# wztzjhn/quantum_basis

Hardware: AMD Instinct MI355X
Metric: lanczos_iters_per_sec (higher is better)
Workload: dtype complex128

## Files before the change

quantum_basis_amd/csrc/qbh_api.cpp:

```cpp
#include <algorithm>
#include <chrono>
#include <cmath>
#include <cstdarg>
#include <cstdlib>
#include <cstring>
#include <initializer_list>
#include <limits>
#include <mutex>
#include <new>
#include <vector>

#include "qbh_api_priv.hpp"

using qbh::d2;
using namespace qbhapi;

namespace qbh {
static thread_local char g_err[512] = "";

void set_error(const char *fmt, ...)
{
    va_list ap;
    va_start(ap, fmt);
    vsnprintf(g_err, sizeof(g_err), fmt, ap);
    va_end(ap);
}

static void parse_debug(const char *e, DebugSw &d)
{
    d = DebugSw{};
    if (!e || !*e) return;
    struct Key { const char *name; int *i; long long *ll; };
    const Key keys[] = {{"flags", &d.flags, nullptr}, {"colmask", &d.colmask, nullptr}, {"tpr", &d.tpr, nullptr}, {"unroll", &d.unroll, nullptr},
                        {"grid", &d.grid, nullptr}, {"wave_tpr", &d.wave_tpr, nullptr}, {"chunk_mult", &d.chunk_mult, nullptr},
                        {"trace_create", &d.trace_create, nullptr}, {"trace_tune", &d.trace_tune, nullptr}, {"trace_dict", &d.trace_dict, nullptr},
                        {"print_ptrs", &d.print_ptrs, nullptr}, {"sec_walk", &d.sec_walk, nullptr}, {"sec_grid", &d.sec_grid, nullptr}, {"sec_tile", &d.sec_tile, nullptr},
                        {"sec_unroll", &d.sec_unroll, nullptr}, {"create_chunk", nullptr, &d.create_chunk},
                        {"force_ragged", &d.force_ragged, nullptr}, {"mf_row", &d.mf_row, nullptr}, {"mf_chunk", &d.mf_chunk, nullptr},
                        {"mf_window", &d.mf_window, nullptr}, {"kronc_abl", &d.kronc_abl, nullptr}, {"kronc_far_chunk", &d.kronc_far_chunk, nullptr},
                        {"kronc_far_ng", &d.kronc_far_ng, nullptr}, {"kronc_far_nt", &d.kronc_far_nt, nullptr}, {"no_far_align", &d.no_far_align, nullptr}, {"far_cols8", &d.far_cols8, nullptr},
                        {"far_vals8", &d.far_vals8, nullptr},
                        {"near_lens", &d.near_lens, nullptr}, {"near_len_cap", &d.near_len_cap, nullptr},
                        {"no_defer", &d.no_defer, nullptr}, {"pipe_nospec", &d.pipe_nospec, nullptr}, {"host_delay_us", &d.host_delay_us, nullptr},
                        {"side_noprio", &d.side_noprio, nullptr}, {"comm_reserve", &d.comm_reserve, nullptr}, {"comm_far_cap", &d.comm_far_cap, nullptr}};
    const std::string all(e);
    size_t pos = 0;
    while (pos <= all.size()) {
        size_t end = all.find(',', pos);
        if (end == std::string::npos) end = all.size();
        const std::string item = all.substr(pos, end - pos);
        pos = end + 1;
        if (item.empty()) continue;
        const size_t eq = item.find('=');
        if (eq == std::string::npos) {
            if (item.find_first_not_of("0123456789") == std::string::npos) d.flags = atoi(item.c_str());
            else fprintf(stderr, "qbhip: QBH_DEBUG: '%s' is not key=value\n", item.c_str());
            continue;
        }
        const std::string k = item.substr(0, eq), v = item.substr(eq + 1);
        bool known = false;
        for (const Key &key : keys)
            if (k == key.name) {
                if (key.i) *key.i = atoi(v.c_str());
                else *key.ll = atoll(v.c_str());
                known = true;
            }
        if (!known) fprintf(stderr, "qbhip: QBH_DEBUG: unknown key '%s'\n", k.c_str());
    }
}

const DebugSw &debug_sw()
{
    static std::mutex mu;
    static std::string seen = "\x01";
    static DebugSw sw[2];
    static int cur = 0;
    const char *e = getenv("QBH_DEBUG");
    std::lock_guard<std::mutex> lock(mu);
    if (seen != (e ? e : "")) {
        seen = e ? e : "";
        cur ^= 1;
        parse_debug(e, sw[cur]);
    }
    return sw[cur];
}
}

extern "C" const char *qbh_last_error(void) { return qbh::g_err; }

extern "C" const char *qbh_strerror(int code)
{
    switch (code) {
    case QBH_OK:        return "success";
    case QBH_EINVAL:    return "invalid argument";
    case QBH_ENODEVICE: return "no HIP device available (libqbhip has no CPU fallback)";
    case QBH_EHIP:      return "HIP runtime call failed";
    case QBH_ENOMEM:    return "out of memory";
    case QBH_ENOTHERM:  return "matrix is not Hermitian";
    case QBH_ECOMM:     return "communicator hook failed";
    case QBH_ENOTNORM:  return "Lanczos start vector is not normalised";
    case QBH_ENOCONV:   return "tridiagonal eigen-solver did not converge";
    case QBH_EUNSUPP:   return "not supported";
    default:            return "unknown error";
    }
}

extern "C" int qbh_version(void) { return QBH_VERSION; }

extern "C" int qbh_device_count(void)
{
    int n = 0;
    if (hipGetDeviceCount(&n) != hipSuccess) {
        (void)hipGetLastError();
        return 0;
    }
    return n;
}

namespace qbhapi {
std::mutex g_defaults_mu;
bool g_have_defaults = false;
qbh_opts g_defaults;
}

extern "C" void qbh_opts_set_default(const qbh_opts *o)
{
    std::lock_guard<std::mutex> lock(g_defaults_mu);
    g_have_defaults = o != nullptr;
    if (o) {
        g_defaults = *o;
        g_defaults.device = -1;
        g_defaults.stream = nullptr;
    }
}

extern "C" void qbh_opts_default(qbh_opts *o)
{
    if (!o) return;
    {
        std::lock_guard<std::mutex> lock(g_defaults_mu);
        if (g_have_defaults) {
            *o = g_defaults;
            return;
        }
    }
    qbh::opts_builtin(o);
}

void qbh::opts_builtin(qbh_opts *o)
{
    o->device = -1;
    o->stream = nullptr;
    o->spmv_kernel = QBH_KERNEL_AUTO;
    o->nnz_per_block = 0;
    o->xcd_swizzle = 2;
    o->value_dict = 1;
    o->profile = 0;
    o->check_hermitian = 1;
    o->real_fast_path = 1;
    o->kron_split = 1;
    o->kron_cols16 = 1;
    o->kron_sliced = 1;
    o->kron_band = 0;
    o->kron_cross_in_near = 1;
    o->kron_coded = -1;
    o->kron_uniform = 7;
    o->gather_parts = 0;
    o->wave_walk = -1;
    o->tile_fold = 1;
    o->autotune = 1;
    o->shard_split = 1;
    o->real_forms = 7;
    o->basis_detect = 1;
    o->sector_orbit = 1;
    o->lanczos_pipeline = 1;
    o->real_wire = 1;
    o->sector_cut = 0;
    o->comm_reserve = 0;
    o->sparse_gather = 1;
    o->major_partition = 0;
    o->kron_minor = 0;
    o->deterministic = 0;
    o->basis_kind = QBH_BASIS_NONE;
    o->n_sites = o->n_up = o->n_dn = 0;
}

namespace qbhapi {

double now_ms()
{
    using namespace std::chrono;
    return duration<double, std::milli>(steady_clock::now().time_since_epoch()).count();
}

int require_device(const qbh_opts *opts, int *dev_out)
// ... 545 lines not shown
                                     int take_ownership, const qbh_opts *opts)
{
    if (!out || !d_ia || !d_ja || !d_val || nrows <= 0 || ncols <= 0 || nnz < 0 || row_offset < 0 ||
        row_offset + nrows > ncols) {
        qbh::set_error("qbh_csr_create_device: invalid argument");
        return QBH_EINVAL;
    }
    if (ncols >= (int64_t)std::numeric_limits<int32_t>::max()) {
        qbh::set_error("ncols %lld does not fit int32 columns", (long long)ncols);
        return QBH_EUNSUPP;
    }
    qbh_csr *A = nullptr;
    QBH_TRY(new_handle(&A, opts));
    A->nrows = nrows;
    A->ncols = ncols;
    A->row_offset = row_offset;
    A->nnz = nnz;
    A->d_ia = d_ia;
    A->d_ja = d_ja;
    A->d_val = reinterpret_cast<d2 *>(d_val);
    A->own_arrays = take_ownership != 0;
    int rc = finalize(A);
    if (rc != QBH_OK) {
        if (!take_ownership && A->d_ia == d_ia) A->own_arrays = false;
        if (!take_ownership && A->d_ia == d_ia) A->d_ia = nullptr, A->d_ja = nullptr, A->d_val = nullptr;
        qbh_csr_destroy(A);
        return rc;
    }
    *out = A;
    return QBH_OK;
}

int qbh::adopt_coded_csr(qbh_csr **out, int64_t nrows, int64_t ncols, int64_t row_offset, int64_t nnz, int64_t *d_ia,
                         int32_t *d_ja, uint8_t *d_code, qbh::d2 *d_dict, int n_dict, const qbh_opts *opts)
{
    if (!out || !d_ia || !d_ja || !d_code || !d_dict || n_dict <= 0 || n_dict > 65536 || nrows <= 0 || nnz < 0 ||
        row_offset < 0 || row_offset + nrows > ncols || ncols >= (int64_t)std::numeric_limits<int32_t>::max()) {
        qbh::set_error("adopt_coded_csr: invalid argument");
        return QBH_EINVAL;
    }
    qbh_csr *A = nullptr;
    QBH_TRY(new_handle(&A, opts));
    A->nrows = nrows;
    A->ncols = ncols;
    A->row_offset = row_offset;
    A->nnz = nnz;
    A->d_ia = d_ia;
    A->d_ja = d_ja;
    A->d_code = d_code;
    A->d_dict = d_dict;
    A->n_dict = n_dict;
    A->own_arrays = true;
    int rc = finalize(A);
    if (rc != QBH_OK) {
        qbh_csr_destroy(A);
        return rc;
    }
    *out = A;
    return QBH_OK;
}

int qbh::adopt_mf_handle(qbh_csr **out, int kind, const std::vector<void *> &own, int64_t bytes, bool values_real, int64_t nrows,
                         int64_t ncols, int64_t row_offset, int64_t nnz_equiv, const qbh_opts *opts)
{
    qbh_csr *A = nullptr;
    if (own.size() > sizeof(A->mf_own) / sizeof(A->mf_own[0])) {
        qbh::set_error("internal: %d device arrays to hand over to a matrix-free operator", (int)own.size());
        return QBH_EHIP;
    }
    QBH_TRY(new_handle(&A, opts));
    A->nrows = nrows;
    A->ncols = ncols;
    A->row_offset = row_offset;
    A->nnz = A->nnz_total = nnz_equiv;
    A->kernel = QBH_KERNEL_ROWS;
    A->values_real = values_real;
    A->n_blocks = (nrows + qbh::kBlock - 1) / qbh::kBlock;
    A->grid = (int)std::min<int64_t>(A->n_blocks, 256 * 8);
    auto fail = [&](int code) {
        qbh_csr_destroy(A);
        return code;
    };
    if (qbh::dev_alloc(&A->d_scal, 16 * sizeof(double)) != hipSuccess) return fail(QBH_ENOMEM);
    if (hipHostMalloc(&A->h_scal, 16 * sizeof(double)) != hipSuccess) return fail(QBH_ENOMEM);
    if (qbh::dev_alloc(&A->d_flag, sizeof(int)) != hipSuccess) return fail(QBH_ENOMEM);
    if (hipMemsetAsync(A->d_flag, 0, sizeof(int), A->stream) != hipSuccess) return fail(QBH_EHIP);
    if (hipEventCreate(&A->ev0) != hipSuccess || hipEventCreate(&A->ev1) != hipSuccess ||
        hipEventCreate(&A->ev2) != hipSuccess || hipEventCreate(&A->ev3) != hipSuccess)
        return fail(QBH_EHIP);
    const size_t nparts = (size_t)std::max(A->grid, qbh::kMaxRedBlocks);
    if (qbh::dev_alloc(&A->d_partials, nparts * 16 * sizeof(double)) != hipSuccess) return fail(QBH_ENOMEM);
    A->stats = qbh_stats{};
    A->stats.ms_spmv_min = std::numeric_limits<double>::infinity();
    A->kind = kind;
    for (void *q : own) A->mf_own[A->n_mf_own++] = q;
    A->mf_bytes = bytes;
    *out = A;
    return QBH_OK;
}

int qbh::adopt_mf_sector(qbh_csr **out, qbh::MfSec *host_tables, qbh::MfSec *dev_tables, int64_t dim, int64_t nnz_equiv,
                         const qbh_opts *opts)
{
    const qbh::MfSec &m = *host_tables;
    std::vector<void *> own;
    for (void *q : {(void *)m.blk, (void *)m.hop, (void *)m.item, (void *)m.ucfg, (void *)m.upell, (void *)m.prank, (void *)m.oid, (void *)m.oek,
                    (void *)m.tpar, (void *)m.usgn, (void *)m.utab, (void *)m.uext, (void *)m.rrow, (void *)m.ria, (void *)m.rja, (void *)m.rval,
                    (void *)dev_tables})
        if (q) own.push_back(q);
    const int64_t bytes = m.n_blocks * (int64_t)sizeof(qbh::MfSecBlock) + m.n_items * 8 + m.n_rrows * 12 + m.rnnz * 20 +
                          (m.orbit ? m.cu * 26 + m.n_orb * m.w_orb * 6 : m.cu * 4 * (1 + m.w_up + m.n_trans));
    QBH_TRY(adopt_mf(out, 3, &qbh_csr::mfsec, host_tables, own, bytes, m.all_real, dim, dim, 0, nnz_equiv, opts));
    (*out)->d_mfsec = dev_tables;
    return QBH_OK;
}

extern "C" int qbh_csr_get_info(const qbh_csr *A, qbh_csr_info *info)
{
    if (!A || !info) return QBH_EINVAL;
    info->nrows = A->nrows;
    info->ncols = A->ncols;
    info->row_offset = A->row_offset;
    const int64_t nnz = A->nnz_total, nb = A->n_blocks + (A->has_rem ? A->rem.n_blocks : 0);
    info->nnz = nnz;
    info->n_blocks = nb;
    info->bytes_matrix = (A->nrows + 1) * 8 * (A->has_rem ? 2 : 1) + nnz * 4 + (A->d_code ? nnz + 256 * 16 : nnz * 16) +
                         (nb + 2) * 12;
    info->bytes_algorithmic = nnz * 20 + (A->nrows + 1) * 8 + A->nrows * 32;
    if (A->kind != 0) info->bytes_matrix = A->mf_bytes;
    info->kernel = A->kind != 0 ? QBH_KERNEL_MATRIX_FREE : A->use_wave ? QBH_KERNEL_WAVE : A->kernel;
    info->value_dict = A->d_code ? A->n_dict : 0;
    info->device = A->device;
    info->stream = (void *)A->stream;
    info->create_ms = A->create_ms;
    info->create_bytes_in = A->create_bytes_in;
    info->kron_minor = A->kron.active ? A->kron.t.S : 0;
    info->kron_far_nnz = A->kron.active ? A->kron.nnz_f : 0;
    info->kron_band = A->kron.active ? A->kron.t.B : 0;
    info->kron_sliced = A->kron.active && A->kron.sliced ? 1 : 0;
    info->kron_inplace = A->kron.active && A->kron.inplace ? 1 : 0;
    info->kron_classes = 0;
    info->kron_cols16 = 0;
    info->kron_cross_nnz = 0;
    info->wire_element_bytes = A->has_comm ? A->wire_bytes_last : 0;
    info->major_partition = A->d_major_inv ? A->major_parts : 0;
    info->gather_sparse = (A->has_comm && A->kron.active && A->kron.comm_tiled && A->kron.sparse) ? 1 : 0;
    info->gather_needed_frac = (A->has_comm && A->kron.active && A->kron.comm_tiled) ? A->kron.need_frac : 1.0;
    info->gather_parts = A->has_comm ? ((A->kron.active && A->kron.comm_tiled) ? A->kron.n_parts : 1) : 0;
    if (A->kron.active) {
        const qbh_csr::KronSplit &K = A->kron;
        info->n_blocks = K.nwb_n + K.nwb_f + K.nwb_x;
        info->bytes_matrix = (A->nrows + 1) * 16 + ((K.sliced ? K.n_groups : A->nrows) + 1) * 8 + (K.n_xrows + 1) * (K.xrow ? 12 : 8) +
                             (K.own_far ? nnz + K.far_slots : nnz) * 20 + (K.nwb_n + K.nwb_f + K.nwb_x + 6) * 16;
        info->bytes_matrix += (A->d_ja ? 0 : -4 * nnz) + 2 * (K.c16_n ? K.nnz_n : 0) + 2 * (K.c16_f ? K.far_slots : 0) + 2 * (K.c8_f ? K.far_slots / 8 + 64 : 0) + 16 * (K.v8_f ? K.far_slots / 8 + 64 : 0) + (K.len_n ? A->nrows + 64 : 0) + ((!A->d_ja && K.own_x) ? 4 * K.nnz_x : 0);
        info->kron_cols16 = (K.c16_n ? 1 : 0) | (K.c16_f ? 2 : 0);
        info->kron_classes = K.map.nc;
        info->kron_cross_nnz = K.nnz_x;
        for (int c = 0; c < K.map.nc; ++c) info->kron_minor = std::max<int64_t>(info->kron_minor, K.map.S[c]);
    }
    info->tuned = A->tuned;
    info->tune_ms_rows = A->tune_ms[0];
    info->tune_ms_wave = A->tune_ms[1];
    info->basis_internal = A->basis.kind;
    info->basis_detected = A->basis.detected ? 1 : 0;
    info->basis_n_sites = A->basis.kind ? A->basis.n_sites : 0;
    info->basis_n_up = A->basis.kind ? A->basis.n_up : 0;
    info->basis_n_dn = A->basis.kind ? A->basis.n_dn : 0;
    info->basis_detect_ms = A->detect_ms;
    info->kron_table_kernel = (A->kronc.active && A->kronc.table_route) ? 1 : 0;
    if (A->kind == 6) info->kron_table_kernel = A->mfqr.tables_lds;
    if (A->kind == 4) info->kron_table_kernel = A->mfq.tables_lds;
    if (A->kronc.active) {
        info->kron_minor = A->kronc.t.S;
        info->kron_far_nnz = A->kronc.sl.active ? A->kronc.sl.slots_f : A->kronc.far_p.nnz;
        info->kron_sliced = A->kronc.sl.active ? 1 : 0;
        info->kron_band = A->kronc.t.B;
    }
    return QBH_OK;
}

extern "C" int qbh_csr_set_basis(qbh_csr *A, int basis_kind, int n_sites, int n_up, int n_dn)
{
    if (!A) return QBH_EINVAL;
    if (A->has_comm || A->has_rem || A->kron.active || A->kronc.active || A->d_code || A->basis.kind != 0 || A->kind != 0) {
        qbh::set_error("qbh_csr_set_basis: needs a plain, unsharded complex128 CSR (value_dict = 0, kron_split = 0 at creation) without a communicator");
        return QBH_EUNSUPP;
    }
    Bind bind(A);
    QBH_HIP(hipStreamSynchronize(A->stream));
    bool applied = false;
    if (basis_kind == QBH_BASIS_DETECT) {
        const double t_d = now_ms();
        QBH_TRY(qbh::basis_detect(A, &applied));
        A->detect_ms = now_ms() - t_d;
    } else {
        QBH_TRY(qbh::basis_to_internal(A, basis_kind, n_sites, n_up, n_dn, &applied));
    }
    if (!applied) return QBH_OK;
    A->opts.basis_kind = A->basis.kind;
    A->opts.n_sites = A->basis.n_sites;
    A->opts.n_up = A->basis.n_up;
    A->opts.n_dn = A->basis.n_dn;
    if (A->opts.kron_split == 0) A->opts.kron_split = 1;
    A->tuned = -1;
    QBH_TRY(build_geometry(A));
    QBH_HIP(hipStreamSynchronize(A->stream));
    return QBH_OK;
}

extern "C" int qbh_sync(const qbh_csr *A)
{
    if (!A) return QBH_EINVAL;
    Bind bind(A);
    QBH_HIP(hipStreamSynchronize(A->stream));
    return QBH_OK;
}

extern "C" int qbh_csr_set_option(qbh_csr *A, const char *name, int value)
{
    if (!A || !name) return QBH_EINVAL;
    const std::string nm(name);
    if (nm == "lanczos_pipeline") A->opts.lanczos_pipeline = value;
    else if (nm == "profile") {
        Bind bind(A);
        harvest_events(A);
        A->opts.profile = value;
    }
    else if (nm == "tile_fold") A->opts.tile_fold = value;
    else if (nm == "comm_reserve") A->opts.comm_reserve = value;
    else {
        qbh::set_error("qbh_csr_set_option: '%s' is not an option that can change after creation", name);
        return QBH_EINVAL;
    }
    return QBH_OK;
}

extern "C" int qbh_csr_major_order(const qbh_csr *A, int32_t *generator_major, int64_t n_major)
{
    if (!A || !generator_major) return QBH_EINVAL;
    if (!A->d_major_inv) {
        qbh::set_error("qbh_csr_major_order: the operator is in the generator's own order");
        return QBH_EUNSUPP;
    }
    if (n_major != A->major_n) return QBH_EINVAL;
    Bind bind(A);
    QBH_HIP(hipMemcpy(generator_major, A->d_major_inv, (size_t)n_major * sizeof(int32_t), hipMemcpyDeviceToHost));
    return QBH_OK;
}

extern "C" int qbh_get_stats(const qbh_csr *Ac, qbh_stats *s, int reset)
{
    qbh_csr *A = const_cast<qbh_csr *>(Ac);
    if (!A) return QBH_EINVAL;
    qbh::harvest_native_comm(A);
    if (s) {
        *s = A->stats;
        if (A->stats.n_spmv == 0) s->ms_spmv_min = 0.0;
    }
    if (reset) {
        A->stats = qbh_stats{};
        A->stats.ms_spmv_min = std::numeric_limits<double>::infinity();
    }
    return QBH_OK;
}


extern "C" int qbh_vec_alloc(qbh_z **d_out, int64_t n)
{
    if (!d_out || n <= 0) return QBH_EINVAL;
    if (qbh_device_count() <= 0) {
        qbh::set_error("no HIP device visible");
        return QBH_ENODEVICE;
    }
    QBH_HIP(qbh::dev_alloc((void **)d_out, (size_t)n * sizeof(qbh_z)));
    return QBH_OK;
}

extern "C" int qbh_vec_free(qbh_z *d)
{
    if (d) QBH_HIP(hipFree(d));
    return QBH_OK;
}

namespace qbhapi {
int vec_h2d(qbh_csr *A, d2 *d_dst, const void *h_src, int64_t n)
{
    if (A->basis.kind == 0) {
        QBH_HIP(hipMemcpyAsync(d_dst, h_src, (size_t)n * sizeof(d2), hipMemcpyHostToDevice, A->stream));
        QBH_HIP(hipStreamSynchronize(A->stream));
        return QBH_OK;
    }
    const int64_t dim = A->nrows;
    if (n % dim != 0) {
        qbh::set_error("vector copy of %lld elements: an operator with a basis map moves whole vectors (%lld elements)", (long long)n, (long long)dim);
        return QBH_EINVAL;
    }
    if (!A->basis.d_stage) QBH_HIP(qbh::dev_alloc(&A->basis.d_stage, (size_t)dim * sizeof(d2)));
    for (int64_t j = 0; j < n / dim; ++j) {
        QBH_HIP(hipMemcpyAsync(A->basis.d_stage, (const char *)h_src + (size_t)j * (size_t)dim * sizeof(d2), (size_t)dim * sizeof(d2),
                               hipMemcpyHostToDevice, A->stream));
        QBH_TRY(qbh::launch_basis_scatter(A->basis.d_map, A->basis.d_stage, d_dst + (size_t)j * (size_t)dim, dim, A->stream));
        QBH_HIP(hipStreamSynchronize(A->stream));
    }
    return QBH_OK;
}
int vec_d2h(qbh_csr *A, void *h_dst, const d2 *d_src, int64_t n)
{
// ... 243 lines not shown
```

quantum_basis_amd/csrc/qbh_api_priv.hpp:

```cpp
#pragma once

#include <initializer_list>
#include <vector>

#include "qbh_internal.hpp"

namespace qbhapi {
using qbh::d2;

double now_ms();
int require_device(const qbh_opts *opts, int *dev_out);
int setup_geometry(qbh_csr *A, const int64_t *d_ia, int64_t nnz, int dict_mode, int *npb_o, int *tpr_o, int *unroll_o, int64_t *window_o,
                   int64_t *n_blocks_o, int32_t **d_rb_o, int64_t **d_bp_o, int *grid_o);
int split_shard(qbh_csr *A);
int setup_wave_geometry(qbh_csr *A, const int64_t *d_ia, int64_t nnz, qbh::WaveDesc **d_wd_o, int64_t *n_wb_o, int *tpr_o, int *grid_o);
int build_geometry(qbh_csr *A);
int autotune_kernel(qbh_csr *A);
int finalize(qbh_csr *A);
int new_handle(qbh_csr **out, const qbh_opts *opts, bool host_arrays = false);
int try_value_dict(qbh_csr *A);
int vec_h2d(qbh_csr *A, d2 *d_dst, const void *h_src, int64_t n);
int vec_d2h(qbh_csr *A, void *h_dst, const d2 *d_src, int64_t n);
void kron_free_aux(qbh_csr *A);
qbh::KronParts kron_parts(const qbh_csr *A);
qbh::KronCols kron_cols_one(int64_t S, int64_t NUg, int B);
int wave_geometry_for(qbh_csr *A, const int64_t *ia, int64_t nr, int64_t nnz, double avg, bool slots, int ops, qbh::WaveDesc **wd_io, int64_t *nwb_o,
                      int *tpr_o, int *grid_o, int64_t shift = 0);
int kron_geometry(qbh_csr *A);
int kron_short_cols(qbh_csr *A);
int kron_near_lens(qbh_csr *A);
int kron_build(qbh_csr *A);
int kron_restore(qbh_csr *A);
void kronc_release(qbh_csr *A);
int kronc_build_sliced(qbh_csr *A, int64_t S, int64_t NU);
int kronc_table_route(qbh_csr *A);
int kronc_build(qbh_csr *A);
int kron_parts_wanted(const qbh_csr *A, const qbh_comm *comm);
int kron_gather_parts(qbh_csr *A, const qbh_comm *comm, int64_t want);
int kron_needed_majors(qbh_csr *A, int nranks, std::vector<uint8_t> *bits_out);
int kron_sparse_setup(qbh_csr *A, const qbh_comm *comm, const std::vector<uint8_t> &bits);
int finish_reduction(qbh_csr *A, int nparts, int ncomp, double *host_out);
void harvest_events(qbh_csr *A);
int next_event_set(qbh_csr *A);
int deferred_reduction(qbh_csr *A, int nparts);
int prof_begin(qbh_csr *A);
int prof_mark(qbh_csr *A, int k);
int cu_count(qbh_csr *A);
int gather_wait(qbh_csr *A, bool expand);
int spmv_finish(qbh_csr *A, int nparts, double *red, bool real_gather);
int spmv_run(qbh_csr *A, const d2 *x, d2 *y, double alpha, double beta, double gamma, double *red);
int enable_real_wire(qbh_csr *A, std::initializer_list<const d2 *> vecs);
int finish_real_wire(qbh_csr *A);
int dotc_run(qbh_csr *A, const d2 *x, const d2 *y, double *res2);
int axpy_norm_run(qbh_csr *A, d2 alpha, const d2 *x, d2 *y, double *nrm2sq);
int axpy_norm_deferred(qbh_csr *A, double scale, const d2 *x, d2 *y, double *dot_out, double *nrm2sq);
int nrm2_run(qbh_csr *A, const d2 *x, double *nrm);
int multmv_host(qbh_csr *A, const qbh_z *x_host, qbh_z *y_host, double beta);
int spmv_kron(qbh_csr *A, const d2 *x, d2 *y, double alpha, double beta, double gamma, double *red);

struct Bind {
    int prev = -1;
    bool ok = true;
    explicit Bind(const qbh_csr *A)
    {
        if (hipGetDevice(&prev) != hipSuccess) prev = -1;
        if (prev != A->device) ok = (hipSetDevice(A->device) == hipSuccess);
    }
    ~Bind()
    {
        if (prev >= 0) (void)hipSetDevice(prev);
    }
};

template <typename T>
class DevPtr {
    T *p_ = nullptr;

  public:
    DevPtr() = default;
    DevPtr(DevPtr &&o) noexcept : p_(o.release()) {}
    DevPtr(const DevPtr &) = delete;
    DevPtr &operator=(const DevPtr &) = delete;
    DevPtr &operator=(DevPtr &&) = delete;
    ~DevPtr() { reset(); }
    hipError_t alloc(size_t count)
    {
        reset();
        const hipError_t e = hipMalloc(&p_, count * sizeof(T));
        if (e != hipSuccess) p_ = nullptr;
        return e;
    }
    T *get() const { return p_; }
    void reset()
    {
        if (p_) (void)hipFree(p_);
        p_ = nullptr;
    }
    T *release()
    {
        T *q = p_;
        p_ = nullptr;
        return q;
    }
};

struct FlagVerdict {
    int rc = QBH_OK;
    hipError_t he = hipSuccess;
    int flag = 0;
    bool ok() const { return rc == QBH_OK && he == hipSuccess; }
};
template <class Launch>
FlagVerdict flag_verdict(qbh_csr *A, Launch &&launch)
{
    FlagVerdict v;
    hipStream_t s = A->stream;
    v.he = hipMemsetAsync(A->d_flag, 0, sizeof(int), s);
    if (v.ok()) v.rc = launch(A->d_flag);
    if (v.ok()) v.he = hipMemcpyAsync(&v.flag, A->d_flag, sizeof(int), hipMemcpyDeviceToHost, s);
    if (v.ok()) v.he = hipStreamSynchronize(s);
    const hipError_t z = hipMemsetAsync(A->d_flag, 0, sizeof(int), s);
    if (v.ok()) v.he = z;
    return v;
}

inline double *scal_buf(qbh_csr *A) { return A->has_comm ? A->comm.d_scal : A->d_scal; }

inline bool kron_path(const qbh_csr *A)
{
    return A->use_wave && A->kron.active && !(A->debug & 1) && A->ovr_yr == nullptr && !(A->real_mode && A->kernel == QBH_KERNEL_ROWS) &&
           (!A->has_comm || A->kron.comm_tiled);
}

inline d2 *tiled_target(const qbh_csr *A)
{
    if (!A->opts.tile_fold || !A->kron.fold || !kron_path(A) || A->kron.map.nc != 1 || A->kron.t.B != 8 || A->kron.t.S < 8) return nullptr;
    if (A->has_comm) return reinterpret_cast<d2 *>(A->comm.d_xsend);
    return (A->nrows == A->ncols && A->kron.xt_cap >= A->nrows) ? A->kron.d_xt : nullptr;
}

inline int tiled_real(const qbh_csr *A) { return (A->has_comm && A->real_wire && A->kron.active && A->kron.comm_tiled) ? 1 : 0; }

inline double *kronc_tiled_target(const qbh_csr *A)
{
    return (A->kronc.active && A->kronc.sl.active && !A->kronc.table_route && !A->has_comm && !A->has_rem && A->opts.tile_fold) ? A->kronc.d_xt : nullptr;
}

struct FoldGuard {
    qbh_csr *A;
    explicit FoldGuard(qbh_csr *a) : A(a)
    {
        A->kron.xt_of = nullptr;
        A->kronc.xt_of = nullptr;
        A->kron.fold = true;
    }
    ~FoldGuard()
    {
        A->kron.xt_of = nullptr;
        A->kron.fold = false;
        A->kronc.xt_of = nullptr;
    }
};

struct WireGuard {
    qbh_csr *A;
    ~WireGuard() { A->real_wire = false; A->real_mode = false; A->xr_of = nullptr; }
};

inline double *packed_target(qbh_csr *A)
{
    if (!A->real_mode || A->kernel != QBH_KERNEL_ROWS) return nullptr;
    if (A->has_comm) return A->real_wire ? reinterpret_cast<double *>(A->comm.d_xsend) : nullptr;
    return (A->nrows == A->ncols) ? A->d_xr : nullptr;
}

}
```

quantum_basis_amd/csrc/qbh_internal.hpp:

```cpp
#pragma once

#include <hip/hip_runtime.h>

#include <cstdint>
#include <cstdio>
#include <string>
#include <vector>

#include "qbhip.h"

namespace qbh {

typedef double d2 __attribute__((ext_vector_type(2)));

constexpr int kBlock = 256;
constexpr int kDictLds = 1024;
constexpr int kMaxRedBlocks = 2048;
constexpr int kRowCap = 1024;

void set_error(const char *fmt, ...);

struct DebugSw {
    int flags = 0;
    int colmask = 0;
    int tpr = 0, unroll = 0, grid = 0, wave_tpr = 0, chunk_mult = 0;
    int trace_create = 0, trace_tune = 0, trace_dict = 0, print_ptrs = 0;
    int sec_walk = -1, sec_grid = 0, sec_unroll = 0, sec_tile = 0;
    long long create_chunk = 0;
    int force_ragged = 0;
    int mf_row = -1, mf_chunk = 0, mf_window = 0;
    int kronc_abl = 0, kronc_far_chunk = 0, kronc_far_ng = 0, kronc_far_nt = 0;
    int no_far_align = 0;
    int far_cols8 = -1;
    int far_vals8 = -1;
    int near_lens = -1;
    int near_len_cap = 0;
    int no_defer = 0;
    int host_delay_us = 0;
    int pipe_nospec = 0;
    int side_noprio = 0;
    int comm_reserve = 0;
    int comm_far_cap = 0;
};
const DebugSw &debug_sw();
void opts_builtin(qbh_opts *o);
inline void opts_generated(const qbh_opts *opts, qbh_opts *out)
{
    if (opts) *out = *opts;
    else opts_builtin(out);
    out->basis_detect = 0;
    if (out->basis_kind == QBH_BASIS_REF_FERMION2) out->basis_kind = QBH_BASIS_NONE;
}

#define QBH_HIP(call)                                                                      \
    do {                                                                                   \
        hipError_t _e = (call);                                                            \
        if (_e != hipSuccess) {                                                            \
            qbh::set_error("%s failed: %s (%s:%d)", #call, hipGetErrorString(_e), __FILE__, \
                           __LINE__);                                                      \
            (void)hipGetLastError();  \
            return (_e == hipErrorOutOfMemory) ? QBH_ENOMEM : QBH_EHIP;                    \
        }                                                                                  \
    } while (0)

#define QBH_TRY(expr)                 \
    do {                              \
        int _rc = (expr);             \
        if (_rc != QBH_OK) return _rc; \
    } while (0)

template <typename... P, typename... A>
inline int launch_kernel(void (*k)(P...), dim3 grid, dim3 block, hipStream_t s, const A &...args)
{
    hipLaunchKernelGGL(k, grid, block, 0, s, args...);
    QBH_HIP(hipGetLastError());
    return QBH_OK;
}

constexpr int kWctrRegions = 3 + 8;

struct WaveDesc {
    int64_t p0;
    int32_t r0;
    int32_t pad;
};

struct SpmvArgs {
    const int64_t *ia;
    const int32_t *ja;
    const d2      *val;
    const uint8_t *code;
    const d2      *dict;
    int            dict_mode;
    const int32_t *rb;
    const int64_t *bp;
    int64_t        n_blocks;
    int64_t        nrows;
    const d2      *xg;
    const double  *xr;
    const d2      *xl;
    d2            *y;
    double         alpha, beta, gamma;
    double        *partials;
    int            swizzle;
    int            chunk_mult;
    int            unroll;
    int            colmask;
    double        *y_re;
    const double  *xl_re;
    const WaveDesc *wd;
    int64_t        n_wb;
    unsigned long long *wctr;
    const d2      *far;
    int64_t        kS, kNU;
    int            kB;
    int            rowmap;
    const struct KronCls *kcls;
    const uint16_t *ja16;
    const uint16_t *ja8;
    const d2      *val8;
    const uint8_t *len8;
    double *chunk_red;
    const d2      *yin;
    const double  *coef;
    int            coef_mode;
};
__device__ __forceinline__ void spmv_args_resolve(SpmvArgs &a)
{
    if (a.coef_mode != 0) {
        a.alpha = a.coef[0];
        if (a.coef_mode == 1) a.beta = a.coef[1];
    }
}

struct KronTile {
    int64_t S, NU;
    int     B;
    __host__ __device__ int64_t tile(int64_t r) const
    {
        const int64_t u = r / S, d = r - u * S;
        const int64_t b = d / B, j = d - b * B;
        const int64_t wB = (S - b * B) < B ? (S - b * B) : B;
        return b * B * NU + u * wB + j;
    }
    __host__ __device__ int64_t orig(int64_t f) const
    {
        const int64_t full = (int64_t)B * NU;
        const int64_t b = f / full;
        const int64_t wB = (S - b * B) < B ? (S - b * B) : B;
        const int64_t rem = f - b * full;
        const int64_t u = rem / wB, j = rem - u * wB;
        return u * S + b * B + j;
    }
};

constexpr int kKronMaxRanks = 16;
struct KronCols {
    int64_t S;
    int     B, nr;
    int64_t cu[kKronMaxRanks + 1];
    __host__ __device__ int64_t tile(int64_t c) const
    {
        const int64_t u = c / S;
        int q = 0;
        while (q + 1 < nr && u >= cu[q + 1]) ++q;
        return cu[q] * S + KronTile{S, cu[q + 1] - cu[q], B}.tile(c - cu[q] * S);
    }
    __host__ __device__ int64_t orig(int64_t i) const
    {
        int q = 0;
        while (q + 1 < nr && i >= cu[q + 1] * S) ++q;
        return cu[q] * S + KronTile{S, cu[q + 1] - cu[q], B}.orig(i - cu[q] * S);
    }
};
constexpr int kKronMaxClasses = 24;
struct KronCls {
    int64_t rbase, S, NU, fbase;
};
struct KronMap {
    int      nc, B, sliced;
    int      cross_near;
    int64_t  U0;
    int64_t  rbase[kKronMaxClasses + 1], S[kKronMaxClasses], NU[kKronMaxClasses];
    int64_t  fbase[kKronMaxClasses + 1];
    KronCols cols;
    __host__ __device__ int cls(int64_t r) const
    {
        int c = 0;
        while (c + 1 < nc && r >= rbase[c + 1]) ++c;
        return c;
    }
    __host__ __device__ bool edge(int c, int64_t d) const { return d >= (S[c] / B) * B; }
    __host__ __device__ int kind(int64_t r, int64_t col) const
    {
        const int c = cls(r);
        const int64_t local = r - rbase[c], u = local / S[c], d = local - u * S[c];
        if (nc == 1) {
            const int64_t cm = col / S[0];
            if (cm == U0 + u) return 0;
            if (col - cm * S[0] == d) return edge(0, d) ? 2 : 1;
            return 2;
        }
        const int64_t lo = rbase[c] + u * S[c];
        if (col >= lo && col < lo + S[c]) return 0;
        if (col >= rbase[c] && col < rbase[c + 1] && (col - rbase[c]) % S[c] == d && !edge(c, d)) return 1;
        return cross_near ? 0 : 2;
    }
    __host__ __device__ int64_t xcol(int64_t col) const
    {
        if (nc == 1) return cols.tile(col);
        const int c = cls(col);
        return rbase[c] + KronTile{S[c], NU[c], B}.tile(col - rbase[c]);
    }
    __host__ __device__ int64_t xcol_orig(int64_t i) const
    {
        if (nc == 1) return cols.orig(i);
        const int c = cls(i);
        return rbase[c] + KronTile{S[c], NU[c], B}.orig(i - rbase[c]);
    }
    __host__ __device__ int64_t frow(int64_t r) const
    {
        const int c = cls(r);
        const int64_t local = r - rbase[c];
        if (sliced && edge(c, local % S[c])) return -1;
        return (sliced ? fbase[c] : rbase[c]) + KronTile{S[c], NU[c], B}.tile(local);
    }
    __host__ __device__ int64_t frow_orig(int64_t f) const
    {
        int c = 0;
        if (sliced) while (c + 1 < nc && f >= fbase[c + 1]) ++c;
        else c = cls(f);
        return rbase[c] + KronTile{S[c], NU[c], B}.orig(f - (sliced ? fbase[c] : rbase[c]));
    }
    __host__ __device__ int64_t nfar_rows() const { return sliced ? fbase[nc] : rbase[nc]; }
};
struct KronParts {
    const int64_t *ia, *ia_n, *fp;
    const int32_t *ja_n, *ja_f;
    const uint16_t *c16_n, *c16_f;
    const d2      *val_n, *val_f;
    const int64_t *ia_x;
    const int32_t *xrow;
    int64_t        n_xrows;
    const int32_t *ja_x;
    const d2      *val_x;
    KronMap        map;
};
int launch_kron_count3(const int64_t *ia, const int32_t *ja, int64_t nrows, const KronMap &map, int32_t *cnt_near, int32_t *cnt_far,
                       int32_t *cnt_x, hipStream_t s);
int launch_kron_far_fill(bool col, const int64_t *ia, const int32_t *ja, const d2 *val, const KronMap &map, const int64_t *fp, int64_t ngroups,
                         int32_t *out_c, d2 *out_v, hipStream_t s);
int launch_kron_part_gather_cols(int part, const int64_t *ia, const int32_t *ja, int64_t r0, int64_t r1, const KronMap &map, const int64_t *iap,
                                 const int32_t *rowidx, int32_t *tmp, hipStream_t s);
int launch_kron_part_gather_vals(int part, const int64_t *ia, const int32_t *ja, const d2 *val, int64_t r0, int64_t r1, const KronMap &map,
                                 const int64_t *iap, const int32_t *rowidx, d2 *tmp, hipStream_t s);
int launch_kron_xrows(const int32_t *cnt_x, int64_t nrows, const int64_t *pos, int32_t *xrow, int32_t *cnt_compact, hipStream_t s);
int launch_kron_flags(const int32_t *cnt, int64_t n, int32_t *flag01, hipStream_t s);
int launch_kron_merge_rows(const KronParts &p, int64_t r0, int64_t r1, int32_t *out_ja, d2 *out_val, int64_t out_base, hipStream_t s);
int launch_kron_remap_cols(int32_t *ja_f, int64_t n, const KronCols &from, const KronCols &to, hipStream_t s);
int launch_kron_combine(const d2 *far, const KronTile &t, const d2 *xl, d2 *y, int64_t n, double alpha, double *partials, int *nparts, hipStream_t s, const double *coef = nullptr);
int launch_kron_cross_rows(const int64_t *ia_x, const int32_t *xrow, int64_t n_xrows, const int32_t *ja_x, const d2 *val_x, const d2 *xt,
                           const KronTile &t, d2 *far, hipStream_t s);
int launch_kron_desc_classes(WaveDesc *wd, int64_t n_wb, const KronCls *cls, int nc, hipStream_t s);
int launch_kron_desc_c16(WaveDesc *wd, int64_t n_wb, int64_t div, bool far, bool undo, hipStream_t s);
int launch_kron_c16_near(const WaveDesc *wd, int64_t n_wb, const int32_t *ja, int64_t S, int64_t col0, uint16_t *out, int *flag, hipStream_t s);
int launch_kron_c16_far(const WaveDesc *wd, const int32_t *ja, int64_t slots, int64_t NU, uint16_t *out, int *flag, hipStream_t s);
int launch_kron_c8_far(const uint16_t *c16, int64_t slots, uint16_t *out, int *flag, hipStream_t s);
int launch_kron_v8_far(const d2 *val, int64_t slots, d2 *out, int *flag, hipStream_t s);
int launch_kron_near_lens(const int64_t *ia, int64_t nrows, const WaveDesc *wd, int64_t n_wb, int cap, uint8_t *out, int *flag, hipStream_t s);
int launch_kron_check2(const int64_t *ia, const int32_t *ja, int64_t nrows, int64_t S, int64_t U0, int *d_flag, hipStream_t s);
int basis_to_internal(qbh_csr *A, int kind, int n_sites, int n_up, int n_dn, bool *applied);
int basis_detect(qbh_csr *A, bool *applied);
int launch_basis_scatter(const uint32_t *map, const d2 *in, d2 *out, int64_t n, hipStream_t s);
int launch_basis_gather(const uint32_t *map, const d2 *in, d2 *out, int64_t n, hipStream_t s);
int launch_basis_scatter_re(const uint32_t *map, const double *in, double *out, int64_t n, hipStream_t s);

hipError_t device_alloc(void **p, size_t bytes);
template <typename T>
inline hipError_t dev_alloc(T **p, size_t bytes)
{
    return device_alloc(reinterpret_cast<void **>(p), bytes);
}

using SpmvKernel = void (*)(SpmvArgs);
int launch_spmv(const SpmvArgs &a, int kernel, int npb, int tpr, int grid, hipStream_t s);
int spmv_grid(int kernel, int64_t n_blocks, int64_t nrows, int tpr);
int rows_kernel_occupancy(int npb, int tpr, int un, int dict_mode);
int vector_kernel_occupancy(int tpr, int un, bool dict);

int launch_spmv_wave(const SpmvArgs &a, int tpr, int grid, hipStream_t s);
int launch_spmv_wave2(const SpmvArgs &a, int tpr, int ops, int grid, hipStream_t s);
int wave2_kernel_occupancy(int tpr, int ops);
int64_t wave2_chunk_slots(int64_t n_wb);
int launch_reduce_chunks(const double *slots, int64_t n_slots, double *partials, int *nparts_out, hipStream_t s);
int wave_kernel_occupancy(int tpr);
int launch_build_wavedesc(const int64_t *d_ia, int64_t nrows, int64_t window, WaveDesc *d_wd, int64_t n_wb, hipStream_t s);

int launch_kron_tile(const d2 *x, d2 *xt, int64_t n, const KronTile &t, hipStream_t s, int xt_real = 0, int *flag = nullptr);
int launch_kron_check(const int64_t *ia, const int32_t *ja, int64_t nrows, int64_t S, int *d_flag, hipStream_t s);
int launch_kron_count(const int64_t *ia, const int32_t *ja, int64_t nrows, const KronTile &t, int32_t *cnt_near, int32_t *cnt_far, hipStream_t s);
int launch_build_slotdesc(const int64_t *gia, int64_t ngroups, int64_t slots, WaveDesc *wd, int64_t n_wb, int64_t shift, hipStream_t s);
int launch_zero_cut_groups(const WaveDesc *wd, int64_t n_wb, int64_t nrows, d2 *far, hipStream_t s);
int launch_kron_group_width(const int32_t *cnt_far, int64_t nrows, int64_t ngroups, int32_t *gw, hipStream_t s);
int launch_kron_fill_sliced(const int64_t *ia, const int32_t *ja, const d2 *val, int64_t nrows, const KronTile &t, const int64_t *ia_n,
                            int32_t *ja_n, d2 *val_n, const int64_t *gia, int64_t ngroups, int32_t *ja_f, d2 *val_f, hipStream_t s);
int launch_kron_fill_codes(const int64_t *ia, const int32_t *ja, const uint8_t *code, int cw, int64_t nrows, const KronTile &t, const int64_t *ia_n,
                           int32_t *ja_n, uint8_t *code_n, const int64_t *ia_f, int32_t *ja_f, uint8_t *code_f, hipStream_t s);
int launch_kron_tile_re(const double *x, double *xt, int64_t n, const KronTile &t, hipStream_t s);
int launch_kron_fill(const int64_t *ia, const int32_t *ja, const d2 *val, int64_t nrows, const KronTile &t, const int64_t *ia_n, int32_t *ja_n,
                     d2 *val_n, const int64_t *ia_f, int32_t *ja_f, d2 *val_f, hipStream_t s);
struct KronPlace {
    const d2 *src;
    d2       *dst;
    int       real, nr, B;
    int64_t   S, NUg, nfb;
    int64_t   cu[kKronMaxRanks + 1];
    int64_t   base[kKronMaxRanks];
    int64_t   off[kKronMaxRanks], len[kKronMaxRanks];
    const int32_t *list;
    int64_t   lo[kKronMaxRanks + 1];
    int64_t   band0, band1;
    int       compact;
    int       skip;
};
int launch_kron_place(const KronPlace &a, hipStream_t s);
struct KronPack {
    const d2 *src;
    d2       *dst;
    int       real, nr, B;
    int64_t   S, NUq, nfb;
    const int32_t *list;
    int64_t   lo[kKronMaxRanks + 1];
    int64_t   base[kKronMaxRanks];
};
int launch_kron_pack(const KronPack &a, hipStream_t s);
int launch_kron_need(const uint16_t *c16_f, const int32_t *ja_f, int64_t far_slots, const int32_t *ja_x, int64_t nnz_x, int64_t S, int64_t NUg, int B,
                     uint8_t *need, hipStream_t s);

int launch_build_rowblocks(const int64_t *d_ia, int64_t nrows, int64_t window, int32_t *d_rb,
                           int64_t *d_bp, int64_t n_blocks, hipStream_t s);
int launch_max_rowlen(const int64_t *d_ia, int64_t nrows, int64_t *d_out, hipStream_t s);
int build_value_dict(const d2 *d_val, int64_t nnz, int cap, uint8_t **d_code_out, d2 **d_dict_out, int *n_out, hipStream_t s);
int exclusive_scan(const int32_t *d_cnt, int64_t n, int64_t *d_ia, hipStream_t s);
int launch_split_count(const int64_t *ia, const int32_t *ja, int64_t nrows, int32_t lo, int32_t hi, int32_t *cnt0, hipStream_t s);
int launch_split_fill(const int64_t *ia, const int32_t *ja, const d2 *val, const uint8_t *code, int64_t nrows, int32_t lo,
                      int32_t hi, const int64_t *ia0, int32_t *ja0, d2 *val0, uint8_t *code0, int64_t *ia1, int32_t *ja1,
                      d2 *val1, uint8_t *code1, int code_w, hipStream_t s);

int blas_grid(int64_t n);
int launch_reduce_partials(const double *partials, int nparts, int ncomp, double *out, hipStream_t s);
int launch_dotc(const d2 *x, const d2 *y, int64_t n, double *partials, hipStream_t s);
int launch_axpy_norm(d2 alpha, const double *alpha_dev, const d2 *x, d2 *y, int64_t n, double *partials, double *yr, int *flag,
                     hipStream_t s, const double *scale_dev = nullptr);
int launch_axpy_norm_tile(d2 alpha, const double *alpha_dev, const d2 *x, d2 *y, d2 *yt, int64_t n, const KronTile &t, double *partials,
                          hipStream_t s, const double *scale_dev = nullptr, int yt_real = 0, int *flag = nullptr);
int launch_lanczos_tail(const double *partials, int nparts, const double *dot, double *state, double *log_slot, double sc_x_host, int use_host,
                        hipStream_t s, const double *sq_ready = nullptr);
int launch_xpby_tile(const d2 *x, double b, d2 *y, d2 *yt, int64_t n, const KronTile &t, hipStream_t s, int yt_real = 0, int *flag = nullptr);
int launch_nrm2sq(const d2 *x, int64_t n, double *partials, hipStream_t s);
int launch_scal(double a, d2 *x, int64_t n, hipStream_t s);
int launch_scal_to(double a, const d2 *x, d2 *y, int64_t n, hipStream_t s);
int launch_axpy_norm_re(double alpha, const double *alpha_dev, const double *x, double *y, int64_t n, double *partials, hipStream_t s,
                        double *yt = nullptr, const KronTile &t = KronTile{1, 1, 1});
int launch_cg_update_re(double alpha, const double *p, const double *pp, double *v, double *r, int64_t n, double *partials, hipStream_t s);
int launch_xpby_re(const double *x, double b, double *y, int64_t n, hipStream_t s);
int launch_dot_re(const double *x, const double *y, int64_t n, double *partials, hipStream_t s);
int launch_nrm2sq_re(const double *x, int64_t n, double *partials, hipStream_t s);
int launch_scal_re(double a, double *x, int64_t n, hipStream_t s);
int launch_xpby(const d2 *x, double b, d2 *y, int64_t n, double *yr, int *flag, hipStream_t s);
int launch_cg_update(d2 alpha, const d2 *p, const d2 *pp, d2 *v, d2 *r, int64_t n, double *partials,
                     hipStream_t s, const double *delta_dev = nullptr, double accu2 = 0.0);
int launch_randomize(d2 *x, double *xr, int64_t n, int64_t global_offset, uint32_t seed, double *partials, hipStream_t s, const int32_t *major_inv = nullptr, int64_t S = 0);
int launch_fill_const(d2 *x, int64_t n, double re, hipStream_t s);
int launch_pack_real(const d2 *x, double *out, int64_t n, int *flag, hipStream_t s);
int launch_unpack_real(const double *in, d2 *out, int64_t n, hipStream_t s);
int launch_imag_norm(const d2 *x, int64_t n, double *partials, hipStream_t s);
struct Coef8 { double v[16]; };
int launch_multi_dot8(const d2 *V, int64_t ldv, const d2 *w, int64_t n, int nv, double *partials, hipStream_t s);
int launch_multi_axpy8(const d2 *V, int64_t ldv, const Coef8 &c, int nv, d2 *w, int64_t n, double *partials, hipStream_t s);
int launch_basis_rotate(d2 *V, int64_t ldv, int64_t n, int m, int keep, const double *d_S, hipStream_t s);

int device_cu_count();

int symmetric_eigen_jacobi(int m, double *a, double *w, double *z);

struct KroncSliced {
    bool      active = false;
    int64_t   S = 0, NU = 0;
    int       nb = 0;
    int64_t   slots_n = 0, slots_f = 0;
    int64_t  *gia_n = nullptr, *gia_f = nullptr;
    uint16_t *ja_n = nullptr;
    uint16_t *ja_f = nullptr;
    bool      near_uni = false;
    uint8_t  *dcode = nullptr;
    bool      far_uni = false;
    int64_t  *tf_ptr = nullptr;
    uint8_t  *code_n = nullptr, *code_f = nullptr;
    double   *d_far = nullptr;
    double   *d_dictr = nullptr;
};
int launch_kronc_near_uniform(const int64_t *ia, const int32_t *ja, const uint8_t *code, int64_t S, int64_t n, int *d_flag, hipStream_t s);
int launch_kronc_s_widths(const int64_t *ia, const int32_t *ja, int64_t S, int nb, int32_t *ws, hipStream_t s);
int launch_kronc_s_fill(const int64_t *ia, const int32_t *ja, const uint8_t *code, int64_t S, int nb, int zcode, const int64_t *gs, uint16_t *scol,
                        uint8_t *scode, hipStream_t s);
int launch_kronc_dcode(const int64_t *ia, const int32_t *ja, const uint8_t *code, int64_t n, int zcode, uint8_t *dcode, hipStream_t s);
int launch_kronc_far_uniform(const int64_t *ia, const int32_t *ja, const uint8_t *code, int64_t S, int64_t n, int *d_flag, hipStream_t s);
int launch_kronc_t_widths(const int64_t *ia, const int32_t *ja, int64_t S, int64_t NU, int32_t *wt, hipStream_t s);
int launch_kronc_t_fill(const int64_t *ia, const int32_t *ja, const uint8_t *code, int64_t S, int64_t NU, int zcode, const int64_t *tp, uint16_t *tcol,
                        uint8_t *tcode, hipStream_t s);
int launch_kronc_widths(const int64_t *ia, const int32_t *ja, int64_t S, int64_t NU, int nb, int32_t *wn, int32_t *wf, hipStream_t s);
int launch_kronc_fill(const int64_t *ia, const int32_t *ja, const uint8_t *code, int64_t S, int64_t NU, int nb, int zcode, const int64_t *gia_n,
                      uint16_t *ja_n, uint8_t *code_n, const int64_t *gia_f, uint16_t *ja_f, uint8_t *code_f, hipStream_t s);
size_t kronc_near_lds_bytes(int64_t S);
int launch_kronc(const KroncSliced &K, const d2 *dict, int n_dict, const double *xt, const double *x, double *y, double alpha, double beta,
                 double gamma, double *partials, unsigned int *ctr, bool static_near, int *nparts_out, hipStream_t s);

int host_threads();
int validate_host_csr(int64_t dim, int64_t nnz, int sym_upper, const int64_t *ia, const int64_t *ja);
int check_hermitian_host(int64_t dim, const int64_t *ia, const int64_t *ja, const d2 *hv);
int build_shard_from_host(int64_t dim, int64_t nnz, int sym, const int64_t *ia, const int64_t *ja, const d2 *val, int64_t r0,
// ... 92 lines not shown
    int w_orb, tile;
};
int launch_mf_sector(const MfSecArgs &a, hipStream_t s, int *nparts_out);

struct MfArgs {
    MfHubbard t;
    MfVec v;
    const uint8_t *dcode = nullptr;
    const double  *ddict = nullptr;
};
int launch_mf_hubbard(const MfArgs &a, int grid, hipStream_t s, int *nparts_out);

struct MfHeis {
    int       n_sites = 0, n_dn = 0, n_bonds = 0, n_chunks = 0;
    uint64_t *binom = nullptr;
    uint64_t *chunk = nullptr;
    uint64_t *mask = nullptr;
    double   *offd = nullptr;
    double   *diag = nullptr;
    int       n_real = 0;
    int       uniform = 0;
    double    offd0 = 0.0, diag0 = 0.0;
};
int launch_mf_heis(const MfHeis &t, const MfVec &v, hipStream_t s, int *nparts_out);
struct MfQudit {
    int       n_sites = 0, d = 0, bits = 0, total = 0, tw = 0;
    int       n_pairs = 0, n_cls = 0, n_ent = 0;
    int       n_slots = 0;
    int       tables_lds = 0;
    int       has_single = 0;
    uint64_t *cum = nullptr;
    int32_t  *pairs = nullptr;
    int32_t  *nrow = nullptr;
    int32_t  *slot = nullptr;
    double   *sdiag = nullptr;
    double   *pdiag = nullptr;
    int32_t  *eout = nullptr;
    d2       *eval = nullptr;
};
int launch_mf_qudit(const MfQudit &t, const MfVec &v, hipStream_t s, int *nparts_out);
struct KondoDev;
struct MfKondo {
    KondoDev *K = nullptr;
};
int launch_mf_kondo(const MfKondo &t, const MfVec &v, hipStream_t s, int *nparts_out);
struct MfQuditRepr {
    const void     *R = nullptr;
    const uint64_t *tab = nullptr;
    const uint64_t *cum = nullptr;
    const uint64_t *reps = nullptr;
    const uint8_t  *info = nullptr;
    const int64_t  *chunk_pos = nullptr;
    int64_t   dim = 0;
    int       n_tab = 0, n_cum = 0;
    int       tables_lds = 0;
};
int launch_mf_qudit_repr(const MfQuditRepr &t, const MfVec &v, hipStream_t s, int *nparts_out);
struct MfKondoRepr {
    const void     *R = nullptr;
    const uint64_t *tab = nullptr;
    const uint64_t *reps = nullptr;
    const uint8_t  *info = nullptr;
    const int64_t  *chunk_pos = nullptr;
    int64_t   dim = 0;
    int       n_tab = 0;
};
int launch_mf_kondo_repr(const MfKondoRepr &t, const MfVec &v, hipStream_t s, int *nparts_out);
int adopt_coded_csr(qbh_csr **out, int64_t nrows, int64_t ncols, int64_t row_offset, int64_t nnz, int64_t *d_ia,
                    int32_t *d_ja, uint8_t *d_code, d2 *d_dict, int n_dict, const qbh_opts *opts);

}

struct CsrPart {
    int64_t  nnz = 0;
    int64_t *d_ia = nullptr;
    int32_t *d_ja = nullptr;
    qbh::d2 *d_val = nullptr;
    uint8_t *d_code = nullptr;
    int      npb = 2048, tpr = 1, unroll = 4, grid = 0;
    int64_t  window = 0, n_blocks = 0;
    int32_t *d_rb = nullptr;
    int64_t *d_bp = nullptr;
    qbh::WaveDesc *d_wd = nullptr;
    int64_t  n_wb = 0;
    int      wtpr = 2, wgrid = 0;
};

struct qbh_csr {
    int          device = 0;
    hipStream_t  stream = nullptr;
    bool         own_stream = false;
    qbh_opts     opts{};

    int64_t nrows = 0, ncols = 0, row_offset = 0, nnz = 0;
    int64_t *d_ia = nullptr;
    int32_t *d_ja = nullptr;
    qbh::d2 *d_val = nullptr;
    uint8_t *d_code = nullptr;
    qbh::d2 *d_dict = nullptr;
    int      n_dict = 0;
    int      code_w = 1;
    int      dict_mode = 0;
    bool     own_arrays = true;

    int      kernel = QBH_KERNEL_STREAM;
    int      npb = 2048;
    int      unroll = 4;
    int      tpr = 4;
    int64_t  window = 0;
    int64_t  n_blocks = 0;
    int32_t *d_rb = nullptr;
    int64_t *d_bp = nullptr;
    int      grid = 0;
    int      chunk_mult = 1;
    struct KronCoded {
        bool     active = false;
        qbh::KronTile t{0, 0, 0};
        CsrPart  near_p, far_p;
        double  *d_xt = nullptr;
        qbh::KroncSliced sl;
        bool     table_route = false;
        qbh::MfHubbard tables;
        const void *xt_of = nullptr;
    } kronc;
    struct KronSplit {
        bool     active = false;
        bool     inplace = false;
        bool     own_far = false;
        bool     own_x = false;
        qbh::KronMap map{};
        qbh::KronTile t{0, 0, 8};
        int64_t  U0 = 0, NUg = 0;
        qbh::KronCols cols{};
        bool     comm_tiled = false;
        int      n_ranks = 1;
        int64_t  rank_cu[qbh::kKronMaxRanks + 1] = {0};
        int32_t *d_need = nullptr;
        int64_t  need_lo[qbh::kKronMaxRanks + 1] = {0};
        double   need_frac = 1.0;
        bool     sparse = false;
        int32_t *d_send_list = nullptr;
        int64_t  send_lo[qbh::kKronMaxRanks + 1] = {0};
        qbh::d2 *d_vsend = nullptr, *d_vrecv = nullptr;
        int64_t  vsend_cap = 0, vrecv_cap = 0;
        int64_t  nnz_n = 0, nnz_f = 0, nnz_x = 0;
        bool     sliced = false;
        int64_t  n_groups = 0, far_slots = 0;
        int64_t *ia_n = nullptr, *ia_f = nullptr;
        int32_t *ja_n = nullptr, *ja_f = nullptr;
        uint16_t *c16_n = nullptr, *c16_f = nullptr;
        uint16_t *c8_f = nullptr;
        qbh::d2 *v8_f = nullptr;
        uint8_t *len_n = nullptr;
        qbh::d2 *val_n = nullptr, *val_f = nullptr;
        qbh::WaveDesc *wd_n = nullptr, *wd_f = nullptr;
        int64_t  nwb_n = 0, nwb_f = 0;
        int      tpr_n = 2, tpr_f = 2, grid_n = 0, grid_f = 0;
        int64_t *ia_x = nullptr;
        int32_t *xrow = nullptr, *ja_x = nullptr;
        qbh::d2 *val_x = nullptr;
        int64_t  n_xrows = 0;
        qbh::WaveDesc *wd_x = nullptr;
        int64_t  nwb_x = 0;
        int      tpr_x = 2, grid_x = 0;
        qbh::KronCls *d_cls = nullptr;
        double  *d_chunk_red = nullptr;
        int64_t  n_chunk_slots = 0;
        qbh::d2 *d_xt = nullptr, *d_far = nullptr;
        int64_t  xt_cap = 0;
        const void *xt_of = nullptr;
        bool     fold = false;
        int      n_parts = 1;
        int64_t  part_blk[9] = {0, 0, 0, 0, 0, 0, 0, 0, 0};
        int64_t  part_band[9] = {0, 0, 0, 0, 0, 0, 0, 0, 0};
        std::vector<int64_t> part_off_len;
    } kron;
    bool     use_wave = false;
    bool     broken = false;
    bool     kron_off = false;
    unsigned long long *d_wctr = nullptr;
    int      tuned = -1;
    double   tune_ms[2] = {0.0, 0.0};
    qbh::WaveDesc *d_wd = nullptr;
    int64_t  n_wb = 0;
    int      wtpr = 2, wgrid = 0;

    double  *d_partials = nullptr;
    double  *d_scal = nullptr;
    double  *h_scal = nullptr;
    qbh::d2 *d_stage_x = nullptr, *d_stage_y = nullptr;
    hipEvent_t ev0 = nullptr, ev1 = nullptr;

    int      kind = 0;
    qbh::MfHubbard mf;
    qbh::MfHeis    mfh;
    qbh::MfSec *mfsec = nullptr;
    qbh::MfSec *d_mfsec = nullptr;
    qbh::MfQudit   mfq;
    qbh::MfKondo   mfk;
    qbh::MfQuditRepr mfqr;
    qbh::MfKondoRepr mfkr;
    void    *mf_own[24] = {};
    int      n_mf_own = 0;
    int64_t  mf_bytes = 0;

    bool     has_rem = false;
    int64_t  nnz_total = 0;
    CsrPart  rem;
    hipEvent_t ev2 = nullptr, ev3 = nullptr;
    bool     ev_pending2 = false;

    bool     values_real = false;
    bool     real_wire = false;
    bool     real_mode = false;
    double  *d_xr = nullptr;
    const void *xr_of = nullptr;
    int     *d_flag = nullptr;

    struct BasisMap {
        int       kind = 0;
        int       n_sites = 0, n_up = 0, n_dn = 0;
        bool      detected = false;
        qbh::KronMap classes{};
        uint32_t *d_map = nullptr;
        qbh::d2  *d_stage = nullptr;
    } basis;

    bool     has_comm = false;
    qbh_comm comm{};
    std::vector<int64_t> comm_cuts;
    int64_t  comm_full = 0;
    int32_t *d_major_inv = nullptr;
    int64_t  major_n = 0, major_S = 0;
    int      major_parts = 0;
    int      wire_bytes_last = 0;
    struct qbh_native_comm *native = nullptr;

    double    create_ms = 0.0, create_ms_upload = 0.0, detect_ms = 0.0;
    int64_t   create_bytes_in = 0;

    qbh_stats stats{};
    bool      ev_pending = false;
    int       debug = 0;
    int ncu = 0;
    qbh::DebugSw dbg;
    const double *ovr_xr = nullptr;
    double       *ovr_yr = nullptr;
    bool      defer_red = false;

    const qbh::d2 *ovr_yin = nullptr;
    const double  *ovr_coef = nullptr;
    struct LzPipe {
        qbh::d2 *d_buf = nullptr;
        int64_t  cap = 0;
        double  *d_state = nullptr;
        double  *h_log = nullptr;
        double  *d_log = nullptr;
        hipEvent_t ev[8] = {nullptr, nullptr, nullptr, nullptr, nullptr, nullptr, nullptr, nullptr};
    } lz;
    struct EvSet {
        hipEvent_t e[4] = {nullptr, nullptr, nullptr, nullptr};
        bool p = false, p2 = false, drop = false;
    };
    EvSet ev_old[3];
    int   n_ev_old = 0;
    bool  ev_keep = false;
    bool  ev_drop = false;
};
constexpr int kLzRing = 8;

namespace qbh {
int adopt_mf_handle(qbh_csr **out, int kind, const std::vector<void *> &own, int64_t bytes, bool values_real, int64_t nrows,
                    int64_t ncols, int64_t row_offset, int64_t nnz_equiv, const qbh_opts *opts);
template <class T>
int adopt_mf(qbh_csr **out, int kind, T qbh_csr::*tables, const T &t, const std::vector<void *> &own, int64_t bytes, bool values_real,
             int64_t nrows, int64_t ncols, int64_t row_offset, int64_t nnz_equiv, const qbh_opts *opts)
{
    QBH_TRY(adopt_mf_handle(out, kind, own, bytes, values_real, nrows, ncols, row_offset, nnz_equiv, opts));
    (*out)->*tables = t;
    return QBH_OK;
}
int adopt_mf_sector(qbh_csr **out, MfSec *host_tables, MfSec *dev_tables, int64_t dim, int64_t nnz_equiv, const qbh_opts *opts);
}
```

quantum_basis_amd/csrc/qbh_kron.hip:

```cpp
#include <algorithm>

#include "qbh_internal.hpp"
#include "qbh_device.hpp"

namespace qbh {

namespace {

__global__ __launch_bounds__(kBlock) void k_kron_check2(const int64_t *ia, const int32_t *ja, int64_t nrows, int64_t S, int64_t U0, int *flag)
{
    for (int64_t r = (int64_t)blockIdx.x * blockDim.x + threadIdx.x; r < nrows; r += (int64_t)gridDim.x * blockDim.x) {
        const int64_t maj = U0 + r / S, mnr = r % S;
        bool bad = false;
        for (int64_t k = ia[r]; k < ia[r + 1]; ++k) {
            const int64_t c = ja[k], cm = c / S;
            bad = bad || (cm != maj && c - cm * S != mnr);
        }
        if (bad) *flag = 1;
    }
}

__global__ __launch_bounds__(kBlock) void k_kron_count3(const int64_t *ia, const int32_t *ja, int64_t nrows, KronMap m, int32_t *cnt_near,
                                                        int32_t *cnt_far, int32_t *cnt_x)
{
// ... 138 lines not shown
            if (cx >= 0 && (which < 0 || cx < best)) { which = 2; best = cx; }
            out_ja[o] = (int32_t)best;
            out_val[o] = which == 0 ? p.val_n[pn] : which == 1 ? p.val_f[fb + fs * k] : which == 2 ? p.val_x[px] : d2{0.0, 0.0};
            if (which == 0) ++pn;
            else if (which == 1) ++k;
            else if (which == 2) ++px;
            ++o;
        }
    }
}

__global__ __launch_bounds__(kBlock) void k_kron_remap_cols(int32_t *ja_f, int64_t n, KronCols from, KronCols to)
{
    for (int64_t i = (int64_t)blockIdx.x * blockDim.x + threadIdx.x; i < n; i += (int64_t)gridDim.x * blockDim.x)
        ja_f[i] = (int32_t)to.tile(from.orig(ja_f[i]));
}

__global__ __launch_bounds__(kBlock) void k_kron_combine(const d2 *far, KronTile t, const d2 *xl, d2 *y, int64_t n, double alpha, double *partials, const double *coef)
{
    __shared__ double red[12];
    double acc[3] = {0.0, 0.0, 0.0};
    if (coef != nullptr) alpha = coef[0];
    for (int64_t r = (int64_t)blockIdx.x * kBlock + threadIdx.x; r < n; r += (int64_t)gridDim.x * kBlock) {
        const d2 v = y[r] + alpha * far[t.tile(r)];
        y[r] = v;
        const d2 xi = xl[r];
        acc[0] += xi.x * v.x + xi.y * v.y;
        acc[1] += xi.x * v.y - xi.y * v.x;
        acc[2] += v.x * v.x + v.y * v.y;
    }
    if (partials != nullptr) {
        for (int c = 0; c < 3; ++c) {
            double v = acc[c];
            for (int off = 32; off > 0; off >>= 1) v += __shfl_xor(v, off, 64);
            if ((threadIdx.x & 63) == 0) red[c * 4 + (threadIdx.x >> 6)] = v;
        }
        __syncthreads();
        if (threadIdx.x == 0)
            for (int c = 0; c < 3; ++c) partials[(size_t)blockIdx.x * 3 + c] = (red[c * 4 + 0] + red[c * 4 + 1]) + (red[c * 4 + 2] + red[c * 4 + 3]);
    }
}

__global__ __launch_bounds__(kBlock) void k_kron_cross_rows(const int64_t *ia_x, const int32_t *xrow, int64_t n_xrows, const int32_t *ja_x,
                                                            const d2 *val_x, const d2 *xt, KronTile t, d2 *far)
{
    const int sub = threadIdx.x & 7;
    for (int64_t i = ((int64_t)blockIdx.x * blockDim.x + threadIdx.x) >> 3; i < ((n_xrows + 31) / 32) * 32; i += ((int64_t)gridDim.x * blockDim.x) >> 3) {
        d2 sum = {0.0, 0.0};
        if (i < n_xrows)
            for (int64_t k = ia_x[i] + sub; k < ia_x[i + 1]; k += 8) sum += cmul(val_x[k], xt[ja_x[k]]);
        for (int off = 4; off > 0; off >>= 1) {
            sum.x += __shfl_xor(sum.x, off, 64);
            sum.y += __shfl_xor(sum.y, off, 64);
        }
        if (sub == 0 && i < n_xrows) far[t.tile(xrow[i])] = sum;
    }
}

__global__ __launch_bounds__(kBlock) void k_kron_desc_classes(WaveDesc *wd, int64_t n_wb, const KronCls *cls, int nc)
{
    for (int64_t w = (int64_t)blockIdx.x * blockDim.x + threadIdx.x; w < n_wb + 2; w += (int64_t)gridDim.x * blockDim.x) {
        const int64_t r = wd[w].r0;
        int c = 0;
        while (c + 1 < nc && r >= cls[c + 1].rbase) ++c;
        wd[w].pad = c;
    }
}

__global__ __launch_bounds__(kBlock) void k_kron_desc_c16(WaveDesc *wd, int64_t n_wb, int64_t div, int far, int undo)
{
    for (int64_t w = (int64_t)blockIdx.x * blockDim.x + threadIdx.x; w < n_wb + 2; w += (int64_t)gridDim.x * blockDim.x) {
        const int32_t cut = far ? (wd[w].pad & 1) : 0;
        const int64_t base = (undo || w >= n_wb) ? 0 : (int64_t)wd[w].r0 / div;
        wd[w].pad = far ? (int32_t)(base << 1) | cut : (int32_t)base;
    }
}

__global__ __launch_bounds__(kBlock) void k_kron_c16_near(const WaveDesc *wd, int64_t n_wb, const int32_t *ja, int64_t S, int64_t col0, uint16_t *out, int *flag)
{
    const int lane = threadIdx.x & 63;
    bool bad = false;
    for (int64_t w = ((int64_t)blockIdx.x * blockDim.x + threadIdx.x) >> 6; w < n_wb; w += ((int64_t)gridDim.x * blockDim.x) >> 6) {
        const int64_t p0 = wd[w].p0, p1 = wd[w + 1].p0, base = col0 + (int64_t)wd[w].pad * S;
        for (int64_t k = p0 + lane; k < p1; k += 64) {
            const int64_t c = (int64_t)ja[k] - base;
            bad = bad || c < 0 || c > 65535;
            out[k] = (uint16_t)c;
        }
    }
    if (bad) *flag = 1;
}

__global__ __launch_bounds__(kBlock) void k_kron_c16_far(const WaveDesc *wd, const int32_t *ja, int64_t slots, int64_t NU, uint16_t *out, int *flag)
{
    bool bad = false;
    for (int64_t i = (int64_t)blockIdx.x * blockDim.x + threadIdx.x; i < slots; i += (int64_t)gridDim.x * blockDim.x) {
        const int64_t band0 = wd[i >> 9].pad >> 1;
        const int64_t col = ja[i], b = col / (8 * NU), rem = col - b * 8 * NU;
        const int64_t c = (rem >> 3) + (b - band0) * NU;
        bad = bad || (rem & 7) != (i & 7) || c < 0 || c > 65535 || wd[i >> 9].p0 != ((i >> 9) << 9);
        out[i] = (uint16_t)c;
    }
    if (bad) *flag = 1;
}

__global__ __launch_bounds__(kBlock) void k_kron_c8_far(const uint16_t *c16, int64_t slots, uint16_t *out, int *flag)
{
    bool bad = false;
    for (int64_t l = (int64_t)blockIdx.x * blockDim.x + threadIdx.x; l < (slots >> 3); l += (int64_t)gridDim.x * blockDim.x) {
        const uint16_t c = c16[l << 3];
        for (int j = 1; j < 8; ++j) bad = bad || c16[(l << 3) + j] != c;
        out[l] = c;
    }
    if (bad) *flag = 1;
}

__global__ __launch_bounds__(kBlock) void k_kron_v8_far(const d2 *val, int64_t slots, d2 *out, int *flag)
{
    bool bad = false;
    for (int64_t l = (int64_t)blockIdx.x * blockDim.x + threadIdx.x; l < (slots >> 3); l += (int64_t)gridDim.x * blockDim.x) {
        const d2 v = val[l << 3];
        const long long re = __double_as_longlong(v.x), im = __double_as_longlong(v.y);
        for (int j = 1; j < 8; ++j) {
            const d2 w = val[(l << 3) + j];
            bad = bad || __double_as_longlong(w.x) != re || __double_as_longlong(w.y) != im;
        }
        out[l] = v;
    }
    if (bad) *flag = 1;
}

__global__ __launch_bounds__(kBlock) void k_kron_near_lens(const int64_t *ia, int64_t nrows, int cap, uint8_t *out, int *flag)
{
    bool bad = false;
    for (int64_t r = (int64_t)blockIdx.x * blockDim.x + threadIdx.x; r < nrows; r += (int64_t)gridDim.x * blockDim.x) {
        const int64_t len = ia[r + 1] - ia[r];
        bad = bad || len < 0 || len > cap;
        out[r] = (uint8_t)len;
    }
    if (bad) *flag = 1;
}

__global__ __launch_bounds__(kBlock) void k_kron_near_lens_check(const WaveDesc *wd, int64_t n_wb, const uint8_t *len, int *flag)
{
    bool bad = false;
    for (int64_t w = (int64_t)blockIdx.x * blockDim.x + threadIdx.x; w < n_wb; w += (int64_t)gridDim.x * blockDim.x) {
        int64_t sum = 0;
        for (int64_t r = wd[w].r0; r < wd[w + 1].r0; ++r) sum += len[r];
        bad = bad || sum != wd[w + 1].p0 - wd[w].p0;
    }
    if (bad) *flag = 1;
}

}

int launch_kron_near_lens(const int64_t *ia, int64_t nrows, const WaveDesc *wd, int64_t n_wb, int cap, uint8_t *out, int *flag, hipStream_t s)
{
    hipLaunchKernelGGL(k_kron_near_lens, dim3(4096), dim3(kBlock), 0, s, ia, nrows, cap, out, flag);
    QBH_HIP(hipGetLastError());
    hipLaunchKernelGGL(k_kron_near_lens_check, dim3(4096), dim3(kBlock), 0, s, wd, n_wb, (const uint8_t *)out, flag);
    QBH_HIP(hipGetLastError());
    return QBH_OK;
}

int launch_kron_desc_c16(WaveDesc *wd, int64_t n_wb, int64_t div, bool far, bool undo, hipStream_t s)
{
    hipLaunchKernelGGL(k_kron_desc_c16, dim3(1024), dim3(kBlock), 0, s, wd, n_wb, div, far ? 1 : 0, undo ? 1 : 0);
    QBH_HIP(hipGetLastError());
    return QBH_OK;
}

int launch_kron_c16_near(const WaveDesc *wd, int64_t n_wb, const int32_t *ja, int64_t S, int64_t col0, uint16_t *out, int *flag, hipStream_t s)
{
    hipLaunchKernelGGL(k_kron_c16_near, dim3(4096), dim3(kBlock), 0, s, wd, n_wb, ja, S, col0, out, flag);
    QBH_HIP(hipGetLastError());
    return QBH_OK;
}

int launch_kron_c16_far(const WaveDesc *wd, const int32_t *ja, int64_t slots, int64_t NU, uint16_t *out, int *flag, hipStream_t s)
{
    hipLaunchKernelGGL(k_kron_c16_far, dim3(4096), dim3(kBlock), 0, s, wd, ja, slots, NU, out, flag);
    QBH_HIP(hipGetLastError());
    return QBH_OK;
}

int launch_kron_c8_far(const uint16_t *c16, int64_t slots, uint16_t *out, int *flag, hipStream_t s)
{
    hipLaunchKernelGGL(k_kron_c8_far, dim3(4096), dim3(kBlock), 0, s, c16, slots, out, flag);
    QBH_HIP(hipGetLastError());
    return QBH_OK;
}

int launch_kron_v8_far(const d2 *val, int64_t slots, d2 *out, int *flag, hipStream_t s)
{
    hipLaunchKernelGGL(k_kron_v8_far, dim3(4096), dim3(kBlock), 0, s, val, slots, out, flag);
    QBH_HIP(hipGetLastError());
    return QBH_OK;
}

int launch_kron_check2(const int64_t *ia, const int32_t *ja, int64_t nrows, int64_t S, int64_t U0, int *d_flag, hipStream_t s)
{
    hipLaunchKernelGGL(k_kron_check2, dim3(4096), dim3(kBlock), 0, s, ia, ja, nrows, S, U0, d_flag);
    QBH_HIP(hipGetLastError());
    return QBH_OK;
}

int launch_kron_count3(const int64_t *ia, const int32_t *ja, int64_t nrows, const KronMap &map, int32_t *cnt_near, int32_t *cnt_far,
                       int32_t *cnt_x, hipStream_t s)
{
    hipLaunchKernelGGL(k_kron_count3, dim3(4096), dim3(kBlock), 0, s, ia, ja, nrows, map, cnt_near, cnt_far, cnt_x);
    QBH_HIP(hipGetLastError());
    return QBH_OK;
}

int launch_kron_far_fill(bool col, const int64_t *ia, const int32_t *ja, const d2 *val, const KronMap &map, const int64_t *fp, int64_t ngroups,
                         int32_t *out_c, d2 *out_v, hipStream_t s)
{
    const dim3 g(4096), b(kBlock);
    if (col) hipLaunchKernelGGL((k_kron_far_fill<true>), g, b, 0, s, ia, ja, val, map, fp, ngroups, out_c, out_v);
    else     hipLaunchKernelGGL((k_kron_far_fill<false>), g, b, 0, s, ia, ja, val, map, fp, ngroups, out_c, out_v);
    QBH_HIP(hipGetLastError());
    return QBH_OK;
}

int launch_kron_part_gather_cols(int part, const int64_t *ia, const int32_t *ja, int64_t r0, int64_t r1, const KronMap &map, const int64_t *iap,
                                 const int32_t *rowidx, int32_t *tmp, hipStream_t s)
{
    const dim3 g(4096), b(kBlock);
    if (part == 0) hipLaunchKernelGGL((k_kron_part_gather<int32_t, 0, true>), g, b, 0, s, ia, ja, ja, r0, r1, map, iap, rowidx, tmp);
    else           hipLaunchKernelGGL((k_kron_part_gather<int32_t, 2, true>), g, b, 0, s, ia, ja, ja, r0, r1, map, iap, rowidx, tmp);
    QBH_HIP(hipGetLastError());
    return QBH_OK;
}

int launch_kron_part_gather_vals(int part, const int64_t *ia, const int32_t *ja, const d2 *val, int64_t r0, int64_t r1, const KronMap &map,
                                 const int64_t *iap, const int32_t *rowidx, d2 *tmp, hipStream_t s)
{
    const dim3 g(4096), b(kBlock);
    if (part == 0) hipLaunchKernelGGL((k_kron_part_gather<d2, 0, false>), g, b, 0, s, ia, ja, val, r0, r1, map, iap, rowidx, tmp);
    else           hipLaunchKernelGGL((k_kron_part_gather<d2, 2, false>), g, b, 0, s, ia, ja, val, r0, r1, map, iap, rowidx, tmp);
    QBH_HIP(hipGetLastError());
    return QBH_OK;
}

int launch_kron_flags(const int32_t *cnt, int64_t n, int32_t *flag01, hipStream_t s)
{
    hipLaunchKernelGGL(k_kron_flags, dim3(2048), dim3(kBlock), 0, s, cnt, n, flag01);
    QBH_HIP(hipGetLastError());
    return QBH_OK;
}

int launch_kron_xrows(const int32_t *cnt_x, int64_t nrows, const int64_t *pos, int32_t *xrow, int32_t *cnt_compact, hipStream_t s)
{
    hipLaunchKernelGGL(k_kron_xrows, dim3(2048), dim3(kBlock), 0, s, cnt_x, nrows, pos, xrow, cnt_compact);
    QBH_HIP(hipGetLastError());
    return QBH_OK;
}

int launch_kron_merge_rows(const KronParts &p, int64_t r0, int64_t r1, int32_t *out_ja, d2 *out_val, int64_t out_base, hipStream_t s)
{
    hipLaunchKernelGGL(k_kron_merge_rows, dim3(4096), dim3(kBlock), 0, s, p, r0, r1, out_ja, out_val, out_base);
    QBH_HIP(hipGetLastError());
    return QBH_OK;
}

int launch_kron_remap_cols(int32_t *ja_f, int64_t n, const KronCols &from, const KronCols &to, hipStream_t s)
{
    if (n <= 0) return QBH_OK;
    hipLaunchKernelGGL(k_kron_remap_cols, dim3(4096), dim3(kBlock), 0, s, ja_f, n, from, to);
    QBH_HIP(hipGetLastError());
    return QBH_OK;
}

int launch_kron_combine(const d2 *far, const KronTile &t, const d2 *xl, d2 *y, int64_t n, double alpha, double *partials, int *nparts, hipStream_t s,
                        const double *coef)
{
    const int g = blas_grid(n);
    hipLaunchKernelGGL(k_kron_combine, dim3(g), dim3(kBlock), 0, s, far, t, xl, y, n, alpha, partials, coef);
    QBH_HIP(hipGetLastError());
    if (nparts) *nparts = g;
    return QBH_OK;
}

int launch_kron_cross_rows(const int64_t *ia_x, const int32_t *xrow, int64_t n_xrows, const int32_t *ja_x, const d2 *val_x, const d2 *xt,
                           const KronTile &t, d2 *far, hipStream_t s)
{
    if (n_xrows <= 0) return QBH_OK;
    const int64_t g = std::min<int64_t>(2048, (n_xrows * 8 + kBlock - 1) / kBlock);
    hipLaunchKernelGGL(k_kron_cross_rows, dim3((unsigned)std::max<int64_t>(g, 1)), dim3(kBlock), 0, s, ia_x, xrow, n_xrows, ja_x, val_x, xt, t, far);
    QBH_HIP(hipGetLastError());
    return QBH_OK;
}

int launch_kron_desc_classes(WaveDesc *wd, int64_t n_wb, const KronCls *cls, int nc, hipStream_t s)
{
    hipLaunchKernelGGL(k_kron_desc_classes, dim3(1024), dim3(kBlock), 0, s, wd, n_wb, cls, nc);
    QBH_HIP(hipGetLastError());
    return QBH_OK;
}

}
```

quantum_basis_amd/csrc/qbh_split.cpp:

```cpp
#include <algorithm>
#include <cstdio>
#include <utility>
#include <vector>

#include "qbh_api_priv.hpp"

using qbh::d2;
using namespace qbhapi;

#define KRON_HIP(call)                                                         \
    do {                                                                       \
        hipError_t e_ = (call);                                                \
        if (e_ != hipSuccess) {                                                \
            (void)hipGetLastError();                                           \
            return fail(e_ == hipErrorOutOfMemory ? QBH_OK : QBH_EHIP);        \
        }                                                                      \
    } while (0)
#define KRON_TRY(expr)                         \
    do {                                       \
        const int rc_ = (expr);                \
        if (rc_ != QBH_OK) return fail(rc_);   \
    } while (0)

namespace {

int verdict_error(const FlagVerdict &v)
{
    QBH_TRY(v.rc);
    const hipError_t device_check = v.he;
    QBH_HIP(device_check);
    return QBH_OK;
}

template <typename T, class Produce>
int derive_into(qbh_csr *A, DevPtr<T> &d, int64_t count, Produce &&produce)
{
    const FlagVerdict v = flag_verdict(A, [&](int *flag) -> int {
        if (hipMemsetAsync(d.get() + count, 0, 64 * sizeof(T), A->stream) != hipSuccess) return QBH_EHIP;
        return produce(d.get(), flag);
    });
    if (v.ok() && !v.flag) return QBH_OK;
    (void)hipGetLastError();
    d.reset();
    return v.rc != QBH_OK ? v.rc : v.he != hipSuccess ? QBH_EHIP : QBH_OK;
}

template <typename T, class Produce>
T *try_derived(qbh_csr *A, int64_t count, Produce &&produce)
{
    DevPtr<T> d;
    if (d.alloc((size_t)count + 64) != hipSuccess) {
        (void)hipGetLastError();
        return nullptr;
    }
    (void)derive_into(A, d, count, produce);
    return d.release();
}

}

namespace qbhapi {
void kron_free_aux(qbh_csr *A)
{
    qbh_csr::KronSplit &K = A->kron;
    for (void *q : {(void *)K.ia_n, (void *)K.ia_f, (void *)K.wd_n, (void *)K.wd_f, (void *)K.d_xt, (void *)K.d_far, (void *)K.ia_x, (void *)K.xrow,
                    (void *)K.wd_x, (void *)K.d_cls, (void *)K.c16_n, (void *)K.c16_f, (void *)K.c8_f, (void *)K.v8_f, (void *)K.len_n, (void *)K.d_chunk_red, (void *)K.d_need, (void *)K.d_send_list, (void *)K.d_vsend, (void *)K.d_vrecv})
        if (q) (void)hipFree(q);
    if (K.own_far) {
        if (K.ja_f) (void)hipFree(K.ja_f);
        if (K.val_f) (void)hipFree(K.val_f);
    }
    if (K.own_x) {
        if (K.ja_x) (void)hipFree(K.ja_x);
        if (K.val_x) (void)hipFree(K.val_x);
    }
    K = qbh_csr::KronSplit{};
}

qbh::KronParts kron_parts(const qbh_csr *A)
{
    const qbh_csr::KronSplit &K = A->kron;
    qbh::KronParts p{};
    p.ia = A->d_ia;
    p.ia_n = K.ia_n;
    p.fp = K.ia_f;
    p.ja_n = K.ja_n;
    p.ja_f = K.ja_f;
    p.c16_n = K.c16_n;
    p.c16_f = K.c16_f;
    p.val_n = K.val_n;
    p.val_f = K.val_f;
    p.ia_x = K.ia_x;
    p.xrow = K.xrow;
    p.n_xrows = K.n_xrows;
    p.ja_x = K.ja_x;
    p.val_x = K.val_x;
    p.map = K.map;
    return p;
}

qbh::KronCols kron_cols_one(int64_t S, int64_t NUg, int B)
{
    qbh::KronCols c{};
    c.S = S;
    c.B = B;
    c.nr = 1;
    c.cu[0] = 0;
    c.cu[1] = NUg;
    return c;
}

int wave_geometry_for(qbh_csr *A, const int64_t *ia, int64_t nr, int64_t nnz, double avg, bool slots, int ops, qbh::WaveDesc **wd_io, int64_t *nwb_o,
                      int *tpr_o, int *grid_o, int64_t shift)
{
    hipStream_t s = A->stream;
    QBH_TRY(qbh::launch_max_rowlen(ia, nr, (int64_t *)A->d_scal, s));
    int64_t maxlen = 0;
    QBH_HIP(hipMemcpyAsync(&maxlen, A->d_scal, sizeof(int64_t), hipMemcpyDeviceToHost, s));
    QBH_HIP(hipStreamSynchronize(s));
    const int64_t window = slots ? 512 : (maxlen <= 256) ? 505 - (maxlen > 0 ? maxlen - 1 : 0) : 249;
    const int64_t n_wb = std::max<int64_t>(1, (nnz + (slots ? shift : 0) + window - 1) / window);
    if (*wd_io) (void)hipFree(*wd_io);
    *wd_io = nullptr;
    QBH_HIP(hipMalloc(wd_io, (size_t)(n_wb + 2) * sizeof(qbh::WaveDesc)));
    if (slots) QBH_TRY(qbh::launch_build_slotdesc(ia, nr, nnz, *wd_io, n_wb, shift, s));
    else       QBH_TRY(qbh::launch_build_wavedesc(ia, nr, window, *wd_io, n_wb, s));
    const int tpr = avg <= 32 ? 2 : avg <= 64 ? 4 : 8;
    int ncu = 256;
    hipDeviceProp_t prop;
    if (hipGetDeviceProperties(&prop, A->device) == hipSuccess && prop.multiProcessorCount > 0) ncu = prop.multiProcessorCount;
    const int occ = std::max(1, ops >= 0 ? qbh::wave2_kernel_occupancy(tpr, ops) : qbh::wave_kernel_occupancy(tpr));
    int64_t g = std::min<int64_t>((int64_t)occ * ncu, ((((n_wb + 3) >> 2) + 7) / 8) * 8);
    g = std::max<int64_t>(8, (g / 8) * 8);
    *nwb_o = n_wb;
    *tpr_o = tpr;
    *grid_o = (int)g;
    return QBH_OK;
}

int kron_geometry(qbh_csr *A)
{
    qbh_csr::KronSplit &K = A->kron;
    const int64_t n = A->nrows;
    QBH_TRY(wave_geometry_for(A, K.ia_n, n, K.nnz_n, (double)K.nnz_n / (double)n, false, K.map.nc > 1 ? 4 : 2, &K.wd_n, &K.nwb_n, &K.tpr_n, &K.grid_n));
    QBH_TRY(wave_geometry_for(A, K.ia_f, K.sliced ? K.n_groups : K.map.nfar_rows(), K.far_slots, (double)K.nnz_f / (double)n, K.sliced, K.sliced ? 3 : 0,
                              &K.wd_f, &K.nwb_f, &K.tpr_f, &K.grid_f));
    if (K.map.nc > 1) {
        std::vector<qbh::KronCls> hc((size_t)K.map.nc + 1);
        for (int c = 0; c <= K.map.nc; ++c)
            hc[(size_t)c] = qbh::KronCls{K.map.rbase[c], c < K.map.nc ? K.map.S[c] : 1, c < K.map.nc ? K.map.NU[c] : 0, K.map.fbase[c]};
        if (!K.d_cls) QBH_HIP(hipMalloc(&K.d_cls, hc.size() * sizeof(qbh::KronCls)));
        QBH_HIP(hipMemcpy(K.d_cls, hc.data(), hc.size() * sizeof(qbh::KronCls), hipMemcpyHostToDevice));
        QBH_TRY(qbh::launch_kron_desc_classes(K.wd_n, K.nwb_n, K.d_cls, K.map.nc, A->stream));
        if (K.nnz_x > 0)
            QBH_TRY(wave_geometry_for(A, K.ia_x, n, K.nnz_x, (double)K.nnz_x / (double)n, false, -1, &K.wd_x, &K.nwb_x, &K.tpr_x, &K.grid_x));
    }
    if (K.d_chunk_red) (void)hipFree(K.d_chunk_red);
    K.d_chunk_red = nullptr;
    K.n_chunk_slots = qbh::wave2_chunk_slots(K.nwb_n);
    QBH_HIP(hipMalloc(&K.d_chunk_red, (size_t)K.n_chunk_slots * 3 * sizeof(double)));
    QBH_HIP(hipMemsetAsync(K.d_chunk_red, 0, (size_t)K.n_chunk_slots * 3 * sizeof(double), A->stream));
    if (K.c16_n) QBH_TRY(qbh::launch_kron_desc_c16(K.wd_n, K.nwb_n, K.t.S, false, false, A->stream));
    if (K.c16_f) QBH_TRY(qbh::launch_kron_desc_c16(K.wd_f, K.nwb_f, K.t.NU, true, false, A->stream));
    QBH_HIP(hipStreamSynchronize(A->stream));
    return QBH_OK;
}

int kron_short_cols(qbh_csr *A)
{
    qbh_csr::KronSplit &K = A->kron;
    if (!A->opts.kron_cols16 || K.map.nc != 1 || !K.inplace || K.c16_n || K.c16_f) return QBH_OK;
    hipStream_t s = A->stream;
    const int64_t S = K.t.S, NU = K.t.NU;
    auto convert = [&](bool far, uint16_t **out) -> int {
        const int64_t cnt = far ? K.far_slots : K.nnz_n;
        auto bases = [&](bool undo) { return qbh::launch_kron_desc_c16(far ? K.wd_f : K.wd_n, far ? K.nwb_f : K.nwb_n, far ? NU : S, far, undo, s); };
        DevPtr<uint16_t> c;
        if (c.alloc((size_t)cnt + 64) != hipSuccess) {
            (void)hipGetLastError();
            return QBH_OK;
        }
        int rc = bases(false);
        if (rc == QBH_OK)
            rc = derive_into(A, c, cnt, [&](uint16_t *o, int *flag) {
                return far ? qbh::launch_kron_c16_far(K.wd_f, K.ja_f, K.far_slots, K.NUg, o, flag, s)
                           : qbh::launch_kron_c16_near(K.wd_n, K.nwb_n, K.ja_n, S, A->row_offset, o, flag, s);
            });
        if (rc != QBH_OK || !c.get()) {
            (void)hipGetLastError();
            const int rc2 = bases(true);
            if (hipStreamSynchronize(s) != hipSuccess || rc2 != QBH_OK) return QBH_EHIP;
            return rc;
        }
        *out = c.release();
        return QBH_OK;
    };
    if (K.nnz_n > 0 && 2 * S <= 65536) QBH_TRY(convert(false, &K.c16_n));
    if (K.sliced && !K.own_far && K.t.B == 8 && 2 * K.NUg <= 65536 && K.far_slots > 0)
        QBH_TRY(convert(true, &K.c16_f));
    if (K.c16_f && K.far_slots % 8 == 0 && qbh::debug_sw().far_cols8 != 0)
        K.c8_f = try_derived<uint16_t>(A, K.far_slots / 8, [&](uint16_t *c, int *flag) { return qbh::launch_kron_c8_far(K.c16_f, K.far_slots, c, flag, s); });
    if (K.c8_f && K.val_f && qbh::debug_sw().far_vals8 != 0)
        K.v8_f = try_derived<d2>(A, K.far_slots / 8, [&](d2 *v, int *flag) { return qbh::launch_kron_v8_far(K.val_f, K.far_slots, v, flag, s); });
    if (K.c16_n && K.c16_f && A->own_arrays && (K.nnz_x == 0 || K.own_x)) {
        (void)hipFree(A->d_ja);
        A->d_ja = nullptr;
    }
    if (K.c16_n) K.ja_n = nullptr;
    if (K.c16_f) K.ja_f = nullptr;
    return QBH_OK;
}

int kron_near_lens(qbh_csr *A)
{
    qbh_csr::KronSplit &K = A->kron;
    const qbh::DebugSw &dbg = qbh::debug_sw();
    if (K.len_n || K.map.nc != 1 || K.nnz_n <= 0 || !K.ia_n || !K.wd_n || dbg.near_lens == 0) return QBH_OK;
    const int cap = (dbg.near_len_cap > 0 && dbg.near_len_cap < 255) ? dbg.near_len_cap : 255;
    K.len_n = try_derived<uint8_t>(
        A, A->nrows, [&](uint8_t *l, int *flag) { return qbh::launch_kron_near_lens(K.ia_n, A->nrows, K.wd_n, K.nwb_n, cap, l, flag, A->stream); });
    return QBH_OK;
}
}

namespace {

bool kron_applies(const qbh_csr *A)
{
    if (A->kron.active) return false;
    if (!A->use_wave || A->kind != 0 || A->has_rem || A->nnz <= 0 || !A->own_arrays || !A->d_val || A->kron_off) return false;
    if (A->opts.kron_split == 0 || (A->debug & 1)) return false;
    if (A->opts.kron_split == 1 && (double)A->nnz * ((double)A->ncols / (double)A->nrows) < 1e8) return false;
    if (A->opts.real_fast_path && A->values_real) return false;
    return true;
}

struct KronBuild {
    qbh_csr *const A;
    qbh_csr::KronSplit &K;
    const int64_t n;
    const hipStream_t s;
    const bool multi;
    int rc = QBH_OK;
    bool touched = false;
    int64_t nfr = 0;
    DevPtr<int32_t> cn, cf, cx;
    int64_t n_chunks = 0;
    std::vector<int32_t> rb;
    std::vector<int64_t> nb;
    DevPtr<d2> chunk;
    DevPtr<int32_t> d_rb;
    DevPtr<int64_t> d_bp;
    DevPtr<d2> far_v, x_v;
    DevPtr<int32_t> far_c, x_c;

    explicit KronBuild(qbh_csr *a)
        : A(a), K(a->kron), n(a->nrows), s(a->stream), multi(a->basis.kind == QBH_BASIS_SPIN_SECTOR && a->basis.classes.nc > 1)
    {
    }

    bool stop(int code)
    {
        rc = code;
        return false;
    }
    bool fail(int code)
    {
        kron_free_aux(A);
        if (touched) {
            if (code == QBH_OK) code = QBH_EHIP;
            qbh::set_error("Kronecker split: the in-place conversion failed half way; the operator is unusable");
            A->broken = true;
        }
        return stop(code);
    }

    bool map_classes()
    {
        if (A->nrows != A->ncols || A->row_offset != 0) return stop(QBH_OK);
        K.map = A->basis.classes;
        K.map.sliced = 1;
        K.map.cross_near = A->opts.kron_cross_in_near ? 1 : 0;
        K.t = qbh::KronTile{K.map.S[0], K.map.NU[0], 8};
        K.U0 = 0;
        K.NUg = 0;
        K.cols = kron_cols_one(1, n, 8);
        return true;
    }
    bool map_two_species()
    {
        const int64_t S = A->opts.kron_minor;
        if (S <= 1 || S >= A->ncols || A->ncols % S != 0 || A->nrows % S != 0 || A->row_offset % S != 0) return stop(QBH_OK);
        const int64_t NU = A->nrows / S, NUg = A->ncols / S, U0 = A->row_offset / S;
        const FlagVerdict v = flag_verdict(A, [&](int *flag) { return qbh::launch_kron_check2(A->d_ia, A->d_ja, n, S, U0, flag, s); });
        if (!v.ok()) return stop(verdict_error(v));
        if (v.flag) return stop(QBH_OK);
        int B = 8;
        while (B > 2 && (double)NUg * B * 16 > 2.5e6) B >>= 1;
        {
            const int b = A->opts.kron_band;
            if (b == 2 || b == 4 || b == 8 || b == 16) B = b;
        }
        K.t = qbh::KronTile{S, NU, B};
        K.U0 = U0;
        K.NUg = NUg;
        K.cols = kron_cols_one(S, NUg, B);
        qbh::KronMap m{};
        m.nc = 1;
        m.B = B;
        m.U0 = U0;
        m.rbase[0] = 0;
        m.rbase[1] = n;
        m.S[0] = S;
        m.NU[0] = NU;
        m.fbase[0] = 0;
        m.fbase[1] = (S / B) * B * NU;
        m.cols = K.cols;
        const int want_sliced = A->opts.kron_sliced;
        m.sliced = (want_sliced && B == 8 && S >= 8) ? 1 : 0;
        K.map = m;
        return true;
    }

    bool counts()
    {
        nfr = K.map.nfar_rows();
        KRON_HIP(cn.alloc((size_t)n));
        KRON_HIP(cf.alloc((size_t)std::max<int64_t>(nfr, n)));
        KRON_HIP(cx.alloc((size_t)n));
        KRON_HIP(hipMemsetAsync(cf.get(), 0, (size_t)std::max<int64_t>(nfr, n) * sizeof(int32_t), s));
        KRON_TRY(qbh::launch_kron_count3(A->d_ia, A->d_ja, n, K.map, cn.get(), cf.get(), cx.get(), s));
        KRON_HIP(hipMalloc(&K.ia_n, (size_t)(n + 1) * sizeof(int64_t)));
        KRON_TRY(qbh::exclusive_scan(cn.get(), n, K.ia_n, s));
        KRON_HIP(hipMemcpy(&K.nnz_n, K.ia_n + n, sizeof(int64_t), hipMemcpyDeviceToHost));
        return true;
    }

    bool far_layout()
    {
        K.sliced = false;
        K.n_groups = nfr / 8;
        if (K.map.sliced && !far_sliced()) return false;
        if (!K.sliced) {
            KRON_HIP(hipMalloc(&K.ia_f, (size_t)(nfr + 1) * sizeof(int64_t)));
            KRON_TRY(qbh::exclusive_scan(cf.get(), nfr, K.ia_f, s));
            KRON_HIP(hipMemcpy(&K.nnz_f, K.ia_f + nfr, sizeof(int64_t), hipMemcpyDeviceToHost));
            K.far_slots = K.nnz_f;
            K.n_groups = (nfr + 7) / 8;
        }
        return true;
    }
    bool far_sliced()
    {
        DevPtr<int32_t> gw;
        DevPtr<int64_t> gia;
        int64_t slots = 0, maxgw = 0, far_true = 0;
        KRON_HIP(gw.alloc((size_t)std::max<int64_t>(K.n_groups, 1)));
        KRON_TRY(qbh::launch_kron_group_width(cf.get(), nfr, K.n_groups, gw.get(), s));
        KRON_HIP(gia.alloc((size_t)(K.n_groups + 1)));
        KRON_TRY(qbh::exclusive_scan(gw.get(), K.n_groups, gia.get(), s));
        {
            DevPtr<int64_t> far_ptr;
            KRON_HIP(far_ptr.alloc((size_t)(nfr + 1)));
            KRON_TRY(qbh::exclusive_scan(cf.get(), nfr, far_ptr.get(), s));
            KRON_HIP(hipMemcpy(&far_true, far_ptr.get() + nfr, sizeof(int64_t), hipMemcpyDeviceToHost));
        }
        KRON_HIP(hipMemcpy(&slots, gia.get() + K.n_groups, sizeof(int64_t), hipMemcpyDeviceToHost));
        KRON_TRY(qbh::launch_max_rowlen(gia.get(), K.n_groups, (int64_t *)A->d_scal, s));
        KRON_HIP(hipMemcpyAsync(&maxgw, A->d_scal, sizeof(int64_t), hipMemcpyDeviceToHost, s));
        KRON_HIP(hipStreamSynchronize(s));
        gw.reset();
        const int want_sliced = A->opts.kron_sliced;
        K.nnz_f = far_true;
        if ((want_sliced == 2 || multi || slots - far_true <= far_true / 8) && maxgw <= 504 && slots < ((int64_t)1 << 40) && K.n_groups > 0) {
            K.ia_f = gia.release();
// ... 17 lines not shown
        if (multi) {
            KRON_HIP(hipMalloc(&K.ia_x, (size_t)(n + 1) * sizeof(int64_t)));
            KRON_TRY(qbh::exclusive_scan(cx.get(), n, K.ia_x, s));
            KRON_HIP(hipMemcpy(&K.nnz_x, K.ia_x + n, sizeof(int64_t), hipMemcpyDeviceToHost));
            K.n_xrows = K.nnz_x > 0 ? n : 0;
        } else {
            DevPtr<int32_t> fl, cc;
            DevPtr<int64_t> pos;
            KRON_HIP(fl.alloc((size_t)n));
            KRON_HIP(pos.alloc((size_t)(n + 1)));
            KRON_TRY(qbh::launch_kron_flags(cx.get(), n, fl.get(), s));
            KRON_TRY(qbh::exclusive_scan(fl.get(), n, pos.get(), s));
            KRON_HIP(hipMemcpy(&K.n_xrows, pos.get() + n, sizeof(int64_t), hipMemcpyDeviceToHost));
            if (K.n_xrows > 0) {
                KRON_HIP(hipMalloc(&K.xrow, (size_t)K.n_xrows * sizeof(int32_t)));
                KRON_HIP(cc.alloc((size_t)K.n_xrows));
                KRON_HIP(hipMalloc(&K.ia_x, (size_t)(K.n_xrows + 1) * sizeof(int64_t)));
                KRON_TRY(qbh::launch_kron_xrows(cx.get(), n, pos.get(), K.xrow, cc.get(), s));
                KRON_TRY(qbh::exclusive_scan(cc.get(), K.n_xrows, K.ia_x, s));
                KRON_HIP(hipMemcpy(&K.nnz_x, K.ia_x + K.n_xrows, sizeof(int64_t), hipMemcpyDeviceToHost));
            }
        }
        cn.reset();
        cf.reset();
        cx.reset();
        return true;
    }

    bool worth_it()
    {
        if (K.nnz_f == 0 || K.nnz_n + K.nnz_f + K.nnz_x != A->nnz) return fail(QBH_OK);
        if (multi && (double)K.nnz_x > 0.4 * (double)A->nnz) return fail(QBH_OK);
        if (multi && K.map.cross_near && (double)K.nnz_f < 0.15 * (double)A->nnz) return fail(QBH_OK);
        return true;
    }

    bool staging()
    {
        KRON_TRY(qbh::launch_max_rowlen(A->d_ia, n, (int64_t *)A->d_scal, s));
        int64_t maxlen = 0;
        KRON_HIP(hipMemcpyAsync(&maxlen, A->d_scal, sizeof(int64_t), hipMemcpyDeviceToHost, s));
        KRON_HIP(hipStreamSynchronize(s));
        const int64_t cw = std::max<int64_t>((int64_t)1 << 26, 4 * maxlen);
        n_chunks = (A->nnz + cw - 1) / cw;
        KRON_HIP(far_v.alloc((size_t)K.far_slots));
        KRON_HIP(far_c.alloc((size_t)K.far_slots));
        if (K.nnz_x > 0) {
            KRON_HIP(x_v.alloc((size_t)K.nnz_x));
            KRON_HIP(x_c.alloc((size_t)K.nnz_x));
        }
        KRON_HIP(chunk.alloc((size_t)(cw + maxlen)));
        KRON_HIP(d_rb.alloc((size_t)(n_chunks + 1)));
        KRON_HIP(d_bp.alloc((size_t)(n_chunks + 1)));
        const int64_t far_len = multi ? K.map.nfar_rows() + 8 : n;
        KRON_HIP(hipMalloc(&K.d_far, (size_t)far_len * sizeof(d2)));
        KRON_HIP(hipMemsetAsync(K.d_far, 0, (size_t)far_len * sizeof(d2), s));
        KRON_TRY(qbh::launch_build_rowblocks(A->d_ia, n, cw, d_rb.get(), d_bp.get(), n_chunks, s));
        rb.resize((size_t)n_chunks + 1);
        KRON_HIP(hipMemcpyAsync(rb.data(), d_rb.get(), rb.size() * sizeof(int32_t), hipMemcpyDeviceToHost, s));
        KRON_HIP(hipStreamSynchronize(s));
        nb.resize((size_t)n_chunks + 1);
        for (int64_t c = 0; c <= n_chunks; ++c) KRON_HIP(hipMemcpyAsync(&nb[(size_t)c], K.ia_n + rb[(size_t)c], sizeof(int64_t), hipMemcpyDeviceToHost, s));
        KRON_HIP(hipStreamSynchronize(s));
        return true;
    }

    bool far_and_cross()
    {
        KRON_TRY(qbh::launch_kron_far_fill(false, A->d_ia, A->d_ja, A->d_val, K.map, K.ia_f, K.n_groups, nullptr, far_v.get(), s));
        KRON_TRY(qbh::launch_kron_far_fill(true, A->d_ia, A->d_ja, A->d_val, K.map, K.ia_f, K.n_groups, far_c.get(), nullptr, s));
        if (K.nnz_x > 0) {
            const int64_t nx = multi ? n : K.n_xrows;
            KRON_TRY(qbh::launch_kron_part_gather_vals(2, A->d_ia, A->d_ja, A->d_val, 0, nx, K.map, K.ia_x, K.xrow, x_v.get(), s));
            KRON_TRY(qbh::launch_kron_part_gather_cols(2, A->d_ia, A->d_ja, 0, nx, K.map, K.ia_x, K.xrow, x_c.get(), s));
        }
        KRON_HIP(hipStreamSynchronize(s));
        return true;
    }

    bool compact_near()
    {
        touched = true;
        if (!compact(A->d_val, [&](int64_t r0, int64_t r1, d2 *out) {
                return qbh::launch_kron_part_gather_vals(0, A->d_ia, A->d_ja, A->d_val, r0, r1, K.map, K.ia_n, nullptr, out, s);
            }))
            return false;
        if (!compact(A->d_ja, [&](int64_t r0, int64_t r1, int32_t *out) {
                return qbh::launch_kron_part_gather_cols(0, A->d_ia, A->d_ja, r0, r1, K.map, K.ia_n, nullptr, out, s);
            }))
            return false;
        K.ja_n = A->d_ja;
        K.val_n = A->d_val;
        return true;
    }
    template <typename T, class Gather>
    bool compact(T *arr, Gather &&gather)
    {
        T *stage = reinterpret_cast<T *>(chunk.get());
        for (int64_t c = 0; c < n_chunks; ++c) {
            const int64_t r0 = rb[(size_t)c], r1 = rb[(size_t)c + 1], cnt = nb[(size_t)c + 1] - nb[(size_t)c];
            if (r1 <= r0 || cnt <= 0) continue;
            KRON_TRY(gather(r0, r1, stage));
            KRON_HIP(hipMemcpyAsync(arr + nb[(size_t)c], stage, (size_t)cnt * sizeof(T), hipMemcpyDeviceToDevice, s));
        }
        return true;
    }

    bool place()
    {
        int64_t tail = K.nnz_n;
        const bool own_x = !multi && K.nnz_x >= 32 && !qbh::debug_sw().no_far_align;
        if (own_x && ((K.nnz_n + 31) / 32) * 32 + K.far_slots <= A->nnz) tail = ((K.nnz_n + 31) / 32) * 32;
        if (tail + K.far_slots + (own_x ? 0 : K.nnz_x) <= A->nnz) {
            KRON_HIP(hipMemcpyAsync(A->d_val + tail, far_v.get(), (size_t)K.far_slots * sizeof(d2), hipMemcpyDeviceToDevice, s));
            KRON_HIP(hipMemcpyAsync(A->d_ja + tail, far_c.get(), (size_t)K.far_slots * sizeof(int32_t), hipMemcpyDeviceToDevice, s));
            KRON_HIP(hipStreamSynchronize(s));
            far_v.reset();
            far_c.reset();
            K.ja_f = A->d_ja + tail;
            K.val_f = A->d_val + tail;
            K.own_far = false;
            tail += K.far_slots;
        } else {
            K.ja_f = far_c.release();
            K.val_f = far_v.release();
            K.own_far = true;
        }
        if (K.nnz_x > 0 && own_x) {
            K.ja_x = x_c.release();
            K.val_x = x_v.release();
            K.own_x = true;
        } else if (K.nnz_x > 0) {
            KRON_HIP(hipMemcpyAsync(A->d_val + tail, x_v.get(), (size_t)K.nnz_x * sizeof(d2), hipMemcpyDeviceToDevice, s));
            KRON_HIP(hipMemcpyAsync(A->d_ja + tail, x_c.get(), (size_t)K.nnz_x * sizeof(int32_t), hipMemcpyDeviceToDevice, s));
            KRON_HIP(hipStreamSynchronize(s));
            K.ja_x = A->d_ja + tail;
            K.val_x = A->d_val + tail;
            x_v.reset();
            x_c.reset();
        }
        KRON_HIP(hipStreamSynchronize(s));
        chunk.reset();
        d_rb.reset();
        d_bp.reset();
        K.inplace = true;
        return true;
    }

    bool finish()
    {
        KRON_TRY(kron_geometry(A));
        KRON_TRY(kron_short_cols(A));
        KRON_TRY(kron_near_lens(A));
        if (qbh::debug_sw().print_ptrs)
            fprintf(stderr, "qbhip kron arrays: ia %p ja %p val %p | ia_n %p fp %p | ja_f %p val_f %p | wd_n %p wd_f %p | far %p | nnz_n %lld far_slots %lld\n", (void *)A->d_ia,
                    (void *)A->d_ja, (void *)A->d_val, (void *)K.ia_n, (void *)K.ia_f, (void *)K.ja_f, (void *)K.val_f, (void *)K.wd_n, (void *)K.wd_f, (void *)K.d_far,
                    (long long)K.nnz_n, (long long)K.far_slots);
        return true;
    }
};

}

namespace qbhapi {
int kron_build(qbh_csr *A)
{
    if (!kron_applies(A)) return QBH_OK;
    KronBuild b(A);
    A->kron.active = (b.multi ? b.map_classes() : b.map_two_species()) && b.counts() && b.far_layout() && b.cross_layout() && b.worth_it() &&
                     b.staging() && b.far_and_cross() && b.compact_near() && b.place() && b.finish();
    return b.rc;
}

int kron_restore(qbh_csr *A)
{
    if (!A->kron.active) return QBH_OK;
    hipStream_t s = A->stream;
    QBH_HIP(hipStreamSynchronize(s));
    int32_t *nja = nullptr;
    d2 *nval = nullptr;
    if (hipMalloc(&nja, (size_t)A->nnz * sizeof(int32_t)) != hipSuccess || hipMalloc(&nval, (size_t)A->nnz * sizeof(d2)) != hipSuccess) {
        (void)hipGetLastError();
        if (nja) (void)hipFree(nja);
        qbh::set_error("Kronecker split: no room to merge the parts back into a CSR (%.1f GB needed beside the operator)", A->nnz * 20e-9);
        return QBH_ENOMEM;
    }
    int rc = qbh::launch_kron_merge_rows(kron_parts(A), 0, A->nrows, nja, nval, 0, s);
    if (rc == QBH_OK && hipStreamSynchronize(s) != hipSuccess) rc = QBH_EHIP;
    if (rc != QBH_OK) {
        (void)hipFree(nja);
        (void)hipFree(nval);
        return rc;
    }
    if (A->d_ja) (void)hipFree(A->d_ja);
    (void)hipFree(A->d_val);
    A->d_ja = nja;
    A->d_val = nval;
    kron_free_aux(A);
    A->kron_off = true;
    return QBH_OK;
}

void kronc_release(qbh_csr *A)
{
    qbh_csr::KronCoded &K = A->kronc;
    for (CsrPart *P : {&K.near_p, &K.far_p})
        for (void *q : {(void *)P->d_ia, (void *)P->d_ja, (void *)P->d_code, (void *)P->d_rb, (void *)P->d_bp})
            if (q) (void)hipFree(q);
    if (K.d_xt) (void)hipFree(K.d_xt);
    for (void *q : {(void *)K.tables.tgt_u, (void *)K.tables.val_u, (void *)K.tables.pk_d})
        if (q) (void)hipFree(q);
    for (void *q : {(void *)K.sl.gia_n, (void *)K.sl.gia_f, (void *)K.sl.ja_n, (void *)K.sl.ja_f, (void *)K.sl.code_n, (void *)K.sl.code_f, (void *)K.sl.d_far, (void *)K.sl.d_dictr, (void *)K.sl.tf_ptr, (void *)K.sl.dcode})
        if (q) (void)hipFree(q);
    K = qbh_csr::KronCoded{};
}
}

namespace {

using KroncUniformCheck = int (*)(const int64_t *, const int32_t *, const uint8_t *, int64_t, int64_t, int *, hipStream_t);
FlagVerdict kronc_uniform(qbh_csr *A, int bit, KroncUniformCheck launch, int64_t S)
{
    if (!(A->opts.kron_uniform & bit)) {
        FlagVerdict no;
        no.flag = 1;
        return no;
    }
    return flag_verdict(A, [&](int *flag) { return launch(A->d_ia, A->d_ja, A->d_code, S, A->nrows, flag, A->stream); });
}

constexpr size_t kKroncPad = 1024;
template <typename T>
hipError_t kronc_stream(T **out, int64_t slots, hipStream_t s)
{
    const hipError_t e = hipMalloc(out, ((size_t)slots + kKroncPad) * sizeof(T));
    return e != hipSuccess ? e : hipMemsetAsync(*out + slots, 0, kKroncPad * sizeof(T), s);
}

struct KroncHost {
    std::vector<int64_t> tp, gs;
    std::vector<uint16_t> tcol, scol;
    std::vector<uint8_t> tcode, scode;
    std::vector<double> dictr;
    explicit KroncHost(const qbh::KroncSliced &L)
        : tp((size_t)L.NU + 1), gs((size_t)L.nb + 1), tcol((size_t)L.slots_f), scol((size_t)L.slots_n), tcode((size_t)L.slots_f),
          scode((size_t)L.slots_n), dictr(256)
    {
    }
};
int kronc_download(qbh_csr *A, KroncHost *h)
{
    const qbh::KroncSliced &L = A->kronc.sl;
    QBH_HIP(hipStreamSynchronize(A->stream));
    QBH_HIP(hipMemcpy(h->tp.data(), L.tf_ptr, h->tp.size() * 8, hipMemcpyDeviceToHost));
    QBH_HIP(hipMemcpy(h->gs.data(), L.gia_n, h->gs.size() * 8, hipMemcpyDeviceToHost));
    QBH_HIP(hipMemcpy(h->tcol.data(), L.ja_f, h->tcol.size() * 2, hipMemcpyDeviceToHost));
    QBH_HIP(hipMemcpy(h->tcode.data(), L.code_f, h->tcode.size(), hipMemcpyDeviceToHost));
    QBH_HIP(hipMemcpy(h->scol.data(), L.ja_n, h->scol.size() * 2, hipMemcpyDeviceToHost));
    QBH_HIP(hipMemcpy(h->scode.data(), L.code_n, h->scode.size(), hipMemcpyDeviceToHost));
    QBH_HIP(hipMemcpy(h->dictr.data(), L.d_dictr, 256 * 8, hipMemcpyDeviceToHost));
    return QBH_OK;
}

struct AmpCodes {
    std::vector<double> amp{0.0};
    int code(double v)
    {
        for (size_t c = 0; c < amp.size(); ++c)
            if (amp[c] == v) return (int)c;
        if (amp.size() == 16) return -1;
        amp.push_back(v);
        return (int)amp.size() - 1;
    }
};
typedef std::vector<std::vector<std::pair<uint32_t, uint8_t>>> HopRows;

bool kronc_decode_t(const KroncHost &h, int64_t NU, AmpCodes *amp, HopRows *tu)
{
    for (int64_t u = 0; u < NU; ++u) {
        const int64_t base = h.tp[(size_t)u], w = h.tp[(size_t)u + 1] - base, nu = w >> 2;
        for (int64_t k = 0; k < w; ++k) {
            const int64_t at = base + (k & 3) * nu + (k >> 2);
            const double v = h.dictr[h.tcode[(size_t)at]];
            if (v == 0.0) continue;
            const int c = amp->code(v);
            if (c < 0) return false;
            (*tu)[(size_t)u].push_back({(uint32_t)h.tcol[(size_t)at], (uint8_t)c});
        }
    }
    return true;
}

bool kronc_decode_s(const KroncHost &h, int64_t S, int nb, AmpCodes *amp, HopRows *td)
{
    for (int64_t b = 0; b < nb; ++b) {
        const int64_t base = h.gs[(size_t)b], w = (h.gs[(size_t)b + 1] - base) >> 4;
        for (int64_t j = 0; j < 16 && b * 16 + j < S; ++j)
            for (int64_t k = 0; k < w; ++k) {
                const int64_t at = base + (16 * (k & 3) + j) * (w >> 2) + (k >> 2);
                const double v = h.dictr[h.scode[(size_t)at]];
                if (v == 0.0) continue;
                const int c = amp->code(v);
                if (c < 0) return false;
                (*td)[(size_t)(b * 16 + j)].push_back({(uint32_t)h.scol[(size_t)at], (uint8_t)c});
            }
    }
// ... 214 lines not shown
```

quantum_basis_amd/csrc/qbh_spmv_kron.cpp:

```cpp
#include <algorithm>
#include <cstdio>
#include <vector>

#include "qbh_api_priv.hpp"

using qbh::d2;
using namespace qbhapi;

namespace {

typedef qbh_csr::KronSplit KronSplit;

struct KronCall {
    qbh_csr  *A;
    const d2 *x, *xl;
    d2       *y;
    double    alpha, beta, gamma;
    double   *red;
    int       walk;
    int       realw;
    bool      sparse;
    int       parts;
    bool      async_gather;
    int64_t   nfb, w_edge;
// ... 128 lines not shown

int gather_in_parts(const KronCall &c)
{
    const qbh_comm &cm = c.A->comm;
    int hrc = 0;
    for (int k = 0; k < c.parts && hrc == 0; ++k) {
        const int64_t *ol = c.A->kron.part_off_len.data() + (size_t)k * 2 * (size_t)cm.nranks;
        hrc = c.realw ? cm.allgather_part_begin_w(cm.ctx, k, c.parts, ol, 1) : cm.allgather_part_begin(cm.ctx, k, c.parts, ol);
    }
    return gather_started(hrc);
}

int sparse_place_own(const KronCall &c, const d2 *send)
{
    const KronSplit &K = c.A->kron;
    const int me = c.A->comm.rank;
    qbh::KronPlace po = place_common(c, send);
    for (int q = 0; q <= po.nr; ++q) po.lo[q] = q <= me ? K.need_lo[me] : K.need_lo[me + 1];
    po.band0 = 0;
    po.band1 = c.nfb + (c.w_edge > 0 ? 1 : 0);
    return qbh::launch_kron_place(po, c.A->stream);
}

int sparse_pack(const KronCall &c, const d2 *send)
{
    const KronSplit &K = c.A->kron;
    qbh::KronPack pk{};
    pk.src = send;
    pk.dst = K.d_vsend;
    pk.real = c.realw;
    pk.nr = c.A->comm.nranks;
    pk.B = K.t.B;
    pk.S = K.t.S;
    pk.NUq = K.t.NU;
    pk.nfb = c.nfb;
    pk.list = K.d_send_list;
    for (int q = 0; q <= pk.nr; ++q) pk.lo[q] = K.send_lo[q];
    for (int q = 0; q < pk.nr; ++q) pk.base[q] = K.send_lo[q] * K.t.S;
    return qbh::launch_kron_pack(pk, c.A->stream);
}

int sparse_exchange(const KronCall &c)
{
    const KronSplit &K = c.A->kron;
    const qbh_comm &cm = c.A->comm;
    const int npk = cm.nranks, me = cm.rank;
    std::vector<int64_t> so((size_t)2 * npk), ro((size_t)2 * npk), rb((size_t)npk, 0);
    recv_bases(c.A, rb.data());
    int hrc = 0;
    for (int k = 0; k < c.parts && hrc == 0; ++k) {
        int64_t pb0, pb1;
        bool with_edge;
        part_bands(c, k, &pb0, &pb1, &with_edge);
        for (int q = 0; q < npk; ++q) {
            const int64_t ns = q == me ? 0 : K.send_lo[q + 1] - K.send_lo[q], nr_ = q == me ? 0 : K.need_lo[q + 1] - K.need_lo[q];
            so[(size_t)2 * q] = K.send_lo[q] * K.t.S + pb0 * K.t.B * ns;
            so[(size_t)2 * q + 1] = (pb1 - pb0) * K.t.B * ns + (with_edge ? ns * c.w_edge : 0);
            ro[(size_t)2 * q] = rb[(size_t)q] + pb0 * K.t.B * nr_;
            ro[(size_t)2 * q + 1] = (pb1 - pb0) * K.t.B * nr_ + (with_edge ? nr_ * c.w_edge : 0);
        }
        hrc = cm.exchange_v(cm.ctx, k, c.parts, so.data(), ro.data(), c.realw ? 1 : 2, K.d_vsend, K.d_vrecv);
    }
    return gather_started(hrc);
}

int start_exchange(KronCall &c)
{
    qbh_csr *A = c.A;
    KronSplit &K = A->kron;
    d2 *send = reinterpret_cast<d2 *>(A->comm.d_xsend);
    if (K.xt_of != (const void *)c.x) QBH_TRY(qbh::launch_kron_tile(c.x, send, A->nrows, K.t, A->stream, c.realw, A->d_flag));
    K.xt_of = nullptr;
    c.async_gather = A->comm.allgather_begin && A->comm.allgather_wait;
    if (c.sparse) {
        QBH_TRY(sparse_place_own(c, send));
        QBH_TRY(sparse_pack(c, send));
        QBH_TRY(sparse_exchange(c));
    } else {
        QBH_TRY(c.parts > 1 ? gather_in_parts(c) : gather_whole(c));
    }
    A->stats.n_gather++;
    A->wire_bytes_last = c.realw ? 8 : 16;
    return QBH_OK;
}

int place(const KronCall &c, int k)
{
    const qbh_csr *A = c.A;
    const KronSplit &K = A->kron;
    int64_t pb0, pb1;
    bool with_edge;
    part_bands(c, k, &pb0, &pb1, &with_edge);
    const d2 *gathered = c.realw ? reinterpret_cast<const d2 *>(A->comm.d_xfull_r) : reinterpret_cast<const d2 *>(A->comm.d_xfull);
    qbh::KronPlace pa = place_common(c, c.sparse ? K.d_vrecv : gathered);
    for (int q = 0; q <= pa.nr; ++q) pa.lo[q] = K.need_lo[q];
    pa.band0 = pb0;
    pa.band1 = pb1 + (with_edge ? 1 : 0);
    if (c.sparse) {
        pa.compact = 1;
        recv_bases(A, pa.base);
        pa.skip = A->comm.rank;
        return qbh::launch_kron_place(pa, A->stream);
    }
    for (int q = 0; q < pa.nr; ++q) {
        pa.base[q] = A->comm.row_cuts ? A->comm.row_cuts[q] : (int64_t)q * A->comm.nblk;
        if (c.parts > 1) {
            pa.off[q] = K.part_off_len[((size_t)k * (size_t)pa.nr + (size_t)q) * 2];
            pa.len[q] = K.part_off_len[((size_t)k * (size_t)pa.nr + (size_t)q) * 2 + 1];
        } else {
            pa.off[q] = 0;
            pa.len[q] = (K.rank_cu[q + 1] - K.rank_cu[q]) * K.t.S;
        }
    }
    return qbh::launch_kron_place(pa, A->stream);
}

qbh::SpmvArgs far_args(const KronCall &c)
{
    const qbh_csr *A = c.A;
    const KronSplit &K = A->kron;
    qbh::SpmvArgs f{};
    f.ia = K.ia_f;
    f.ja = K.ja_f;
    f.ja16 = K.c16_f;
    f.ja8 = K.c8_f;
    f.val8 = K.v8_f;
    f.kS = K.t.S;
    f.kNU = K.NUg;
    f.kB = K.t.B;
    f.val = K.val_f;
    f.wd = K.wd_f;
    f.n_wb = K.nwb_f;
    f.nrows = K.map.nfar_rows();
    f.xg = K.d_xt;
    f.xl = c.xl;
    f.y = K.d_far;
    f.alpha = 1.0;
    f.colmask = -1;
    f.chunk_mult = A->chunk_mult;
    f.swizzle = c.walk == 3 ? 3 : 1;
    f.wctr = A->d_wctr ? A->d_wctr + 128 : nullptr;
    return f;
}

int near_args(const KronCall &c, qbh::SpmvArgs *out)
{
    const qbh_csr *A = c.A;
    const KronSplit &K = A->kron;
    qbh::SpmvArgs nr{};
    nr.ia = K.ia_n;
    nr.ja = K.ja_n;
    nr.ja16 = K.c16_n;
    nr.len8 = K.len_n;
    nr.val = K.val_n;
    nr.wd = K.wd_n;
    nr.n_wb = K.nwb_n;
    nr.nrows = A->nrows;
    nr.xg = K.c16_n ? c.xl : c.xl - A->row_offset;
    nr.xl = c.xl;
    nr.y = c.y;
    nr.alpha = c.alpha;
    nr.beta = c.beta;
    nr.gamma = c.gamma;
    nr.colmask = -1;
    nr.chunk_mult = A->chunk_mult;
    nr.kS = K.t.S;
    nr.kNU = K.t.NU;
    nr.kB = K.t.B;
    nr.swizzle = c.walk;
    nr.wctr = A->d_wctr ? A->d_wctr + 256 : nullptr;
    nr.chunk_red = K.d_chunk_red;
    nr.yin = A->ovr_yin;
    nr.coef = A->ovr_coef;
    nr.coef_mode = A->ovr_coef ? 1 : 0;
    if (c.walk == 3 && !K.d_chunk_red) {
        qbh::set_error("Kronecker split: the chunk partials of the near pass were not allocated");
        return QBH_EHIP;
    }
    *out = nr;
    return QBH_OK;
}

qbh::SpmvArgs cross_args(const KronCall &c)
{
    const qbh_csr *A = c.A;
    const KronSplit &K = A->kron;
    qbh::SpmvArgs cr{};
    cr.ia = K.ia_x;
    cr.ja = K.ja_x;
    cr.val = K.val_x;
    cr.wd = K.wd_x;
    cr.n_wb = K.nwb_x;
    cr.nrows = A->nrows;
    cr.xg = K.d_xt;
    cr.xl = c.xl;
    cr.y = c.y;
    cr.alpha = c.alpha;
    cr.beta = 1.0;
    cr.gamma = 0.0;
    cr.coef = A->ovr_coef;
    cr.coef_mode = A->ovr_coef ? 2 : 0;
    cr.colmask = -1;
    cr.chunk_mult = A->chunk_mult;
    cr.swizzle = (A->opts.xcd_swizzle == 3 && !A->opts.deterministic && A->d_wctr) ? 3 : (A->opts.xcd_swizzle == 3 ? 2 : A->opts.xcd_swizzle);
    cr.wctr = A->d_wctr;
    cr.partials = c.red ? A->d_partials : nullptr;
    return cr;
}

int reduce_chunks(const KronCall &c, int *nparts)
{
    const KronSplit &K = c.A->kron;
    if (c.walk != 3) return QBH_OK;
    return qbh::launch_reduce_chunks(K.d_chunk_red, K.n_chunk_slots, c.A->d_partials, nparts, c.A->stream);
}

int near_one_class(const KronCall &c, qbh::SpmvArgs &nr, int *nparts)
{
    qbh_csr *A = c.A;
    const KronSplit &K = A->kron;
    QBH_TRY(qbh::launch_kron_cross_rows(K.ia_x, K.xrow, K.n_xrows, K.ja_x, K.val_x, K.d_xt, K.t, K.d_far, A->stream));
    nr.partials = c.red ? A->d_partials : nullptr;
    QBH_TRY(qbh::launch_spmv_wave2(nr, K.tpr_n, 2, K.grid_n, A->stream));
    if (c.red) QBH_TRY(reduce_chunks(c, nparts));
    return QBH_OK;
}

int near_classes(const KronCall &c, qbh::SpmvArgs &nr, int *nparts)
{
    qbh_csr *A = c.A;
    const KronSplit &K = A->kron;
    nr.kcls = K.d_cls;
    nr.partials = (c.red && K.nnz_x == 0) ? A->d_partials : nullptr;
    QBH_TRY(qbh::launch_spmv_wave2(nr, K.tpr_n, 4, K.grid_n, A->stream));
    if (K.nnz_x == 0) return c.red ? reduce_chunks(c, nparts) : QBH_OK;
    QBH_TRY(qbh::launch_spmv_wave(cross_args(c), K.tpr_x, K.grid_x, A->stream));
    *nparts = K.grid_x;
    return QBH_OK;
}

int apply_one_gpu(const KronCall &c, int *nparts)
{
    qbh_csr *A = c.A;
    KronSplit &K = A->kron;
    hipStream_t s = A->stream;
    QBH_TRY(prof_begin(A));
    if (K.xt_of != (const void *)c.x) {
        if (K.map.nc == 1) {
            QBH_TRY(qbh::launch_kron_tile(c.x, K.d_xt, A->ncols, qbh::KronTile{K.t.S, K.NUg, K.t.B}, s));
        } else {
            for (int k = 0; k < K.map.nc; ++k)
                QBH_TRY(qbh::launch_kron_tile(c.x + K.map.rbase[k], K.d_xt + K.map.rbase[k], K.map.rbase[k + 1] - K.map.rbase[k],
                                              qbh::KronTile{K.map.S[k], K.map.NU[k], K.map.B}, s));
        }
    }
    K.xt_of = nullptr;
    const qbh::SpmvArgs f = far_args(c);
    qbh::SpmvArgs nr;
    QBH_TRY(near_args(c, &nr));
    if (K.sliced) QBH_TRY(qbh::launch_zero_cut_groups(K.wd_f, K.nwb_f, f.nrows, K.d_far, s));
    QBH_TRY(qbh::launch_spmv_wave2(f, K.tpr_f, K.sliced ? 3 : 0, K.grid_f, s));
    nr.far = K.d_far;
    QBH_TRY(K.map.nc == 1 ? near_one_class(c, nr, nparts) : near_classes(c, nr, nparts));
#ifdef QBH_XCD_TIMING
    QBH_TRY(xcd_timing_dump(A));
#endif
#ifdef QBH_WAVE_TIMING
    QBH_TRY(wave_timing_dump(A));
#endif
    return prof_mark(A, 1);
}

void comm_grids(qbh_csr *A, int *grid_n, int *grid_f)
{
    const KronSplit &K = A->kron;
    int reserve = 0, far_cap = K.grid_f;
    if (A->comm.nranks > 1 && A->opts.comm_reserve >= 0) {
        reserve = A->opts.comm_reserve > 0 ? (A->opts.comm_reserve / 8) * 8 : 64;
        far_cap = std::min(K.grid_f, 2 * cu_count(A));
    }
    if (A->dbg.comm_reserve != 0) reserve = A->dbg.comm_reserve > 0 ? (A->dbg.comm_reserve / 8) * 8 : 0;
    if (A->dbg.comm_far_cap != 0) far_cap = A->dbg.comm_far_cap > 0 ? std::min(K.grid_f, A->dbg.comm_far_cap * std::max(A->ncu, 256)) : K.grid_f;
    auto mult8 = [](int g) { return std::max(8, (g / 8) * 8); };
    *grid_n = mult8(std::max(K.grid_n / 2, K.grid_n - reserve));
    *grid_f = mult8(std::max(std::min(far_cap, K.grid_f) / 2, far_cap - reserve));
}

int far_after_gather(const KronCall &c, const qbh::SpmvArgs &f, int grid_f)
{
    qbh_csr *A = c.A;
    const KronSplit &K = A->kron;
    hipStream_t s = A->stream;
    if (c.parts == 1 && !c.sparse) {
        if (c.async_gather) QBH_TRY(gather_wait(A, false));
        QBH_TRY(prof_mark(A, 2));
        QBH_TRY(place(c, 0));
        if (K.sliced) QBH_TRY(qbh::launch_zero_cut_groups(K.wd_f, K.nwb_f, f.nrows, K.d_far, s));
        return qbh::launch_spmv_wave2(f, K.tpr_f, K.sliced ? 3 : 0, grid_f, s);
    }
    QBH_TRY(qbh::launch_zero_cut_groups(K.wd_f, K.nwb_f, f.nrows, K.d_far, s));
    for (int k = 0; k < c.parts; ++k) {
        if (A->comm.allgather_part_wait(A->comm.ctx, k) != 0) {
            qbh::set_error("allgather_part_wait hook failed");
            return QBH_ECOMM;
        }
        if (k == 0) QBH_TRY(prof_mark(A, 2));
// ... 71 lines not shown
```

quantum_basis_amd/csrc/qbh_spmv_wave.hip:

```cpp
#include "qbh_internal.hpp"
#include "qbh_device.hpp"

namespace qbh {

__device__ __forceinline__ void wave_lds_fence()
{
    __builtin_amdgcn_fence(__ATOMIC_RELEASE, "wavefront");
    __builtin_amdgcn_wave_barrier();
    __builtin_amdgcn_fence(__ATOMIC_ACQUIRE, "wavefront");
}

template <int TPR, bool DYN>
__global__ __launch_bounds__(kBlock) void k_spmv_wave(SpmvArgs a)
{
    spmv_args_resolve(a);
    constexpr int U = 8, NW = 64 * U, RP = 64 / TPR;
    __shared__ d2 prod_s[4 * NW];
    __shared__ double red[12];
    const int tid = threadIdx.x, lane = tid & 63, wv = tid >> 6;
    d2 *prod = prod_s + wv * NW;
    const int sub = lane % TPR, rloc = lane / TPR;
    double acc[3] = {0.0, 0.0, 0.0};
    const bool need_y = a.beta != 0.0;
    const bool need_x = a.gamma != 0.0 || a.partials != nullptr;
// ... 42 lines not shown
                    if (need_y) yo = a.yin[r0 + rloc];
                    if (need_x) xi = a.xl[r0 + rloc];
                }
            }
            if (n > 0) {
                const int nm1 = n - 1;
                int c[U];
                d2 v[U], xv[U];
#pragma unroll
                for (int u = 0; u < U; ++u) {
                    const int i = lane + u * 64;
                    c[u] = ntload(a.ja + base + (i < n ? i : nm1)) & a.colmask;
                }
#pragma unroll
                for (int u = 0; u < U; ++u) {
                    const int i = lane + u * 64;
                    v[u] = ntload(a.val + base + (i < n ? i : nm1));
                }
#pragma unroll
                for (int u = 0; u < U; ++u) xv[u] = a.xg[c[u]];
#pragma unroll
                for (int u = 0; u < U; ++u) prod[lane + u * 64] = cmul(v[u], xv[u]);
            }
            wave_lds_fence();
            for (int rbase = 0; rbase < nr; rbase += RP) {
                const int row = rbase + rloc;
                int s = s0, e = e0;
                if (rbase > 0) {
                    s = e = 0;
                    if (row < nr) {
                        s = (int)(a.ia[r0 + row] - base);
                        e = (int)(a.ia[r0 + row + 1] - base);
                    }
                }
                d2 sum = {0.0, 0.0};
                for (int k = s + sub; k < e; k += TPR) sum += prod[k];
#pragma unroll
                for (int off = TPR / 2; off > 0; off >>= 1) {
                    sum.x += __shfl_xor(sum.x, off, 64);
                    sum.y += __shfl_xor(sum.y, off, 64);
                }
                if (sub == 0 && row < nr) {
                    if (rbase == 0) row_epilogue2(a, (int64_t)r0 + row, sum, yo, xi, acc);
                    else            row_epilogue(a, (int64_t)r0 + row, sum, acc);
                }
            }
            wave_lds_fence();
        } else {
            for (int r = 0; r < nr; ++r) {
                const int64_t s = a.ia[r0 + r], e = a.ia[r0 + r + 1];
                d2 sum = {0.0, 0.0};
                for (int64_t k = s + lane; k < e; k += 64) sum += cmul(a.val[k], a.xg[a.ja[k] & a.colmask]);
                sum.x = wave_sum(sum.x);
                sum.y = wave_sum(sum.y);
                if (lane == 0) row_epilogue(a, (int64_t)r0 + r, sum, acc);
            }
        }
    }
    if (a.partials != nullptr) {
#pragma unroll
        for (int c = 0; c < 3; ++c) acc[c] = wave_sum(acc[c]);
        if (lane == 0) {
#pragma unroll
            for (int c = 0; c < 3; ++c) red[c * 4 + wv] = acc[c];
        }
        __syncthreads();
        if (tid == 0) {
#pragma unroll
            for (int c = 0; c < 3; ++c)
                a.partials[(size_t)blockIdx.x * 3 + c] = (red[c * 4 + 0] + red[c * 4 + 1]) + (red[c * 4 + 2] + red[c * 4 + 3]);
        }
    }
}

template <bool DYN>
static SpmvKernel wave_kernel_tpr(int tpr)
{
    switch (tpr) {
    case 2:  return k_spmv_wave<2, DYN>;
    case 4:  return k_spmv_wave<4, DYN>;
    case 8:  return k_spmv_wave<8, DYN>;
    default: return k_spmv_wave<16, DYN>;
    }
}

static SpmvKernel wave_kernel(int tpr, bool dyn)
{
    return dyn ? wave_kernel_tpr<true>(tpr) : wave_kernel_tpr<false>(tpr);
}

static int kernel_occupancy(SpmvKernel k)
{
    int occ = 0;
    if (hipOccupancyMaxActiveBlocksPerMultiprocessor(&occ, k, kBlock, 0) != hipSuccess) {
        (void)hipGetLastError();
        return 0;
    }
    return occ;
}

int launch_spmv_wave(const SpmvArgs &a_in, int tpr, int grid, hipStream_t s)
{
    SpmvArgs a = a_in;
    if (a.yin == nullptr) a.yin = a.y;
    return launch_kernel(wave_kernel(tpr, a.swizzle == 3), grid, kBlock, s, a);
}

int wave_kernel_occupancy(int tpr)
{
    return kernel_occupancy(wave_kernel(tpr, false));
}

__global__ void k_build_wavedesc(const int64_t *ia, int64_t nrows, int64_t window, WaveDesc *wd, int64_t n_wb)
{
    const int64_t w = (int64_t)blockIdx.x * blockDim.x + threadIdx.x;
    if (w > n_wb + 1) return;
    WaveDesc d;
    d.pad = 0;
    if (w >= n_wb) {
        d.p0 = ia[nrows];
        d.r0 = (int32_t)nrows;
    } else {
        const int64_t target = w * window;
        int64_t lo = 0, hi = nrows;
        while (lo < hi) {
            const int64_t mid = (lo + hi) >> 1;
            if (ia[mid] < target) lo = mid + 1;
            else hi = mid;
        }
        d.p0 = ia[lo];
        d.r0 = (int32_t)lo;
    }
    wd[w] = d;
}

int launch_build_wavedesc(const int64_t *d_ia, int64_t nrows, int64_t window, WaveDesc *d_wd, int64_t n_wb, hipStream_t s)
{
    const int64_t n = n_wb + 2;
    return launch_kernel(k_build_wavedesc, (unsigned)((n + 255) / 256), 256, s, d_ia, nrows, window, d_wd, n_wb);
}


#ifndef QBH_NEAR_WAVES
#define QBH_NEAR_WAVES 2
#endif
#ifndef QBH_FAR_WAVES
#define QBH_FAR_WAVES 3
#endif
#ifdef QBH_NT_ROW_STORE
#define QBH_ROW_STORE(p, v) __builtin_nontemporal_store((v), (p))
#else
#define QBH_ROW_STORE(p, v) (*(p) = (v))
#endif
template <int TPR, int OPS, bool DYN, bool C16 = false, bool G8 = false, bool NL = false, bool V8 = false>
__global__ __launch_bounds__(kBlock) __attribute__((amdgpu_waves_per_eu((OPS == 0 || OPS == 3) ? QBH_FAR_WAVES : QBH_NEAR_WAVES, (OPS == 0 || OPS == 3) ? QBH_FAR_WAVES : QBH_NEAR_WAVES))) void k_spmv_wave2(SpmvArgs a)
{
    spmv_args_resolve(a);
    static_assert(!C16 || OPS == 1 || OPS == 2 || OPS == 3, "2-byte columns: the one-class near passes and the sliced far pass");
    static_assert(!G8 || (C16 && OPS == 3), "grouped columns: the sliced far pass with 2-byte columns");
    static_assert(!NL || OPS == 1 || OPS == 2, "row lengths: the one-class near passes");
    static_assert(!V8 || G8, "grouped values: only beside the grouped columns");
    constexpr int NW = 512, RP = 64 / TPR;
    constexpr bool EPI = OPS == 1 || OPS == 2 || OPS == 4, FAR = OPS == 2 || OPS == 4;
    constexpr bool CHUNKRED = DYN && (OPS == 1 || OPS == 2 || OPS == 4);
    constexpr bool MULTI = OPS == 4;
    __shared__ d2 prod_s[4 * NW];
    __shared__ double red[12];
    const int tid = threadIdx.x, lane = tid & 63, wv = tid >> 6;
    d2 *prod = prod_s + wv * NW;
    const int sub = lane % TPR, rloc = lane / TPR;
    double acc[3] = {0.0, 0.0, 0.0};
    const bool need_y = a.beta != 0.0;

    BlockWalk walk((a.n_wb + 3) >> 2, a.swizzle, a.chunk_mult);
    constexpr bool dyn = DYN;
    DynWalk dw;
    auto load_desc = [&](int64_t lb) -> int {
        int64_t w = a.n_wb;
        if (dyn) {
            w = dw.block(lb);
        } else if (lb < walk.per_xcd) {
            w = walk.block(lb) * 4 + wv;
            if (w > a.n_wb) w = a.n_wb;
        }
        return reinterpret_cast<const int *>(a.wd + w)[lane & 7];
    };
    const int64_t step = dyn ? 1 : walk.nslot;
    struct Blk {
        int64_t p0;
        int r0, nr, n;
        bool cont0, cont1;
        int cls;
        int64_t xb;
        int lead;
    };
    const uint32_t kS32 = (uint32_t)a.kS, kB32 = (uint32_t)a.kB;
    const int kLB = 31 - __builtin_clz(kB32 | 1u);
    auto far_at = [&](int64_t row, int c0) -> d2 {
        if constexpr (MULTI) {
            int c = c0;
            while (row >= a.kcls[c + 1].rbase) ++c;
            const KronCls k = a.kcls[c];
            const uint32_t local = (uint32_t)(row - k.rbase), S32 = (uint32_t)k.S, u = local / S32, d = local - u * S32;
            if (d >= ((S32 >> 3) << 3)) return d2{0.0, 0.0};
            return a.far[k.fbase + (int64_t)(d >> 3) * 8 * k.NU + (int64_t)u * 8 + (d & 7)];
        } else {
            const uint32_t r = (uint32_t)row, u = r / kS32, d = r - u * kS32;
            const uint32_t b = d >> kLB, j = d & (kB32 - 1u), rem = kS32 - (b << kLB), wB = rem < kB32 ? rem : kB32;
            return a.far[(int64_t)b * (a.kNU << kLB) + (int64_t)u * wB + j];
        }
    };
    auto decode = [&](int dq) -> Blk {
        const uint32_t q0 = (uint32_t)__builtin_amdgcn_readlane(dq, 0), q1 = (uint32_t)__builtin_amdgcn_readlane(dq, 1);
        const uint32_t q4 = (uint32_t)__builtin_amdgcn_readlane(dq, 4), q5 = (uint32_t)__builtin_amdgcn_readlane(dq, 5);
        Blk b;
        const int64_t pfirst = (int64_t)(((uint64_t)q1 << 32) | q0);
        b.p0 = OPS == 3 ? pfirst : pfirst - (pfirst & 7);
        b.lead = OPS == 3 ? 0 : (int)(pfirst & 7);
        const int64_t p1 = (int64_t)(((uint64_t)q5 << 32) | q4);
        b.r0 = __builtin_amdgcn_readlane(dq, 2);
        b.nr = __builtin_amdgcn_readlane(dq, 6) - b.r0;
        b.cls = MULTI ? __builtin_amdgcn_readlane(dq, 3) : 0;
        b.xb = 0;
        if constexpr (C16) {
            const int64_t pad = (uint32_t)__builtin_amdgcn_readlane(dq, 3);
            b.xb = OPS == 3 ? (pad >> 1) * 8 * a.kNU : pad * a.kS;
        }
        b.cont0 = OPS == 3 && (__builtin_amdgcn_readlane(dq, 3) & 1);
        b.cont1 = OPS == 3 && (__builtin_amdgcn_readlane(dq, 7) & 1);
        if (b.cont1) b.nr += 1;
        b.n = (p1 - b.p0) <= NW ? (int)(p1 - b.p0) : -1;
        return b;
    };
    struct Ops {
        int s, e;
        d2 yo, xi, fr;
    };
    auto group_range = [&](const Blk &b, int gp, int row, int &s_, int &e_, bool &clip) {
        const int gi = row >> 3;
        const int gs = __shfl(gp, gi & 63, 64);
        int ge = __shfl(gp, (gi + 1) & 63, 64);
        if (gi + 1 >= 64) ge = b.n;
        clip = gs < 0 || ge > b.n;
        s_ = (gs < 0 ? 0 : gs) + (row & 7);
        e_ = ge > b.n ? b.n : ge;
    };
    auto issue = [&](const Blk &b, int (&c)[8], d2 (&v)[8], Ops &o) {
        const int nn = b.n > 0 ? b.n : 1;
        const int nm1 = nn - 1;
        const int64_t base = b.n > 0 ? b.p0 : 0;
        if constexpr (G8) {
            const int lm = nm1 >> 3;
            c[0] = ntload(a.ja8 + (base >> 3) + (lane < lm ? lane : lm));
#pragma unroll
            for (int u = 1; u < 8; ++u) c[u] = 0;
        } else {
#pragma unroll
            for (int u = 0; u < 8; ++u) {
                const int i = lane + u * 64;
                if constexpr (C16) c[u] = ntload(a.ja16 + base + (i < nn ? i : nm1));
                else               c[u] = ntload(a.ja + base + (i < nn ? i : nm1)) & a.colmask;
            }
        }
        if constexpr (C16 && OPS != 3) {
            if (b.n > 0 && lane < b.lead) c[0] = 0;
        }
        if constexpr (V8) {
            const int lm = nm1 >> 3;
#pragma unroll
            for (int u = 0; u < 8; ++u) {
                const int l = (lane >> 3) + 8 * u;
                v[u] = ntload(a.val8 + (base >> 3) + (l < lm ? l : lm));
            }
        } else {
#pragma unroll
            for (int u = 0; u < 8; ++u) {
                const int i = lane + u * 64;
                v[u] = ntload(a.val + base + (i < nn ? i : nm1));
            }
        }
        if (OPS == 3) {
            const int64_t ng = (a.nrows + 7) >> 3;
            int64_t g = (int64_t)b.r0 + lane;
            g = g < ng ? g : ng;
            int64_t rel = a.ia[g] - base;
            rel = rel < -4096 ? -4096 : rel > 4096 ? 4096 : rel;
            o.s = (int)rel;
            o.e = 0;
        } else if constexpr (NL) {
            const int last = b.nr > 0 ? b.nr - 1 : 0;
            o.s = a.len8[(int64_t)b.r0 + (lane < last ? lane : last)];
            o.e = 0;
        } else {
            const bool mine = rloc < b.nr;
            const int64_t row = mine ? (int64_t)b.r0 + rloc : 0;
            o.s = (int)(a.ia[row] - base);
            o.e = (int)(a.ia[row + 1] - base);
            if (!mine) o.s = o.e = 0;
        }
    };
    auto issue_ops = [&](const Blk &b, Ops &o) {
        if (EPI) {
            int64_t row = rloc < b.nr ? (int64_t)b.r0 + rloc : 0;
            if (MULTI && rloc >= b.nr) row = b.r0 < a.nrows ? b.r0 : a.nrows - 1;
            o.yo = a.yin[row];
            o.xi = a.xl[row];
            o.fr = FAR ? far_at(row, b.cls) : d2{0.0, 0.0};
            if (!need_y) o.yo = d2{0.0, 0.0};
        }
    };
#ifndef QBH_BUF_MODE
#define QBH_BUF_MODE 1
#endif
    constexpr bool BUF = DYN && (QBH_BUF_MODE == 2 || (QBH_BUF_MODE == 1 && OPS == 3));
    constexpr int CAP = 256;
    __shared__ d2 rbuf_s[BUF ? 4 * CAP : 1];
    d2 *rbuf = rbuf_s + (BUF ? wv * CAP : 0);
    int64_t buf_r0 = 0;
    int buf_n = 0, buf_nb = 0;
    bool at_first = false, at_last = false, merge_first = false, direct = !BUF;
    auto emit = [&](int64_t row, d2 v, bool atomic) {
        if (OPS == 3) {
            if (row < a.nrows) {
                if (atomic) {
                    double *yp = reinterpret_cast<double *>(a.y + row);
                    unsafeAtomicAdd(yp, v.x);
                    unsafeAtomicAdd(yp + 1, v.y);
                } else {
                    QBH_ROW_STORE(a.y + row, v);
                }
            }
        } else {
            QBH_ROW_STORE(a.y + row, v);
        }
    };
    auto flush = [&]() {
        if (BUF && buf_n > 0) {
            wave_lds_fence();
            for (int i = lane; i < buf_n; i += 64) emit(buf_r0 + i, rbuf[i], OPS == 3 && ((i < 8 && at_first) || (i >= buf_n - 8 && at_last)));
            wave_lds_fence();
            buf_n = 0;
        }
    };
    auto open_block = [&](int64_t first, int nrows_blk, bool c0, bool fits) {
        if (BUF) {
            if (buf_n > 0 && (!fits || first != buf_r0 + buf_n - (c0 ? 8 : 0) || first + nrows_blk - buf_r0 > CAP)) flush();
            direct = !fits || nrows_blk > CAP;
            if (!direct) {
                if (buf_n == 0) {
                    buf_r0 = first;
                    at_first = c0;
                    merge_first = false;
                } else {
                    merge_first = c0;
                }
                buf_nb = buf_n;
            }
        }
    };
    auto close_block = [&](int64_t first, int nrows_blk, bool c1) {
        if (BUF && !direct) {
            buf_n = (int)(first + nrows_blk - buf_r0);
            at_last = c1;
        }
    };
    auto finish_row = [&](int64_t row, d2 sum, d2 yo, d2 xi, d2 fr, bool clip) {
        d2 v = sum;
        if (EPI) {
            if (FAR) sum += fr;
            v = a.alpha * sum + a.beta * yo + a.gamma * xi;
            acc[0] += xi.x * v.x + xi.y * v.y;
            acc[1] += xi.x * v.y - xi.y * v.x;
            acc[2] += v.x * v.x + v.y * v.y;
        }
        if (BUF && !direct) {
            const int idx = (int)(row - buf_r0);
            if (OPS == 3 && merge_first && idx < buf_nb) v += rbuf[idx];
            rbuf[idx] = v;
        } else {
            emit(row, v, clip);
        }
    };

    constexpr int NHOP =
#ifdef QBH_NO_XCD_STEAL
        1;
#else
        dyn ? 8 : 1;
#endif
#ifdef QBH_WAVE_TIMING
    unsigned long long tm[4] = {0, 0, 0, 0}, nblk = 0;
#endif
    int64_t red_slot = -1;
    auto red_flush = [&]() {
        if constexpr (CHUNKRED) {
            if (red_slot >= 0) {
#pragma unroll
                for (int c = 0; c < 3; ++c) acc[c] = wave_sum(acc[c]);
                if (lane == 0) {
                    double *slot = a.chunk_red + red_slot * 3;
                    slot[0] = acc[0];
                    slot[1] = acc[1];
                    slot[2] = acc[2];
                }
                acc[0] = acc[1] = acc[2] = 0.0;
            }
        }
    };
    for (int hop = 0; hop < NHOP; ++hop) {
    if constexpr (dyn) dw.init(a.n_wb, a.wctr, lane, (int)((blockIdx.x + hop) & 7));
    int64_t lb = dyn ? 0 : walk.slot;
    int dq0 = load_desc(lb), dq1 = load_desc(lb + step);
    Blk b0 = decode(dq0), b1 = decode(dq1);
    int cA[8];
    d2 vA[8];
    Ops oA;
    issue(b0, cA, vA, oA);
#ifdef QBH_WAVE_TIMING
#define QBH_TICK(i, t_from) do { __builtin_amdgcn_sched_barrier(0); const unsigned long long t_ = __builtin_amdgcn_s_memtime(); tm[i] += t_ - (t_from); t_from = t_; __builtin_amdgcn_sched_barrier(0); } while (0)
    unsigned long long t_mark = __builtin_amdgcn_s_memtime();
#else
#define QBH_TICK(i, t_from) do { } while (0)
#endif
    while (dyn ? dw.live(lb) : (lb < walk.per_xcd)) {
        const int dq2 = load_desc(lb + 2 * step);
        unsigned int reply = 0;
        bool asking = false;
        if constexpr (dyn) {
            asking = dw.asks(lb);
            if (asking) {
                if constexpr (CHUNKRED) {
                    red_flush();
                    red_slot = dw.chunk_slot();
                }
                reply = dw.ask(lane);
            }
        }
        d2 xv[8];
        if constexpr (C16) {
            const d2 *xq = a.xg + b0.xb + (OPS == 3 ? (lane & 7) : 0);
            if constexpr (G8) {
#pragma unroll
                for (int u = 0; u < 8; ++u) xv[u] = xq[__shfl(cA[0], (lane >> 3) + 8 * u, 64) << 3];
            } else {
#pragma unroll
                for (int u = 0; u < 8; ++u) xv[u] = xq[OPS == 3 ? (cA[u] << 3) : cA[u]];
            }
        } else {
#pragma unroll
            for (int u = 0; u < 8; ++u) xv[u] = a.xg[cA[u]];
        }
        issue_ops(b0, oA);
        __builtin_amdgcn_sched_barrier(0);
        int cB[8];
        d2 vB[8];
        Ops oB;
        issue(b1, cB, vB, oB);
        __builtin_amdgcn_sched_barrier(0);
        QBH_TICK(0, t_mark);
        if (b0.n >= 0) {
#pragma unroll
            for (int u = 0; u < 8; ++u) prod[lane + u * 64] = cmul(vA[u], xv[u]);
            wave_lds_fence();
            QBH_TICK(1, t_mark);
            constexpr int RSTRIDE = OPS == 3 ? 8 : 1;
            const int nrows_blk = OPS == 3 ? 8 * b0.nr : b0.nr;
            const int64_t first_row = OPS == 3 ? (int64_t)b0.r0 * 8 : (int64_t)b0.r0;
            open_block(first_row, nrows_blk, b0.cont0, true);
            int pk = 0, round_end = b0.lead;
            auto lens_round = [&](int len_raw, int rb) {
                const int len = rb + lane < b0.nr ? len_raw : 0;
                int inc = len;
                inc += __builtin_amdgcn_update_dpp(0, inc, 0x111, 0xf, 0xf, false);
                inc += __builtin_amdgcn_update_dpp(0, inc, 0x112, 0xf, 0xf, false);
                inc += __builtin_amdgcn_update_dpp(0, inc, 0x114, 0xf, 0xf, false);
                inc += __builtin_amdgcn_update_dpp(0, inc, 0x118, 0xf, 0xf, false);
                inc += __builtin_amdgcn_update_dpp(0, inc, 0x142, 0xa, 0xf, false);
                inc += __builtin_amdgcn_update_dpp(0, inc, 0x143, 0xc, 0xf, false);
                pk = (round_end + inc - len) | (len << 16);
                round_end += __builtin_amdgcn_readlane(inc, 63);
            };
            if constexpr (NL) lens_round(oA.s, 0);
            for (int rbase = 0; rbase < nrows_blk; rbase += RP) {
                const int row = rbase + rloc;
                int s_ = oA.s, e_ = oA.e;
                bool clip = false;
                d2 yo = oA.yo, xi = oA.xi, fr = oA.fr;
                if (OPS == 3) {
                    group_range(b0, oA.s, row, s_, e_, clip);
                    if (row >= nrows_blk) s_ = e_ = 0;
                } else if constexpr (NL) {
                    if (rbase > 0 && (rbase & 63) == 0) {
                        const int last = b0.nr - rbase - 1;
                        lens_round(a.len8[(int64_t)b0.r0 + rbase + (lane < last ? lane : last)], rbase);
                    }
                    const int q = __shfl(pk, row & 63, 64);
                    s_ = q & 0xffff;
                    e_ = s_ + (q >> 16);
                    if (row >= nrows_blk) s_ = e_ = 0;
                    if (EPI && rbase > 0 && sub == 0 && row < nrows_blk) {
                        yo = need_y ? a.yin[b0.r0 + row] : d2{0.0, 0.0};
                        xi = a.xl[b0.r0 + row];
                        if (FAR) fr = far_at((int64_t)b0.r0 + row, b0.cls);
                    }
                } else if (rbase > 0) {
                    s_ = e_ = 0;
                    if (row < nrows_blk) {
                        s_ = (int)(a.ia[b0.r0 + row] - b0.p0);
                        e_ = (int)(a.ia[b0.r0 + row + 1] - b0.p0);
                        if (EPI && sub == 0) {
                            yo = need_y ? a.yin[b0.r0 + row] : d2{0.0, 0.0};
                            xi = a.xl[b0.r0 + row];
                            if (FAR) fr = far_at((int64_t)b0.r0 + row, b0.cls);
                        }
                    }
                }
                d2 sum = {0.0, 0.0};
                for (int k = s_ + sub * RSTRIDE; k < e_; k += TPR * RSTRIDE) sum += prod[k];
#pragma unroll
                for (int off = TPR / 2; off > 0; off >>= 1) {
                    sum.x += __shfl_xor(sum.x, off, 64);
                    sum.y += __shfl_xor(sum.y, off, 64);
                }
                if (sub == 0 && row < nrows_blk) finish_row(first_row + row, sum, yo, xi, fr, clip);
            }
            close_block(first_row, nrows_blk, b0.cont1);
            QBH_TICK(2, t_mark);
            wave_lds_fence();
        } else {
            open_block(0, 0, false, false);
            for (int r = 0; r < (OPS == 3 ? 0 : b0.nr); ++r) {
                const int64_t row = (int64_t)b0.r0 + r;
                const int64_t s_ = a.ia[row], e_ = a.ia[row + 1];
                d2 sum = {0.0, 0.0};
                for (int64_t k = s_ + lane; k < e_; k += 64) sum += cmul(a.val[k], C16 ? a.xg[b0.xb + a.ja16[k]] : a.xg[a.ja[k] & a.colmask]);
                sum.x = wave_sum(sum.x);
                sum.y = wave_sum(sum.y);
                if (lane == 0) {
                    d2 yo = {0.0, 0.0}, xi = {0.0, 0.0}, fr = {0.0, 0.0};
                    if (EPI) {
                        if (need_y) yo = a.yin[row];
                        xi = a.xl[row];
                        if (FAR) fr = far_at(row, b0.cls);
                    }
                    finish_row(row, sum, yo, xi, fr, false);
                }
            }
        }
#pragma unroll
        for (int u = 0; u < 8; ++u) {
            cA[u] = cB[u];
            vA[u] = vB[u];
        }
        oA.s = oB.s;
        oA.e = oB.e;
        b0 = b1;
        b1 = decode(dq2);
        if constexpr (dyn) {
            if (asking) dw.nxt = dw.take(reply);
        }
        lb += step;
        if constexpr (dyn) dw.advance(lb);
#ifdef QBH_WAVE_TIMING
        asm volatile("s_waitcnt vmcnt(0)" ::: "memory");
        QBH_TICK(3, t_mark);
        ++nblk;
#endif
    }
    flush();
    red_flush();
    red_slot = -1;
    }
#ifdef QBH_XCD_TIMING
    if (dyn && lane == 0) {
        const unsigned long long t_end = wall_clock64();
        atomicMax(a.wctr + (blockIdx.x & 7) * 16 + 1, t_end);
        atomicMin(a.wctr + (blockIdx.x & 7) * 16 + 2, t_end);
    }
#endif
#ifdef QBH_WAVE_TIMING
    if (lane == 0) {
        unsigned long long *dbg = a.wctr + 128 - 8;
        for (int i = 0; i < 4; ++i) atomicAdd(dbg + i, tm[i]);
        atomicAdd(dbg + 4, nblk);
    }
#endif
    if (!CHUNKRED && a.partials != nullptr) {
#pragma unroll
        for (int c = 0; c < 3; ++c) acc[c] = wave_sum(acc[c]);
        if (lane == 0) {
#pragma unroll
            for (int c = 0; c < 3; ++c) red[c * 4 + wv] = acc[c];
        }
        __syncthreads();
        if (tid == 0) {
#pragma unroll
            for (int c = 0; c < 3; ++c)
                a.partials[(size_t)blockIdx.x * 3 + c] = (red[c * 4 + 0] + red[c * 4 + 1]) + (red[c * 4 + 2] + red[c * 4 + 3]);
        }
    }
}

__global__ __launch_bounds__(256) void k_reduce_chunks(const double *slots, int64_t n_slots, double *partials)
{
    __shared__ double sm[12];
    const int64_t per = (n_slots + gridDim.x - 1) / gridDim.x, s0 = (int64_t)blockIdx.x * per, s1 = s0 + per < n_slots ? s0 + per : n_slots;
    double v[3] = {0.0, 0.0, 0.0};
    for (int64_t i = s0 + threadIdx.x; i < s1; i += 256) {
        v[0] += slots[i * 3 + 0];
        v[1] += slots[i * 3 + 1];
        v[2] += slots[i * 3 + 2];
    }
#pragma unroll
    for (int c = 0; c < 3; ++c) v[c] = wave_sum(v[c]);
    if ((threadIdx.x & 63) == 0)
        for (int c = 0; c < 3; ++c) sm[c * 4 + (threadIdx.x >> 6)] = v[c];
    __syncthreads();
    if (threadIdx.x == 0)
        for (int c = 0; c < 3; ++c) partials[(size_t)blockIdx.x * 3 + c] = (sm[c * 4 + 0] + sm[c * 4 + 1]) + (sm[c * 4 + 2] + sm[c * 4 + 3]);
}
int launch_reduce_chunks(const double *slots, int64_t n_slots, double *partials, int *nparts_out, hipStream_t s)
{
    const int g = 256;
    hipLaunchKernelGGL(k_reduce_chunks, dim3(g), dim3(256), 0, s, slots, n_slots, partials);
    QBH_HIP(hipGetLastError());
    if (nparts_out) *nparts_out = g;
    return QBH_OK;
}
int64_t wave2_chunk_slots(int64_t n_wb)
{
    const int64_t per = (n_wb + 7) >> 3;
    return 8 * ((per + kDynChunk - 1) / kDynChunk);
}

template <int OPS, bool C16, bool G8 = false, bool NL = false, bool V8 = false>
static SpmvKernel wave2_kernel_tpr(int tpr, bool dyn)
{
    switch (tpr) {
    case 2:  return dyn ? k_spmv_wave2<2, OPS, true, C16, G8, NL, V8> : k_spmv_wave2<2, OPS, false, C16, G8, NL, V8>;
    case 4:  return dyn ? k_spmv_wave2<4, OPS, true, C16, G8, NL, V8> : k_spmv_wave2<4, OPS, false, C16, G8, NL, V8>;
    default: return dyn ? k_spmv_wave2<8, OPS, true, C16, G8, NL, V8> : k_spmv_wave2<8, OPS, false, C16, G8, NL, V8>;
    }
}

template <int OPS, bool C16>
static SpmvKernel wave2_kernel_nl(int tpr, bool dyn, bool nl)
{
    return nl ? wave2_kernel_tpr<OPS, C16, false, true>(tpr, dyn) : wave2_kernel_tpr<OPS, C16>(tpr, dyn);
}

static SpmvKernel wave2_kernel(int tpr, int ops, bool dyn, bool c16, bool g8, bool nl, bool v8)
{
    if (nl && ops != 1 && ops != 2) return nullptr;
    if (v8 && !g8) return nullptr;
    if (g8) {
        if (!c16 || ops != 3) return nullptr;
        return v8 ? wave2_kernel_tpr<3, true, true, false, true>(tpr, dyn) : wave2_kernel_tpr<3, true, true>(tpr, dyn);
    }
    if (c16) {
        switch (ops) {
        case 1:  return wave2_kernel_nl<1, true>(tpr, dyn, nl);
        case 2:  return wave2_kernel_nl<2, true>(tpr, dyn, nl);
        case 3:  return wave2_kernel_tpr<3, true>(tpr, dyn);
        default: return nullptr;
        }
    }
    switch (ops) {
    case 0:  return wave2_kernel_tpr<0, false>(tpr, dyn);
    case 1:  return wave2_kernel_nl<1, false>(tpr, dyn, nl);
    case 3:  return wave2_kernel_tpr<3, false>(tpr, dyn);
    case 4:  return wave2_kernel_tpr<4, false>(tpr, dyn);
    default: return wave2_kernel_nl<2, false>(tpr, dyn, nl);
    }
}

int launch_spmv_wave2(const SpmvArgs &a_in, int tpr, int ops, int grid, hipStream_t s)
{
    SpmvArgs a = a_in;
    if (a.yin == nullptr) a.yin = a.y;
    if (a.swizzle == 3 && (ops == 1 || ops == 2 || ops == 4) && a.chunk_red == nullptr) {
        set_error("launch_spmv_wave2: the dynamic walk of an epilogue pass needs its chunk-partial slots");
        return QBH_EINVAL;
    }
    const SpmvKernel k = wave2_kernel(tpr, ops, a.swizzle == 3, a.ja16 != nullptr, a.ja8 != nullptr, a.len8 != nullptr, a.val8 != nullptr);
    if (k == nullptr) {
        set_error("launch_spmv_wave2: 2-byte%s columns%s%s with pass form %d", a.ja8 ? " grouped" : "", a.len8 ? " / row lengths" : "",
                  a.val8 ? " / grouped values" : "", ops);
        return QBH_EINVAL;
    }
    return launch_kernel(k, grid, kBlock, s, a);
}

int wave2_kernel_occupancy(int tpr, int ops)
{
    return kernel_occupancy(wave2_kernel(tpr, ops, true, false, false, false, false));
}

}
```

Measured before the change: 50.18.

## Share near-pass value pattern across Kronecker blocks, storing only diagonal per row

Adds a setup kernel that checks whether every block of S rows in the near part repeats the same off-diagonal values and column layout. When it does, it keeps one shared value pattern plus a per-row diagonal and diagonal position. The near SpMV kernel gets a VP variant that reads values from the small shared pattern, which should stay cache-resident, and substitutes the diagonal product in place. This is meant to cut the per-nonzero value traffic from HBM. In exchange it adds extra per-row loads, a compare inside the inner loop, and new kernel instantiations.

```diff
diff --git a/quantum_basis_amd/csrc/qbh_api.cpp b/quantum_basis_amd/csrc/qbh_api.cpp
--- a/quantum_basis_amd/csrc/qbh_api.cpp
+++ b/quantum_basis_amd/csrc/qbh_api.cpp
@@ -40,7 +40,7 @@
                         {"mf_window", &d.mf_window, nullptr}, {"kronc_abl", &d.kronc_abl, nullptr}, {"kronc_far_chunk", &d.kronc_far_chunk, nullptr},
                         {"kronc_far_ng", &d.kronc_far_ng, nullptr}, {"kronc_far_nt", &d.kronc_far_nt, nullptr}, {"no_far_align", &d.no_far_align, nullptr}, {"far_cols8", &d.far_cols8, nullptr},
                         {"far_vals8", &d.far_vals8, nullptr},
-                        {"near_lens", &d.near_lens, nullptr}, {"near_len_cap", &d.near_len_cap, nullptr},
+                        {"near_lens", &d.near_lens, nullptr}, {"near_vals", &d.near_vals, nullptr}, {"near_len_cap", &d.near_len_cap, nullptr},
                         {"no_defer", &d.no_defer, nullptr}, {"pipe_nospec", &d.pipe_nospec, nullptr}, {"host_delay_us", &d.host_delay_us, nullptr},
                         {"side_noprio", &d.side_noprio, nullptr}, {"comm_reserve", &d.comm_reserve, nullptr}, {"comm_far_cap", &d.comm_far_cap, nullptr}};
     const std::string all(e);
@@ -892,7 +892,7 @@
         info->n_blocks = K.nwb_n + K.nwb_f + K.nwb_x;
         info->bytes_matrix = (A->nrows + 1) * 16 + ((K.sliced ? K.n_groups : A->nrows) + 1) * 8 + (K.n_xrows + 1) * (K.xrow ? 12 : 8) +
                              (K.own_far ? nnz + K.far_slots : nnz) * 20 + (K.nwb_n + K.nwb_f + K.nwb_x + 6) * 16;
-        info->bytes_matrix += (A->d_ja ? 0 : -4 * nnz) + 2 * (K.c16_n ? K.nnz_n : 0) + 2 * (K.c16_f ? K.far_slots : 0) + 2 * (K.c8_f ? K.far_slots / 8 + 64 : 0) + 16 * (K.v8_f ? K.far_slots / 8 + 64 : 0) + (K.len_n ? A->nrows + 64 : 0) + ((!A->d_ja && K.own_x) ? 4 * K.nnz_x : 0);
+        info->bytes_matrix += (A->d_ja ? 0 : -4 * nnz) + 2 * (K.c16_n ? K.nnz_n : 0) + 2 * (K.c16_f ? K.far_slots : 0) + 2 * (K.c8_f ? K.far_slots / 8 + 64 : 0) + 16 * (K.v8_f ? K.far_slots / 8 + 64 : 0) + (K.len_n ? A->nrows + 64 : 0) + (K.vp_n ? 16 * (K.pat_n + 64) + 9 * (A->nrows + 64) : 0) + ((!A->d_ja && K.own_x) ? 4 * K.nnz_x : 0);
         info->kron_cols16 = (K.c16_n ? 1 : 0) | (K.c16_f ? 2 : 0);
         info->kron_classes = K.map.nc;
         info->kron_cross_nnz = K.nnz_x;
diff --git a/quantum_basis_amd/csrc/qbh_api_priv.hpp b/quantum_basis_amd/csrc/qbh_api_priv.hpp
--- a/quantum_basis_amd/csrc/qbh_api_priv.hpp
+++ b/quantum_basis_amd/csrc/qbh_api_priv.hpp
@@ -29,6 +29,7 @@
 int kron_geometry(qbh_csr *A);
 int kron_short_cols(qbh_csr *A);
 int kron_near_lens(qbh_csr *A);
+int kron_near_vals(qbh_csr *A);
 int kron_build(qbh_csr *A);
 int kron_restore(qbh_csr *A);
 void kronc_release(qbh_csr *A);
diff --git a/quantum_basis_amd/csrc/qbh_internal.hpp b/quantum_basis_amd/csrc/qbh_internal.hpp
--- a/quantum_basis_amd/csrc/qbh_internal.hpp
+++ b/quantum_basis_amd/csrc/qbh_internal.hpp
@@ -34,6 +34,7 @@
     int far_cols8 = -1;
     int far_vals8 = -1;
     int near_lens = -1;
+    int near_vals = -1;
     int near_len_cap = 0;
     int no_defer = 0;
     int host_delay_us = 0;
@@ -120,6 +121,10 @@
     const uint16_t *ja8;
     const d2      *val8;
     const uint8_t *len8;
+    const d2      *valp;
+    const double  *diag;
+    const uint8_t *dpos8;
+    int64_t        kK;
     double *chunk_red;
     const d2      *yin;
     const double  *coef;
@@ -267,6 +272,7 @@
 int launch_kron_c16_far(const WaveDesc *wd, const int32_t *ja, int64_t slots, int64_t NU, uint16_t *out, int *flag, hipStream_t s);
 int launch_kron_c8_far(const uint16_t *c16, int64_t slots, uint16_t *out, int *flag, hipStream_t s);
 int launch_kron_v8_far(const d2 *val, int64_t slots, d2 *out, int *flag, hipStream_t s);
+int launch_kron_near_vals(const int64_t *ia, const uint16_t *c16, const d2 *val, int64_t nrows, int64_t S, int64_t K, d2 *vp, double *dg, uint8_t *dp, int *flag, hipStream_t s);
 int launch_kron_near_lens(const int64_t *ia, int64_t nrows, const WaveDesc *wd, int64_t n_wb, int cap, uint8_t *out, int *flag, hipStream_t s);
 int launch_kron_check2(const int64_t *ia, const int32_t *ja, int64_t nrows, int64_t S, int64_t U0, int *d_flag, hipStream_t s);
 int basis_to_internal(qbh_csr *A, int kind, int n_sites, int n_up, int n_dn, bool *applied);
@@ -665,6 +671,10 @@
         uint16_t *c8_f = nullptr;
         qbh::d2 *v8_f = nullptr;
         uint8_t *len_n = nullptr;
+        qbh::d2 *vp_n = nullptr;
+        double  *dg_n = nullptr;
+        uint8_t *dp_n = nullptr;
+        int64_t  pat_n = 0;
         qbh::d2 *val_n = nullptr, *val_f = nullptr;
         qbh::WaveDesc *wd_n = nullptr, *wd_f = nullptr;
         int64_t  nwb_n = 0, nwb_f = 0;
diff --git a/quantum_basis_amd/csrc/qbh_kron.hip b/quantum_basis_amd/csrc/qbh_kron.hip
--- a/quantum_basis_amd/csrc/qbh_kron.hip
+++ b/quantum_basis_amd/csrc/qbh_kron.hip
@@ -314,6 +314,56 @@
     if (bad) *flag = 1;
 }
 
+__global__ __launch_bounds__(kBlock) void k_kron_near_vals(const int64_t *ia, const uint16_t *c16, const d2 *val, int64_t nrows, int64_t S, int64_t K, d2 *vp,
+                                                           double *dg, uint8_t *dp, int *flag)
+{
+    const int sub = threadIdx.x & 7;
+    const int64_t ia0 = ia[0];
+    bool bad = false;
+    for (int64_t r = ((int64_t)blockIdx.x * blockDim.x + threadIdx.x) >> 3; r < ((nrows + 7) / 8) * 8; r += ((int64_t)gridDim.x * blockDim.x) >> 3) {
+        int nd = 0, pos = 0;
+        if (r < nrows) {
+            const int64_t u = r / S, d = r - u * S;
+            const int64_t s = ia[r], e = ia[r + 1], s0 = ia[d], e0 = ia[d + 1];
+            const bool same = e - s == e0 - s0 && s - u * K == s0;
+            bad = bad || !same;
+            for (int64_t k = s + sub; same && k < e; k += 8) {
+                const int64_t k0 = s0 + (k - s);
+                const bool diag = (int64_t)c16[k] % S == d, diag0 = (int64_t)c16[k0] % S == d;
+                const d2 v = val[k];
+                if (diag) {
+                    ++nd;
+                    pos = (int)(k - s);
+                    dg[r] = v.x;
+                    bad = bad || __double_as_longlong(v.y) != 0;
+                } else {
+                    const d2 w = val[k0];
+                    bad = bad || __double_as_longlong(v.x) != __double_as_longlong(w.x) || __double_as_longlong(v.y) != __double_as_longlong(w.y);
+                }
+                bad = bad || diag != diag0;
+                if (u == 0 && k - ia0 < K) vp[k - ia0] = v;
+            }
+        }
+        for (int off = 4; off > 0; off >>= 1) {
+            nd += __shfl_xor(nd, off, 64);
+            pos += __shfl_xor(pos, off, 64);
+        }
+        if (sub == 0 && r < nrows) {
+            bad = bad || nd != 1 || pos > 255;
+            dp[r] = (uint8_t)pos;
+        }
+    }
+    if (bad) *flag = 1;
+}
+
+}
+
+int launch_kron_near_vals(const int64_t *ia, const uint16_t *c16, const d2 *val, int64_t nrows, int64_t S, int64_t K, d2 *vp, double *dg, uint8_t *dp, int *flag,
+                          hipStream_t s)
+{
+    hipLaunchKernelGGL(k_kron_near_vals, dim3(8192), dim3(kBlock), 0, s, ia, c16, val, nrows, S, K, vp, dg, dp, flag);
+    QBH_HIP(hipGetLastError());
+    return QBH_OK;
 }
 
 int launch_kron_near_lens(const int64_t *ia, int64_t nrows, const WaveDesc *wd, int64_t n_wb, int cap, uint8_t *out, int *flag, hipStream_t s)
diff --git a/quantum_basis_amd/csrc/qbh_split.cpp b/quantum_basis_amd/csrc/qbh_split.cpp
--- a/quantum_basis_amd/csrc/qbh_split.cpp
+++ b/quantum_basis_amd/csrc/qbh_split.cpp
@@ -64,7 +64,7 @@
 {
     qbh_csr::KronSplit &K = A->kron;
     for (void *q : {(void *)K.ia_n, (void *)K.ia_f, (void *)K.wd_n, (void *)K.wd_f, (void *)K.d_xt, (void *)K.d_far, (void *)K.ia_x, (void *)K.xrow,
-                    (void *)K.wd_x, (void *)K.d_cls, (void *)K.c16_n, (void *)K.c16_f, (void *)K.c8_f, (void *)K.v8_f, (void *)K.len_n, (void *)K.d_chunk_red, (void *)K.d_need, (void *)K.d_send_list, (void *)K.d_vsend, (void *)K.d_vrecv})
+                    (void *)K.wd_x, (void *)K.d_cls, (void *)K.c16_n, (void *)K.c16_f, (void *)K.c8_f, (void *)K.v8_f, (void *)K.len_n, (void *)K.vp_n, (void *)K.dg_n, (void *)K.dp_n, (void *)K.d_chunk_red, (void *)K.d_need, (void *)K.d_send_list, (void *)K.d_vsend, (void *)K.d_vrecv})
         if (q) (void)hipFree(q);
     if (K.own_far) {
         if (K.ja_f) (void)hipFree(K.ja_f);
@@ -221,6 +221,40 @@
         A, A->nrows, [&](uint8_t *l, int *flag) { return qbh::launch_kron_near_lens(K.ia_n, A->nrows, K.wd_n, K.nwb_n, cap, l, flag, A->stream); });
     return QBH_OK;
 }
+
+int kron_near_vals(qbh_csr *A)
+{
+    qbh_csr::KronSplit &K = A->kron;
+    if (K.vp_n || K.map.nc != 1 || !K.c16_n || !K.ia_n || !K.val_n || qbh::debug_sw().near_vals == 0) return QBH_OK;
+    const int64_t S = K.t.S, n = A->nrows;
+    if (S <= 0 || n < S || n % S != 0) return QBH_OK;
+    int64_t first = 0, next = 0;
+    if (hipMemcpy(&first, K.ia_n, sizeof(int64_t), hipMemcpyDeviceToHost) != hipSuccess ||
+        hipMemcpy(&next, K.ia_n + S, sizeof(int64_t), hipMemcpyDeviceToHost) != hipSuccess) {
+        (void)hipGetLastError();
+        return QBH_OK;
+    }
+    const int64_t pat = next - first;
+    if (pat < 1024 || pat >= ((int64_t)1 << 30)) return QBH_OK;
+    DevPtr<d2> vp;
+    DevPtr<double> dg;
+    DevPtr<uint8_t> dp;
+    if (vp.alloc((size_t)pat + 64) != hipSuccess || dg.alloc((size_t)n + 64) != hipSuccess || dp.alloc((size_t)n + 64) != hipSuccess) {
+        (void)hipGetLastError();
+        return QBH_OK;
+    }
+    (void)derive_into(A, vp, pat, [&](d2 *p, int *flag) -> int {
+        if (hipMemsetAsync(dg.get() + n, 0, 64 * sizeof(double), A->stream) != hipSuccess || hipMemsetAsync(dp.get() + n, 0, 64, A->stream) != hipSuccess)
+            return QBH_EHIP;
+        return qbh::launch_kron_near_vals(K.ia_n, K.c16_n, K.val_n, n, S, pat, p, dg.get(), dp.get(), flag, A->stream);
+    });
+    if (!vp.get()) return QBH_OK;
+    K.vp_n = vp.release();
+    K.dg_n = dg.release();
+    K.dp_n = dp.release();
+    K.pat_n = pat;
+    return QBH_OK;
+}
 }
 
 namespace {
@@ -544,6 +578,7 @@
         KRON_TRY(kron_geometry(A));
         KRON_TRY(kron_short_cols(A));
         KRON_TRY(kron_near_lens(A));
+        KRON_TRY(kron_near_vals(A));
         if (qbh::debug_sw().print_ptrs)
             fprintf(stderr, "qbhip kron arrays: ia %p ja %p val %p | ia_n %p fp %p | ja_f %p val_f %p | wd_n %p wd_f %p | far %p | nnz_n %lld far_slots %lld\n", (void *)A->d_ia,
                     (void *)A->d_ja, (void *)A->d_val, (void *)K.ia_n, (void *)K.ia_f, (void *)K.ja_f, (void *)K.val_f, (void *)K.wd_n, (void *)K.wd_f, (void *)K.d_far,
diff --git a/quantum_basis_amd/csrc/qbh_spmv_kron.cpp b/quantum_basis_amd/csrc/qbh_spmv_kron.cpp
--- a/quantum_basis_amd/csrc/qbh_spmv_kron.cpp
+++ b/quantum_basis_amd/csrc/qbh_spmv_kron.cpp
@@ -304,6 +304,12 @@
     nr.ja = K.ja_n;
     nr.ja16 = K.c16_n;
     nr.len8 = K.len_n;
+    if (K.vp_n && K.c16_n) {
+        nr.valp = K.vp_n;
+        nr.diag = K.dg_n;
+        nr.dpos8 = K.dp_n;
+        nr.kK = K.pat_n;
+    }
     nr.val = K.val_n;
     nr.wd = K.wd_n;
     nr.n_wb = K.nwb_n;
diff --git a/quantum_basis_amd/csrc/qbh_spmv_wave.hip b/quantum_basis_amd/csrc/qbh_spmv_wave.hip
--- a/quantum_basis_amd/csrc/qbh_spmv_wave.hip
+++ b/quantum_basis_amd/csrc/qbh_spmv_wave.hip
@@ -218,7 +218,7 @@
 #else
 #define QBH_ROW_STORE(p, v) (*(p) = (v))
 #endif
-template <int TPR, int OPS, bool DYN, bool C16 = false, bool G8 = false, bool NL = false, bool V8 = false>
+template <int TPR, int OPS, bool DYN, bool C16 = false, bool G8 = false, bool NL = false, bool V8 = false, bool VP = false>
 __global__ __launch_bounds__(kBlock) __attribute__((amdgpu_waves_per_eu((OPS == 0 || OPS == 3) ? QBH_FAR_WAVES : QBH_NEAR_WAVES, (OPS == 0 || OPS == 3) ? QBH_FAR_WAVES : QBH_NEAR_WAVES))) void k_spmv_wave2(SpmvArgs a)
 {
     spmv_args_resolve(a);
@@ -226,6 +226,7 @@
     static_assert(!G8 || (C16 && OPS == 3), "grouped columns: the sliced far pass with 2-byte columns");
     static_assert(!NL || OPS == 1 || OPS == 2, "row lengths: the one-class near passes");
     static_assert(!V8 || G8, "grouped values: only beside the grouped columns");
+    static_assert(!VP || (C16 && (OPS == 1 || OPS == 2)), "shared value pattern: the one-class near passes with 2-byte columns");
     constexpr int NW = 512, RP = 64 / TPR;
     constexpr bool EPI = OPS == 1 || OPS == 2 || OPS == 4, FAR = OPS == 2 || OPS == 4;
     constexpr bool CHUNKRED = DYN && (OPS == 1 || OPS == 2 || OPS == 4);
@@ -259,6 +260,7 @@
         int cls;
         int64_t xb;
         int lead;
+        int ve;
     };
     const uint32_t kS32 = (uint32_t)a.kS, kB32 = (uint32_t)a.kB;
     const int kLB = 31 - __builtin_clz(kB32 | 1u);
@@ -288,9 +290,14 @@
         b.nr = __builtin_amdgcn_readlane(dq, 6) - b.r0;
         b.cls = MULTI ? __builtin_amdgcn_readlane(dq, 3) : 0;
         b.xb = 0;
+        b.ve = 0;
         if constexpr (C16) {
             const int64_t pad = (uint32_t)__builtin_amdgcn_readlane(dq, 3);
             b.xb = OPS == 3 ? (pad >> 1) * 8 * a.kNU : pad * a.kS;
+            if constexpr (VP) {
+                const int64_t ve = b.p0 - pad * a.kK;
+                b.ve = (ve >= -8 && ve < a.kK) ? (int)ve : 0;
+            }
         }
         b.cont0 = OPS == 3 && (__builtin_amdgcn_readlane(dq, 3) & 1);
         b.cont1 = OPS == 3 && (__builtin_amdgcn_readlane(dq, 7) & 1);
@@ -301,6 +308,8 @@
     struct Ops {
         int s, e;
         d2 yo, xi, fr;
+        int dp;
+        double dg;
     };
     auto group_range = [&](const Blk &b, int gp, int row, int &s_, int &e_, bool &clip) {
         const int gi = row >> 3;
@@ -337,6 +346,16 @@
             for (int u = 0; u < 8; ++u) {
                 const int l = (lane >> 3) + 8 * u;
                 v[u] = ntload(a.val8 + (base >> 3) + (l < lm ? l : lm));
+            }
+        } else if constexpr (VP) {
+            const int kk = (int)a.kK, e0 = b.n > 0 ? b.ve : 0;
+#pragma unroll
+            for (int u = 0; u < 8; ++u) {
+                const int i = lane + u * 64;
+                int e = e0 + (i < nn ? i : nm1);
+                e = e >= kk ? e - kk : e;
+                e = e < 0 ? e + kk : e;
+                v[u] = a.valp[e];
             }
         } else {
 #pragma unroll
@@ -357,12 +376,14 @@
             const int last = b.nr > 0 ? b.nr - 1 : 0;
             o.s = a.len8[(int64_t)b.r0 + (lane < last ? lane : last)];
             o.e = 0;
+            if constexpr (VP) o.dp = a.dpos8[(int64_t)b.r0 + (lane < last ? lane : last)];
         } else {
             const bool mine = rloc < b.nr;
             const int64_t row = mine ? (int64_t)b.r0 + rloc : 0;
             o.s = (int)(a.ia[row] - base);
             o.e = (int)(a.ia[row + 1] - base);
             if (!mine) o.s = o.e = 0;
+            if constexpr (VP) o.dp = a.dpos8[row];
         }
     };
     auto issue_ops = [&](const Blk &b, Ops &o) {
@@ -372,6 +393,7 @@
             o.yo = a.yin[row];
             o.xi = a.xl[row];
             o.fr = FAR ? far_at(row, b.cls) : d2{0.0, 0.0};
+            if constexpr (VP) o.dg = a.diag[row];
             if (!need_y) o.yo = d2{0.0, 0.0};
         }
     };
@@ -534,7 +556,7 @@
             const int64_t first_row = OPS == 3 ? (int64_t)b0.r0 * 8 : (int64_t)b0.r0;
             open_block(first_row, nrows_blk, b0.cont0, true);
             int pk = 0, round_end = b0.lead;
-            auto lens_round = [&](int len_raw, int rb) {
+            auto lens_round = [&](int len_raw, int dp_raw, int rb) {
                 const int len = rb + lane < b0.nr ? len_raw : 0;
                 int inc = len;
                 inc += __builtin_amdgcn_update_dpp(0, inc, 0x111, 0xf, 0xf, false);
@@ -544,45 +566,72 @@
                 inc += __builtin_amdgcn_update_dpp(0, inc, 0x142, 0xa, 0xf, false);
                 inc += __builtin_amdgcn_update_dpp(0, inc, 0x143, 0xc, 0xf, false);
                 pk = (round_end + inc - len) | (len << 16);
+                if constexpr (VP) pk |= dp_raw << 24;
                 round_end += __builtin_amdgcn_readlane(inc, 63);
             };
-            if constexpr (NL) lens_round(oA.s, 0);
+            if constexpr (NL) lens_round(oA.s, VP ? oA.dp : 0, 0);
             for (int rbase = 0; rbase < nrows_blk; rbase += RP) {
                 const int row = rbase + rloc;
                 int s_ = oA.s, e_ = oA.e;
                 bool clip = false;
                 d2 yo = oA.yo, xi = oA.xi, fr = oA.fr;
+                double dg = 0.0;
+                int dk = -1;
+                if constexpr (VP) dg = oA.dg;
                 if (OPS == 3) {
                     group_range(b0, oA.s, row, s_, e_, clip);
                     if (row >= nrows_blk) s_ = e_ = 0;
                 } else if constexpr (NL) {
                     if (rbase > 0 && (rbase & 63) == 0) {
                         const int last = b0.nr - rbase - 1;
-                        lens_round(a.len8[(int64_t)b0.r0 + rbase + (lane < last ? lane : last)], rbase);
+                        const int64_t at = (int64_t)b0.r0 + rbase + (lane < last ? lane : last);
+                        lens_round(a.len8[at], VP ? a.dpos8[at] : 0, rbase);
                     }
                     const int q = __shfl(pk, row & 63, 64);
                     s_ = q & 0xffff;
-                    e_ = s_ + (q >> 16);
+                    if constexpr (VP) {
+                        e_ = s_ + ((q >> 16) & 0xff);
+                        dk = s_ + (int)((uint32_t)q >> 24);
+                    } else {
+                        e_ = s_ + (q >> 16);
+                    }
                     if (row >= nrows_blk) s_ = e_ = 0;
-                    if (EPI && rbase > 0 && sub == 0 && row < nrows_blk) {
-                        yo = need_y ? a.yin[b0.r0 + row] : d2{0.0, 0.0};
-                        xi = a.xl[b0.r0 + row];
-                        if (FAR) fr = far_at((int64_t)b0.r0 + row, b0.cls);
-                    }
-                } else if (rbase > 0) {
-                    s_ = e_ = 0;
-                    if (row < nrows_blk) {
-                        s_ = (int)(a.ia[b0.r0 + row] - b0.p0);
-                        e_ = (int)(a.ia[b0.r0 + row + 1] - b0.p0);
-                        if (EPI && sub == 0) {
+                    if (EPI && rbase > 0 && (VP || sub == 0) && row < nrows_blk) {
+                        if (sub == 0) {
                             yo = need_y ? a.yin[b0.r0 + row] : d2{0.0, 0.0};
-                            xi = a.xl[b0.r0 + row];
                             if (FAR) fr = far_at((int64_t)b0.r0 + row, b0.cls);
                         }
+                        xi = a.xl[b0.r0 + row];
+                        if constexpr (VP) dg = a.diag[b0.r0 + row];
                     }
+                } else {
+                    int dp = 0;
+                    if constexpr (VP) dp = oA.dp;
+                    if (rbase > 0) {
+                        s_ = e_ = 0;
+                        if (row < nrows_blk) {
+                            s_ = (int)(a.ia[b0.r0 + row] - b0.p0);
+                            e_ = (int)(a.ia[b0.r0 + row + 1] - b0.p0);
+                            if constexpr (VP) dp = a.dpos8[b0.r0 + row];
+                            if (EPI && (VP || sub == 0)) {
+                                if (sub == 0) {
+                                    yo = need_y ? a.yin[b0.r0 + row] : d2{0.0, 0.0};
+                                    if (FAR) fr = far_at((int64_t)b0.r0 + row, b0.cls);
+                                }
+                                xi = a.xl[b0.r0 + row];
+                                if constexpr (VP) dg = a.diag[b0.r0 + row];
+                            }
+                        }
+                    }
+                    if constexpr (VP) dk = s_ + dp;
                 }
                 d2 sum = {0.0, 0.0};
-                for (int k = s_ + sub * RSTRIDE; k < e_; k += TPR * RSTRIDE) sum += prod[k];
+                if constexpr (VP) {
+                    const d2 dprod = cmul(d2{dg, 0.0}, xi);
+                    for (int k = s_ + sub; k < e_; k += TPR) sum += k == dk ? dprod : prod[k];
+                } else {
+                    for (int k = s_ + sub * RSTRIDE; k < e_; k += TPR * RSTRIDE) sum += prod[k];
+                }
 #pragma unroll
                 for (int off = TPR / 2; off > 0; off >>= 1) {
                     sum.x += __shfl_xor(sum.x, off, 64);
@@ -620,6 +669,7 @@
         }
         oA.s = oB.s;
         oA.e = oB.e;
+        if constexpr (VP) oA.dp = oB.dp;
         b0 = b1;
         b1 = decode(dq2);
         if constexpr (dyn) {
@@ -699,34 +749,40 @@
     return 8 * ((per + kDynChunk - 1) / kDynChunk);
 }
 
-template <int OPS, bool C16, bool G8 = false, bool NL = false, bool V8 = false>
+template <int OPS, bool C16, bool G8 = false, bool NL = false, bool V8 = false, bool VP = false>
 static SpmvKernel wave2_kernel_tpr(int tpr, bool dyn)
 {
     switch (tpr) {
-    case 2:  return dyn ? k_spmv_wave2<2, OPS, true, C16, G8, NL, V8> : k_spmv_wave2<2, OPS, false, C16, G8, NL, V8>;
-    case 4:  return dyn ? k_spmv_wave2<4, OPS, true, C16, G8, NL, V8> : k_spmv_wave2<4, OPS, false, C16, G8, NL, V8>;
-    default: return dyn ? k_spmv_wave2<8, OPS, true, C16, G8, NL, V8> : k_spmv_wave2<8, OPS, false, C16, G8, NL, V8>;
+    case 2:  return dyn ? k_spmv_wave2<2, OPS, true, C16, G8, NL, V8, VP> : k_spmv_wave2<2, OPS, false, C16, G8, NL, V8, VP>;
+    case 4:  return dyn ? k_spmv_wave2<4, OPS, true, C16, G8, NL, V8, VP> : k_spmv_wave2<4, OPS, false, C16, G8, NL, V8, VP>;
+    default: return dyn ? k_spmv_wave2<8, OPS, true, C16, G8, NL, V8, VP> : k_spmv_wave2<8, OPS, false, C16, G8, NL, V8, VP>;
     }
 }
 
 template <int OPS, bool C16>
-static SpmvKernel wave2_kernel_nl(int tpr, bool dyn, bool nl)
-{
+static SpmvKernel wave2_kernel_nl(int tpr, bool dyn, bool nl, bool vp = false)
+{
+    if constexpr (C16) {
+        if (vp) return nl ? wave2_kernel_tpr<OPS, true, false, true, false, true>(tpr, dyn) : wave2_kernel_tpr<OPS, true, false, false, false, true>(tpr, dyn);
+    } else {
+        if (vp) return nullptr;
+    }
     return nl ? wave2_kernel_tpr<OPS, C16, false, true>(tpr, dyn) : wave2_kernel_tpr<OPS, C16>(tpr, dyn);
 }
 
-static SpmvKernel wave2_kernel(int tpr, int ops, bool dyn, bool c16, bool g8, bool nl, bool v8)
+static SpmvKernel wave2_kernel(int tpr, int ops, bool dyn, bool c16, bool g8, bool nl, bool v8, bool vp)
 {
     if (nl && ops != 1 && ops != 2) return nullptr;
     if (v8 && !g8) return nullptr;
+    if (vp && !c16) return nullptr;
     if (g8) {
         if (!c16 || ops != 3) return nullptr;
         return v8 ? wave2_kernel_tpr<3, true, true, false, true>(tpr, dyn) : wave2_kernel_tpr<3, true, true>(tpr, dyn);
     }
     if (c16) {
         switch (ops) {
-        case 1:  return wave2_kernel_nl<1, true>(tpr, dyn, nl);
-        case 2:  return wave2_kernel_nl<2, true>(tpr, dyn, nl);
+        case 1:  return wave2_kernel_nl<1, true>(tpr, dyn, nl, vp);
+        case 2:  return wave2_kernel_nl<2, true>(tpr, dyn, nl, vp);
         case 3:  return wave2_kernel_tpr<3, true>(tpr, dyn);
         default: return nullptr;
         }
@@ -748,10 +804,10 @@
         set_error("launch_spmv_wave2: the dynamic walk of an epilogue pass needs its chunk-partial slots");
         return QBH_EINVAL;
     }
-    const SpmvKernel k = wave2_kernel(tpr, ops, a.swizzle == 3, a.ja16 != nullptr, a.ja8 != nullptr, a.len8 != nullptr, a.val8 != nullptr);
+    const SpmvKernel k = wave2_kernel(tpr, ops, a.swizzle == 3, a.ja16 != nullptr, a.ja8 != nullptr, a.len8 != nullptr, a.val8 != nullptr, a.valp != nullptr);
     if (k == nullptr) {
-        set_error("launch_spmv_wave2: 2-byte%s columns%s%s with pass form %d", a.ja8 ? " grouped" : "", a.len8 ? " / row lengths" : "",
-                  a.val8 ? " / grouped values" : "", ops);
+        set_error("launch_spmv_wave2: %s%s columns%s%s%s with pass form %d", a.ja16 ? "2-byte" : "int32", a.ja8 ? " grouped" : "", a.len8 ? " / row lengths" : "",
+                  a.val8 ? " / grouped values" : "", a.valp ? " / shared value pattern" : "", ops);
         return QBH_EINVAL;
     }
     return launch_kernel(k, grid, kBlock, s, a);
@@ -759,7 +815,7 @@
 
 int wave2_kernel_occupancy(int tpr, int ops)
 {
-    return kernel_occupancy(wave2_kernel(tpr, ops, true, false, false, false, false));
-}
-
-}
+    return kernel_occupancy(wave2_kernel(tpr, ops, true, false, false, false, false, false));
+}
+
+}
```

After: 59.83, median of 6. +19.2%, better.
